# yangao07/LAMSA

Hardware: AMD Instinct MI355X
Metric: aligned Gbase/s, 10 kbp ONT-error reads (12%: sub/ins/del 4% each), -T ont2d vs GRCh37-sized stand-in; inputs resident in HBM when the timed region starts (upload excluded: see pcie_inclusive_*) (higher is better)
Workload: dtype int32

## Files before the change

lamsa_amd/csrc/hp_align_api.hip:

```cpp
#include <hip/hip_runtime.h>
#include <algorithm>
#include <atomic>
#include <map>
#include <mutex>
#include <stdlib.h>
#include <string.h>
#include <time.h>
#include "hp_phase.h"
#include "hp_handle.h"
#include "hp_hostprep.h"

using namespace hp;

#ifndef HP_WAVES_PER_SIMD
#define HP_WAVES_PER_SIMD 4
#endif
__global__ __launch_bounds__(64, HP_WAVES_PER_SIMD) void k_align_batch(AlignArgs a)
{
    __shared__ int32_t lds[HP_BOTH_LDS_WORDS];
    const int slot = blockIdx.x;
    for (;;) {
        int u = 0;
        if (wv::leader()) u = atomicAdd(a.counter, 1);
        u = wv::uni(u);
// ... 144 lines not shown
    for (int64_t i = (int64_t)blockIdx.x * blockDim.x + threadIdx.x; i < n; i += (int64_t)gridDim.x * blockDim.x) { const int b = src[i]; dst[i] = ((b & 63) << 4) | (b >> 6); }
}
__global__ void k_off_widen(const int32_t *src, int64_t *dst, int64_t n)
{
    for (int64_t i = (int64_t)blockIdx.x * blockDim.x + threadIdx.x; i < n; i += (int64_t)gridDim.x * blockDim.x) dst[i] = src[i];
}
#define HP_SCAN_BLOCK 4096
__global__ __launch_bounds__(256) void k_scan_sums(const uint8_t *src, int64_t n, int64_t *sums)
{
    __shared__ int part[256];
    const int64_t b0 = (int64_t)blockIdx.x * HP_SCAN_BLOCK;
    int s = 0;
    for (int i = threadIdx.x; i < HP_SCAN_BLOCK; i += 256) { const int64_t k = b0 + i; s += k < n ? src[k] : 0; }
    part[threadIdx.x] = s;
    __syncthreads();
    for (int st = 128; st > 0; st >>= 1) { if ((int)threadIdx.x < st) part[threadIdx.x] += part[threadIdx.x + st]; __syncthreads(); }
    if (threadIdx.x == 0) sums[blockIdx.x] = part[0];
}
__global__ __launch_bounds__(256) void k_scan_bases(int64_t *sums, int64_t nb)
{
    __shared__ long long tot[256];
    const int64_t per = (nb + 255) / 256, a = (int64_t)threadIdx.x * per, b = a + per < nb ? a + per : nb;
    long long s = 0;
    for (int64_t i = a; i < b; ++i) s += sums[i];
    tot[threadIdx.x] = s;
    __syncthreads();
    if (threadIdx.x == 0) { long long run = 0; for (int t = 0; t < 256; ++t) { const long long v = tot[t]; tot[t] = run; run += v; } }
    __syncthreads();
    long long run = tot[threadIdx.x];
    for (int64_t i = a; i < b; ++i) { const long long v = sums[i]; sums[i] = run; run += v; }
}
__global__ __launch_bounds__(256) void k_scan_apply(const uint8_t *src, int64_t n, const int64_t *bases, int64_t *dst)
{
    __shared__ int part[256];
    const int64_t b0 = (int64_t)blockIdx.x * HP_SCAN_BLOCK + (int64_t)threadIdx.x * 16;
    int v[16], s = 0;
#pragma unroll
    for (int i = 0; i < 16; ++i) { const int64_t k = b0 + i; v[i] = k < n ? src[k] : 0; s += v[i]; }
    part[threadIdx.x] = s;
    __syncthreads();
    if (threadIdx.x == 0) { int run = 0; for (int t = 0; t < 256; ++t) { const int x = part[t]; part[t] = run; run += x; } }
    __syncthreads();
    long long run = bases[blockIdx.x] + part[threadIdx.x];
#pragma unroll
    for (int i = 0; i < 16; ++i) { const int64_t k = b0 + i; if (k < n) dst[k] = run; run += v[i]; }
}

static double now_s() { timespec t; clock_gettime(CLOCK_MONOTONIC, &t); return t.tv_sec + 1e-9 * t.tv_nsec; }
static const bool g_trace = getenv("LAMSA_HP_TRACE") != nullptr;
static const bool g_noshare = getenv("LAMSA_HP_FULL_GRIDS") != nullptr;
static const bool g_nowave = getenv("LAMSA_HP_NO_WAVE_JOBS") != nullptr;
static const bool g_nolane = getenv("LAMSA_HP_NO_LANE_DP") != nullptr;
static const bool g_mono = getenv("LAMSA_HP_ONE_KERNEL") != nullptr;

struct HostBuf {
    void *p = nullptr, *dev = nullptr; size_t cap = 0;
    int ensure(size_t bytes) {
        if (bytes <= cap) return 0;
        if (p) hipHostFree(p);
        p = dev = nullptr; cap = 0;
        size_t want = bytes + bytes / 4 + 256;
        if (hipHostMalloc(&p, want, hipHostMallocMapped) != hipSuccess) { p = nullptr; return -1; }
        if (hipHostGetDevicePointer(&dev, p, 0) != hipSuccess) { hipHostFree(p); p = nullptr; return -1; }
        cap = want;
        return 0;
    }
    void release() { if (p) hipHostFree(p); p = dev = nullptr; cap = 0; }
};

struct OutDev {
    DevBuf buf; HostBuf host; int64_t stream_cap = 0; int n_cap = 0;
    static size_t hdr(int n) { return al256(8 * (size_t)n) + 3 * al256(4 * (size_t)n) + 256 + al256(16 * (size_t)n); }
    int ensure(int n, int64_t cap) { stream_cap = cap; n_cap = n; return buf.ensure(4 * (size_t)cap + 256) || host.ensure(hdr(n) + 256); }
    int64_t *off() const { return (int64_t *)host.dev; }
    int32_t *len(int n) const { return (int32_t *)((char *)host.dev + al256(8 * (size_t)n)); }
    int32_t *st(int n) const { return (int32_t *)((char *)host.dev + al256(8 * (size_t)n) + al256(4 * (size_t)n)); }
    int32_t *tb(int n) const { return (int32_t *)((char *)host.dev + al256(8 * (size_t)n) + 2 * al256(4 * (size_t)n)); }
    unsigned long long *diag(int n) const { return (unsigned long long *)((char *)host.dev + al256(8 * (size_t)n) + 3 * al256(4 * (size_t)n)); }
    const unsigned long long *h_diag(int n) const { return (const unsigned long long *)((const char *)host.p + al256(8 * (size_t)n) + 3 * al256(4 * (size_t)n)); }
    int32_t *work(int n) const { return (int32_t *)((char *)host.dev + al256(8 * (size_t)n) + 3 * al256(4 * (size_t)n) + 256); }
    const int32_t *h_work(int n) const { return (const int32_t *)((const char *)host.p + al256(8 * (size_t)n) + 3 * al256(4 * (size_t)n) + 256); }
    const int64_t *h_off() const { return (const int64_t *)host.p; }
    const int32_t *h_len(int n) const { return (const int32_t *)((const char *)host.p + al256(8 * (size_t)n)); }
    const int32_t *h_st(int n) const { return (const int32_t *)((const char *)host.p + al256(8 * (size_t)n) + al256(4 * (size_t)n)); }
    const int32_t *h_tb(int n) const { return (const int32_t *)((const char *)host.p + al256(8 * (size_t)n) + 2 * al256(4 * (size_t)n)); }
    int32_t *stream(int) const { return (int32_t *)buf.p; }
    void release() { buf.release(); host.release(); }
};

struct Slot {
    DevBuf bin, misc, slab, pers, prof; OutDev out1;
    HostBuf args_host;
    hipEvent_t ep[7] = {nullptr, nullptr, nullptr, nullptr, nullptr, nullptr, nullptr};
    hipStream_t cs = nullptr;
    bool valid = false;
    bool phased = false;
    int32_t n_reads = 0; int64_t n_bases = 0, n_cig = 0, n_hits = 0;
    BatchIn in; const int32_t *d_order = nullptr;
    std::vector<int32_t> order, h_len, h_H; std::vector<uint8_t> h_skip;
    int32_t max_L = 0, max_H = 0;
    int32_t sort_pb = 40, sort_cb = 24;
    hipEvent_t e0 = nullptr, e1 = nullptr;
};

struct AlignState {
    Slot slot[2];
    int fifo[2] = {0, 0}, n_fifo = 0;
    int res_fifo[2] = {0, 0}, n_res = 0;
    DevBuf retry_list;
    OutDev out2;
    HostBuf stream;
    std::vector<int32_t> r_len, r_st, r_tb, r_work; std::vector<int64_t> r_off;
};

static std::map<lamsa_hp_handle *, AlignState *> g_states;
static std::mutex g_states_lock;
static AlignState *state_of(lamsa_hp_handle *h)
{
    std::lock_guard<std::mutex> guard(g_states_lock);
    auto it = g_states.find(h);
    if (it != g_states.end()) return it->second;
    return g_states[h] = new AlignState();
}
extern "C" void lamsa_hp_release_state_(lamsa_hp_handle *h)
{
    AlignState *S = nullptr;
    {
        std::lock_guard<std::mutex> guard(g_states_lock);
        auto it = g_states.find(h);
        if (it == g_states.end()) return;
        S = it->second;
        g_states.erase(it);
    }
    if (h->stream) hipStreamSynchronize(h->stream);
    if (h->stream_b) hipStreamSynchronize(h->stream_b);
    for (Slot &T : S->slot) { T.bin.release(); T.misc.release(); T.slab.release(); T.pers.release(); T.prof.release(); T.args_host.release(); T.out1.release(); for (hipEvent_t e : {T.e0, T.e1, T.ep[0], T.ep[1], T.ep[2], T.ep[3], T.ep[4], T.ep[5], T.ep[6]}) if (e) hipEventDestroy(e); }
    S->retry_list.release(); S->out2.release(); S->stream.release();
    delete S;
}

static int grow(lamsa_hp_handle *h, DevBuf &b, size_t bytes)
{
    if (bytes <= b.cap) return 0;
    if (hipStreamSynchronize(h->stream) != hipSuccess || hipStreamSynchronize(h->stream_b) != hipSuccess) return -1;
    return b.ensure(bytes);
}

static size_t tag_slab_per_base(int tags, int eqx) { return (size_t)((tags & HP_TAGS_LISTS) ? 152 : 128) + ((tags & LAMSA_HP_TAG_EQX) ? (size_t)eqx : 0); }
static size_t slab_bytes_for(const lamsa_hp_para &P, int L, int H, int scale, int tags)
{
    const size_t z = (2 * (size_t)P.band_w + 128) * ((size_t)L + 256);
    return al256(((size_t)256 << 10) + (size_t)scale * tag_slab_per_base(tags, 40) * (size_t)L + 424 * (size_t)H + z * (size_t)(scale > 1 ? 4 : 1));
}


static int upload_into(lamsa_hp_handle *h, Slot *S, const lamsa_hp_batch *B)
{
    S->valid = false;
    const double t_0 = now_s();
    const int n = B->n_reads;
    const int64_t n_slots = n ? B->seed_off[n] : 0, n_hits = n_slots ? B->hit_off[n_slots] : 0, n_bases = n ? B->read_off[n] : 0;
    S->h_len.assign((size_t)n, 0); S->h_H.assign((size_t)n, 0); S->h_skip.assign((size_t)n + 1, 0); S->max_L = 0; S->max_H = 0;
    if (n && (B->seed_off[0] != 0 || B->read_off[0] != 0 || (n_slots && B->hit_off[0] != 0))) { h->err = "offsets must start at 0"; return LAMSA_HP_EINVAL; }
    const bool packed_off = B->h_cig_off == nullptr, cig_bytes = B->cig8 != nullptr;
    if (B->n_cig < 0 || (!packed_off && B->n_cig > 0x7fffffffll)) { h->err = "more than 2^31-1 seed CIGAR elements with 32-bit h_cig_off: pass h_cig_off = NULL (CIGARs back to back in hit order) or split the batch"; return LAMSA_HP_EINVAL; }
    if (!cig_bytes && !B->cig && B->n_cig > 0) { h->err = "neither cig nor cig8 given"; return LAMSA_HP_EINVAL; }
    {
        std::atomic<int> bad(0);
        const int64_t sl = h->para.seed_len, ss = h->para.seed_step > 0 ? h->para.seed_step : 1;
        std::atomic<long long> max_pos(0), sum_cig(0);
        hp_parallel_blocks(n, [&](int r0, int r1) {
            long long mp = 0, sc = 0;
            for (int r = r0; r < r1 && !bad.load(std::memory_order_relaxed); ++r) {
                const int64_t L = B->read_off[r + 1] - B->read_off[r], ns = B->seed_off[r + 1] - B->seed_off[r];
                if (L < 0 || L > (1 << 24) || ns < 0) { bad = 1; return; }
                if (ns > HP_MAX_SLOTS) S->h_skip[r] = 1;
                {
                    const int64_t sa = L < sl ? 0 : 1 + (L - sl) / ss;
                    if (B->seed_all[r] != sa || B->last_len[r] != L - sl - (sa - 1) * ss) { bad = 7; return; }
                    if (sa > 32767) S->h_skip[r] = 1;
                }
                int64_t H = 0;
                for (int64_t s = B->seed_off[r]; s < B->seed_off[r + 1]; ++s) {
                    const int64_t m = B->hit_off[s + 1] - B->hit_off[s];
                    if (m < 0 || (m > HP_MAX_HITS_PER_SEED && !S->h_skip[r])) { bad = 2; return; }
                    if (B->seed_id[s] < 1 || B->seed_id[s] > B->seed_all[r] || (s > B->seed_off[r] && B->seed_id[s] <= B->seed_id[s - 1])) { bad = 3; return; }
                    H += m;
                }
                if (H > (1 << 22) && !S->h_skip[r]) { bad = 4; return; }
                for (int64_t i = B->read_off[r]; i < B->read_off[r + 1]; ++i) if (B->read_seq[i] > 4) { bad = 5; return; }
                for (int64_t k = B->hit_off[B->seed_off[r]]; k < B->hit_off[B->seed_off[r + 1]]; ++k) {
                    mp = B->h_pos[k] > mp ? B->h_pos[k] : mp;
                    if (B->h_len_dif[k] < -127 || B->h_len_dif[k] > 127) S->h_skip[r] = 1;
                    if (B->h_chr[k] < 1 || B->h_chr[k] > h->n_seqs || (B->h_strand[k] != 1 && B->h_strand[k] != -1) || B->h_pos[k] < 0 || B->h_pos[k] >= (1ll << 40) ||
                        (!packed_off && (B->h_cig_off[k] < 0 || (int64_t)B->h_cig_off[k] + B->h_cig_n[k] > B->n_cig))) { bad = 6; return; }
                    sc += B->h_cig_n[k];
                }
                S->h_len[r] = (int32_t)L; S->h_H[r] = (int32_t)H;
            }
            long long seen = max_pos.load();
            while (mp > seen && !max_pos.compare_exchange_weak(seen, mp)) { }
            sum_cig += sc;
        });
        static const char *why[] = {"", "read longer than 2^24 bases", "too many hits in one seed", "seed ids must be ascending in [1, seed_all]",
                                    "too many hits in one read", "read base code > 4",
                                    "bad hit record (contig id, strand, position or seed CIGAR range)",
                                    "seed_all / last_len do not match the read length and the handle's seed length and step"};
        if (bad) { h->err = why[bad.load()]; return LAMSA_HP_EINVAL; }
        if (packed_off && sum_cig.load() != B->n_cig) { h->err = "h_cig_off is NULL but the h_cig_n do not add up to n_cig"; return LAMSA_HP_EINVAL; }
        for (int r = 0; r < n; ++r) { if (S->h_skip[r]) { S->h_len[r] = 0; S->h_H[r] = 0; } S->max_L = std::max(S->max_L, S->h_len[r]); S->max_H = std::max(S->max_H, S->h_H[r]); }
        auto bits = [](unsigned long long x) { int b = 0; while (x) { ++b; x >>= 1; } return b; };
        S->sort_pb = bits((unsigned long long)max_pos.load()); S->sort_cb = bits((unsigned long long)(2 * (long long)h->n_seqs + 1));
    }
    const double t_1 = now_s();
    S->order.resize((size_t)n);
    for (int r = 0; r < n; ++r) S->order[r] = r;
    {
        std::vector<double> cost((size_t)n);
        for (int r = 0; r < n; ++r) cost[r] = (double)S->h_H[r] * S->h_H[r] / 64.0 + (double)S->h_len[r] * (2.0 * h->para.band_w + 1) / 16.0;
        std::stable_sort(S->order.begin(), S->order.end(), [&](int x, int y) { return cost[x] > cost[y]; });
    }
    size_t off = 0;
    auto place = [&](size_t bytes) { size_t o = off; off = al256(off + bytes + 16); return o; };
    const size_t o_roff = place(8 * ((size_t)n + 1)), o_rseq = place((size_t)n_bases), o_sall = place(4 * (size_t)n), o_last = place(4 * (size_t)n),
                 o_soff = place(8 * ((size_t)n + 1)), o_sid = place(4 * (size_t)n_slots), o_hoff = place(8 * ((size_t)n_slots + 1)),
                 o_pos = place(8 * (size_t)n_hits), o_chr = place(4 * (size_t)n_hits), o_coff = place(8 * (size_t)n_hits), o_nm = place(2 * (size_t)n_hits),
                 o_ld = place(2 * (size_t)n_hits), o_st = place((size_t)n_hits), o_cn = place((size_t)n_hits), o_cig = place(4 * (size_t)B->n_cig), o_ord = place(4 * (size_t)n),
                 o_stage = place(packed_off ? 8 * ((size_t)n_hits / HP_SCAN_BLOCK + 2) : 4 * (size_t)n_hits), o_cig8 = place(cig_bytes ? (size_t)B->n_cig : 0), o_skip = place((size_t)n);
    const double t_3 = now_s();
    if (S->bin.ensure(off)) { h->err = "hipMalloc(batch)"; return LAMSA_HP_ENOMEM; }
    char *d = (char *)S->bin.p;
    hipStream_t s = h->copy_stream;
    static const int64_t zero64 = 0;
#define UP(o, src, bytes) do { if ((bytes) > 0) HIPCHK(h, hipMemcpyAsync(d + (o), (src), (bytes), hipMemcpyHostToDevice, s), LAMSA_HP_EKERNEL); } while (0)
    if (n) { UP(o_roff, B->read_off, 8 * ((size_t)n + 1)); UP(o_soff, B->seed_off, 8 * ((size_t)n + 1)); }
    else { UP(o_roff, &zero64, 8); UP(o_soff, &zero64, 8); }
    UP(o_rseq, B->read_seq, (size_t)n_bases); UP(o_sall, B->seed_all, 4 * (size_t)n); UP(o_last, B->last_len, 4 * (size_t)n);
    UP(o_sid, B->seed_id, 4 * (size_t)n_slots);
    if (n_slots) UP(o_hoff, B->hit_off, 8 * ((size_t)n_slots + 1)); else UP(o_hoff, &zero64, 8);
    UP(o_pos, B->h_pos, 8 * (size_t)n_hits); UP(o_chr, B->h_chr, 4 * (size_t)n_hits);
    if (!packed_off) UP(o_stage, B->h_cig_off, 4 * (size_t)n_hits);
    UP(o_nm, B->h_nm, 2 * (size_t)n_hits); UP(o_ld, B->h_len_dif, 2 * (size_t)n_hits); UP(o_st, B->h_strand, (size_t)n_hits); UP(o_cn, B->h_cig_n, (size_t)n_hits);
    if (cig_bytes) UP(o_cig8, B->cig8, (size_t)B->n_cig); else UP(o_cig, B->cig, 4 * (size_t)B->n_cig);
    UP(o_ord, S->order.data(), 4 * (size_t)n); UP(o_skip, S->h_skip.data(), (size_t)n);
#undef UP
    if (cig_bytes && B->n_cig > 0) hipLaunchKernelGGL(k_cig8_expand, dim3(2048), dim3(256), 0, s, (const uint8_t *)(d + o_cig8), (int32_t *)(d + o_cig), (int64_t)B->n_cig);
    if (n_hits > 0) {
        if (!packed_off) hipLaunchKernelGGL(k_off_widen, dim3(2048), dim3(256), 0, s, (const int32_t *)(d + o_stage), (int64_t *)(d + o_coff), (int64_t)n_hits);
        else {
            const int64_t nb = (n_hits + HP_SCAN_BLOCK - 1) / HP_SCAN_BLOCK;
            hipLaunchKernelGGL(k_scan_sums, dim3((unsigned)nb), dim3(256), 0, s, (const uint8_t *)(d + o_cn), (int64_t)n_hits, (int64_t *)(d + o_stage));
            hipLaunchKernelGGL(k_scan_bases, dim3(1), dim3(256), 0, s, (int64_t *)(d + o_stage), nb);
            hipLaunchKernelGGL(k_scan_apply, dim3((unsigned)nb), dim3(256), 0, s, (const uint8_t *)(d + o_cn), (int64_t)n_hits, (const int64_t *)(d + o_stage), (int64_t *)(d + o_coff));
        }
    }
    HIPCHK(h, hipGetLastError(), LAMSA_HP_EKERNEL);
    HIPCHK(h, hipStreamSynchronize(s), LAMSA_HP_EKERNEL);
    if (g_trace) fprintf(stderr, "[lamsa_hp] upload: validate %.1f ms, order %.1f ms, copy %.1f ms (%.2f GB on the device)\n", 1e3 * (t_1 - t_0), 1e3 * (t_3 - t_1), 1e3 * (now_s() - t_3), off / 1e9);
    BatchIn &in = S->in;
    in.n_reads = n; in.read_skip = (const uint8_t *)(d + o_skip); in.read_off = (const int64_t *)(d + o_roff); in.read_seq = (const uint8_t *)(d + o_rseq);
    in.seed_all = (const int32_t *)(d + o_sall); in.last_len = (const int32_t *)(d + o_last); in.seed_off = (const int64_t *)(d + o_soff);
    in.seed_id = (const int32_t *)(d + o_sid); in.hit_off = (const int64_t *)(d + o_hoff); in.h_pos = (const int64_t *)(d + o_pos);
    in.h_chr = (const int32_t *)(d + o_chr); in.h_cig_off = (const int64_t *)(d + o_coff); in.h_nm = (const int16_t *)(d + o_nm);
    in.h_len_dif = (const int16_t *)(d + o_ld); in.h_strand = (const int8_t *)(d + o_st); in.h_cig_n = (const uint8_t *)(d + o_cn);
    in.cig = (const int32_t *)(d + o_cig);
    S->d_order = (const int32_t *)(d + o_ord);
    S->n_reads = n; S->n_bases = n_bases; S->n_cig = B->n_cig; S->n_hits = n_hits;
    S->valid = true;
    return LAMSA_HP_OK;
}

static int cap_waves(int n_waves, size_t slab_per_wave, int n_cu)
{
    static const size_t budget = []() { size_t f = 0, t = 0; if (hipMemGetInfo(&f, &t) != hipSuccess || t == 0) { t = (size_t)288 << 30; f = t; } return std::min(t / 4, f / 3); }();
    if (slab_per_wave * (size_t)n_waves <= budget) return n_waves;
    size_t fit = budget / (slab_per_wave ? slab_per_wave : 1);
    if (n_cu > 0 && fit >= (size_t)n_cu) fit -= fit % (size_t)n_cu;
    return fit < 1 ? 1 : (int)fit;
}

#ifdef HP_PROF
static void prof_report(Slot &T, const long long *d_prof, int n)
{
    if (!d_prof) return;
    {
        std::vector<long long> pr((size_t)n * 64);
        hipMemcpy(pr.data(), d_prof, sizeof(long long) * pr.size(), hipMemcpyDeviceToHost);
        if (const char *dump = getenv("LAMSA_HP_PROF_DUMP")) {
            if (FILE *fp = fopen(dump, "wb")) {
                for (int r = 0; r < n; ++r) { long long hl[2] = {T.h_H[r], T.h_len[r]}; fwrite(hl, 8, 2, fp); fwrite(&pr[(size_t)r * 64], 8, 64, fp); }
                fclose(fp);
            }
        }
        std::vector<int> idx((size_t)n); for (int i = 0; i < n; ++i) idx[i] = i;
        auto tot = [&](int r) { long long t = 0; for (int k = 0; k < 6; ++k) t += pr[(size_t)r * 64 + k]; return t; };
        std::sort(idx.begin(), idx.end(), [&](int x, int y) { return tot(x) > tot(y); });
        long long sum[64] = {0}; for (int r = 0; r < n; ++r) for (int k = 0; k < 64; ++k) sum[k] += pr[(size_t)r * 64 + k];
        fprintf(stderr, "[HP_PROF] cycles: setup chain1 fill1 chain2 fill2 publish | in chain1: init+minext mainscan track pop-loop bound+flines | o_l H\n");
        fprintf(stderr, "[HP_PROF] SUM  "); for (int k = 0; k < 11; ++k) fprintf(stderr, " %lld", sum[k] / 1000000); fprintf(stderr, " (Mcycles) targets %lld trips %lld init_Mcyc %lld\n", sum[11], sum[12], sum[13] / 1000000);
#ifdef HP_PROF_TRACK
        fprintf(stderr, "[HP_PROF] branch tracking (-DHP_PROF_TRACK: the line_build stamps below are off): marking pass, image build and write-back %lld Mcyc; %lld seeds visited; %lld tracks, %lld Mcyc in them, %lld steps up; "
                        "%lld arrivals at a node with several sons, %lld Mcyc in cut_branch\n", sum[16] / 1000000, sum[19], sum[18], sum[17] / 1000000, sum[20], sum[21], sum[22] / 1000000);
#endif
        fprintf(stderr, "[HP_PROF] line_build: %lld lines (%lld without a gap), %lld anchors, %lld gaps | Mcyc: anchor walk %lld, gap list %lld, gaps in lanes %lld, gaps one by one %lld, assembly %lld\n",
                sum[21], sum[22], sum[12], sum[23], sum[16] / 1000000, sum[17] / 1000000, sum[18] / 1000000, sum[19] / 1000000, sum[20] / 1000000);
        fprintf(stderr, "[HP_PROF] gaps: %lld in lines with fewer than HP_GAP_MIN gaps (%lld lines with gaps); lane gaps: %lld hits scanned, %lld refused (range too long or too many active hits)\n", sum[54], sum[55], sum[11], sum[13]);
        { const char *nm[] = {"ksw_global", "ksw_extend", "backtrack", "ref_fetch", "head_fix", "frag_extend", "split_mapping", "tail_fix", "res_split", "res_aux", "mini_line_regs", "sort index"};
          for (int k = 0; k < 12; ++k) fprintf(stderr, "[HP_PROF] %-16s %8lld Mcyc %10lld calls\n", nm[k], sum[24 + 2 * k] / 1000000, sum[25 + 2 * k]);
#ifdef HP_PROF_FILL
          fprintf(stderr, "[HP_PROF] in frags_merge: boundary repair (merge_cigar_full) %lld Mcyc %lld calls; junctions through split_mapping %lld Mcyc %lld calls; fragments of several seeds %lld Mcyc %lld calls; 64-step gathers %lld Mcyc %lld\n", sum[16] / 1000000, sum[17], sum[18] / 1000000, sum[19], sum[20] / 1000000, sum[21], sum[22] / 1000000, sum[23]);
#endif
          fprintf(stderr, "[HP_PROF] direction-matrix bytes in HBM %lld (%lld jobs); hits passed through nodes_per_init %lld (%lld calls)\n", sum[52], sum[53], sum[54], sum[55]);
          fprintf(stderr, "[HP_PROF] chain_first start: seed loop %lld, node_set loop %lld, min_extend %lld Mcyc (%lld reads with a MIN pass)\n", sum[56] / 1000000, sum[57] / 1000000, sum[58] / 1000000, sum[59]);
          fprintf(stderr, "[HP_PROF] query <= 62: ksw_extend %lld Mcyc %lld calls, ksw_global %lld Mcyc %lld calls\n", sum[60] / 1000000, sum[61], sum[62] / 1000000, sum[63]);
          const char *bn[] = {"[bi_extend total]", "[bi_extend after left ext]", "17-32", "33-64", "65-128", "129-256", "257-512", ">512"};
          for (int k = 0; k < 2; ++k) fprintf(stderr, "[HP_PROF] ksw_extend qlen %-8s %8lld Mcyc %10lld calls\n", bn[k], sum[48 + 2 * k] / 1000000, sum[49 + 2 * k]); }
        {
            std::vector<long long> pd((size_t)n * 64);
            hipMemcpy(pd.data(), d_prof + ((size_t)n + 1) * 64, sizeof(long long) * pd.size(), hipMemcpyDeviceToHost);
            long long sd[64] = {0}; for (int r = 0; r < n; ++r) for (int k = 0; k < 64; ++k) sd[k] += pd[(size_t)r * 64 + k];
            const char *cn[] = {"one set, q <= 62", "packed, one set", "packed, two sets", "band 1 set slides", "band 2 sets slides", "band 4 sets slides", "int32 sets", "LDS / HBM rows",
                                "band 1 set fixed", "band 2 sets fixed", "band 4 sets fixed"};
            for (int c = 0; c < 11; ++c) fprintf(stderr, "[HP_PROF] wave jobs, ksw_extend %-18s %8lld Mcyc %10lld Mcells %9lld calls %10lld rows\n", cn[c], sd[4 * c] / 1000000, sd[4 * c + 1] / 1000000, sd[4 * c + 2], sd[4 * c + 3]);
            fprintf(stderr, "[HP_PROF] wave jobs, junctions of the class 'band 2 sets fixed': %lld jobs, wj_run %lld Mcyc of which staging %lld; ksw_bi_extend %lld Mcyc of which after the left extension %lld; "
                            "in ksw_extend_band<2>: setup and first fill %lld, rows %lld, backtrack %lld Mcyc\n",
                    sd[51], sd[50] / 1000000, sd[49] / 1000000, sd[47] / 1000000, sd[48] / 1000000, sd[44] / 1000000, sd[45] / 1000000, sd[46] / 1000000);
        }
        for (int q = 0; q < 8 && q < n; ++q) { int r = idx[q]; fprintf(stderr, "[HP_PROF] read %d L=%d:", r, T.h_len[r]); for (int k = 0; k < 11; ++k) fprintf(stderr, " %lld", pr[(size_t)r * 64 + k] / 1000000); fprintf(stderr, " | o_l %lld H %lld | targets %lld trips %lld init_Mcyc %lld\n", pr[(size_t)r * 64 + 14], pr[(size_t)r * 64 + 15], pr[(size_t)r * 64 + 11], pr[(size_t)r * 64 + 12], pr[(size_t)r * 64 + 13] / 1000000); }
    }
}
#endif

struct PhasedLayout { size_t bytes, o[15]; int unit_cap, lj_cap, wj_cap; int64_t fl_cap, line_cap, job_cap; };
static PhasedLayout phased_layout(int n, int64_t n_hits, int64_t n_bases, int64_t stream_cap)
{
    PhasedLayout Y;
    const size_t n_ent = (size_t)n_hits + (size_t)n + 1;
    Y.unit_cap = 8 * n + 1024;
    Y.fl_cap = 4 * n_hits + 2304 * (int64_t)n + 4096; Y.line_cap = stream_cap + 64 * (int64_t)Y.unit_cap;
    Y.job_cap = std::min<int64_t>(0x7fffff00ll, 4096 + 256 * (int64_t)n + 2 * n_bases);
    Y.lj_cap = (int)std::min<int64_t>(0x3fffffffll, 1024 + 16 * (int64_t)n + n_bases / 100);
    Y.wj_cap = (int)std::min<int64_t>(0x3fffffffll, 1024 + 32 * (int64_t)n + n_bases / 200);
    size_t off = 0;
    auto place = [&](size_t bytes) { size_t o = off; off = al256(off + bytes + 16); return o; };
    const size_t sz[15] = {sizeof(PhaseArgs), sizeof(PhaseCtl), sizeof(RdMeta) * ((size_t)n + 1), sizeof(NodeS) * n_ent, 4 * n_ent, 8 * n_ent, sizeof(UnitRec) * 2 * (size_t)Y.unit_cap,
                           4 * 2 * (size_t)PH_NBUCKET * Y.unit_cap, 4 * (size_t)Y.fl_cap, 4 * (size_t)Y.line_cap, 4 * (size_t)Y.job_cap, sizeof(LjRec) * (size_t)Y.lj_cap, 4 * (size_t)LJ_NBUCKET * Y.lj_cap,
                           sizeof(WjRec) * (size_t)Y.wj_cap, 4 * (size_t)WJ_NBUCKET * Y.wj_cap};
    for (int k = 0; k < 15; ++k) Y.o[k] = place(sz[k]);
    Y.bytes = off;
    return Y;
}
static int64_t main_stream_cap(int n, int64_t n_bases, int tags)
{
    return 1024 + (int64_t)n * 256 + 4 * n_bases + ((tags & LAMSA_HP_TAG_MISMATCHES) ? (int64_t)n * 128 + 2 * n_bases : 0) + ((tags & LAMSA_HP_TAG_EQX) ? (int64_t)n * 128 + 4 * n_bases : 0);
}

struct SlabPlan { size_t chain, fill, wj, wjb, wjb_off; int w_chain, w_fill, w_dp, w_wj, n_wjb, shape; size_t bytes; };
static int chain_shape(const lamsa_hp_para &P, int64_t n_reads, int64_t n_bases)
{
    static const int force = getenv("LAMSA_HP_CHAIN_SHAPE") ? atoi(getenv("LAMSA_HP_CHAIN_SHAPE")) : -1;
    if (force >= 0 && force < 3) return force;
    const int64_t mean_L = n_reads > 0 ? n_bases / n_reads : 0, ss = P.seed_step > 0 ? P.seed_step : 1;
    const int64_t est = mean_L / ss * 2 / 3;
    for (int k = 0; k < 2; ++k) if (est <= g_chain_shapes[k].lds_words / 5) return k;
    return 2;
}
static SlabPlan slab_plan(lamsa_hp_handle *h, int max_L, int max_H, bool shared = false, int shape = 0)
{
    SlabPlan Q;
    Q.shape = shape;
    const lamsa_hp_para &P = h->para;
    Q.chain = al256(((size_t)256 << 10) + 128 * (size_t)max_L + 424 * (size_t)max_H);
    Q.fill = al256(((size_t)256 << 10) + tag_slab_per_base(h->result_tags, 16) * (size_t)max_L + sizeof(cig_t) * 3 * HP_LJ_CIG * 64 + (size_t)HP_LJ_QSMALL * HP_LJ_TSMALL * 64 + 64);
    { static const int kb = getenv("LAMSA_HP_WJ_SLAB_KB") ? atoi(getenv("LAMSA_HP_WJ_SLAB_KB")) : 0;
      Q.wj = ((size_t)(kb > 0 ? kb : 1024) << 10) + 33 * 256; }
    Q.wjb = al256((size_t)wj_need(&P, WJ_HEAD, max_L, max_L + 2 * P.hash_step + 64) + ((size_t)64 << 10)) + 33 * 256;
    if (Q.wjb < Q.wj) Q.wjb = Q.wj;
    if (g_nowave) Q.fill = std::max(Q.fill, slab_bytes_for(P, max_L, max_H, 1, h->result_tags));
    if (h->scratch_limit) { const size_t lim = al256(h->scratch_limit); Q.chain = std::min(Q.chain, lim); Q.fill = std::min(Q.fill, lim); Q.wj = std::min(Q.wj, lim); Q.wjb = std::min(Q.wjb, lim); }
    int pc = 0, pf = 0, pd = 0, pw = 0;
    if (hipOccupancyMaxActiveBlocksPerMultiprocessor(&pc, g_chain_shapes[shape].k1, 64, 0) != hipSuccess || pc < 1) pc = 4 * g_chain_shapes[shape].waves_per_simd;
    if (hipOccupancyMaxActiveBlocksPerMultiprocessor(&pf, k_fill, 64, 0) != hipSuccess || pf < 1) pf = 4;
    if (hipOccupancyMaxActiveBlocksPerMultiprocessor(&pd, k_filldp_small, 64, 0) != hipSuccess || pd < 1) pd = 4;
    if (hipOccupancyMaxActiveBlocksPerMultiprocessor(&pw, k_filldp_wave, 64, 0) != hipSuccess || pw < 1) pw = 4;
    if (shared && !g_noshare) { pc = std::min(pc, 8); pf = std::min(pf, 16); pw = std::min(pw, 16); }
    { static const int cf = getenv("LAMSA_HP_FILL_PER_CU") ? atoi(getenv("LAMSA_HP_FILL_PER_CU")) : 0, cc = getenv("LAMSA_HP_CHAIN_PER_CU") ? atoi(getenv("LAMSA_HP_CHAIN_PER_CU")) : 0,
                       cw = getenv("LAMSA_HP_WJ_PER_CU") ? atoi(getenv("LAMSA_HP_WJ_PER_CU")) : 0;
      if (cf > 0 && cf < pf) pf = cf;
      if (cc > 0 && cc < pc) pc = cc;
      if (cw > 0 && cw < pw) pw = cw; }
    Q.w_chain = cap_waves(h->n_cu * pc, Q.chain, h->n_cu); Q.w_fill = cap_waves(h->n_cu * pf, Q.fill, h->n_cu);
    Q.w_dp = std::min(h->n_cu * pd, Q.w_fill); Q.w_wj = cap_waves(h->n_cu * pw, Q.wj, h->n_cu);
    { const size_t budget_big = (size_t)12 << 30; size_t nb = budget_big / Q.wjb; if (nb < 1) nb = 1; Q.n_wjb = (int)std::min<size_t>(nb, (size_t)Q.w_wj); }
    Q.wjb_off = al256(Q.wj * (size_t)Q.w_wj);
    const size_t wj_bytes = Q.wjb_off + Q.wjb * (size_t)Q.n_wjb;
    Q.bytes = std::max(std::max(Q.chain * (size_t)Q.w_chain, Q.fill * (size_t)Q.w_fill), wj_bytes);
    return Q;
}

static int launch_phased(lamsa_hp_handle *h, AlignState *S, Slot &T, Slot &Ln, OutDev &O, hipEvent_t e0, hipEvent_t e1)
{
    const int n = T.n_reads;
    const int64_t n_hits = T.n_hits;
    const SlabPlan Q = slab_plan(h, T.max_L, T.max_H, S->n_fifo + S->n_res > 0, chain_shape(h->para, T.n_reads, T.n_bases));
    const int w_chain = Q.w_chain, w_fill = Q.w_fill, w_dp = Q.w_dp, w_wj = Q.w_wj;
    const PhasedLayout Y = phased_layout(n, n_hits, T.n_bases, O.stream_cap);
    const int unit_cap = Y.unit_cap, lj_cap = Y.lj_cap; const int64_t fl_cap = Y.fl_cap, line_cap = Y.line_cap, job_cap = Y.job_cap;
    const size_t off = Y.bytes, o_args = Y.o[0], o_ctl = Y.o[1], o_meta = Y.o[2], o_nd = Y.o[3], o_ns = Y.o[4], o_sx = Y.o[5], o_un = Y.o[6], o_bq = Y.o[7], o_fl = Y.o[8], o_ln = Y.o[9],
                 o_jb = Y.o[10], o_lj = Y.o[11], o_lq = Y.o[12], o_wj = Y.o[13], o_wq = Y.o[14];
    if (grow(h, Ln.slab, Q.bytes) || grow(h, Ln.pers, off) || Ln.misc.ensure(256)) { h->err = "hipMalloc(slab)"; return LAMSA_HP_ENOMEM; }
    char *d = (char *)Ln.pers.p;
    PhaseArgs a;
    a.P = h->para;
    a.ref.pac = h->d_pac; a.ref.l_pac = h->l_pac; a.ref.n_seqs = h->n_seqs; a.ref.seq_off = h->d_seq_off; a.ref.seq_len = h->d_seq_len;
    a.in = T.in; a.in.tags = h->result_tags;
    a.out.read_out_off = O.off(); a.out.read_out_len = O.len(n); a.out.read_status = O.st(n); a.out.read_tbases = O.tb(n); a.out.read_work = O.work(n); a.out.stream = O.stream(n);
    a.out.stream_cap = O.stream_cap; a.out.cursor = (unsigned long long *)((char *)Ln.misc.p + 64); a.out.diag = O.diag(n);
    a.slab = (char *)Ln.slab.p; a.slab_per_wave = Q.chain; a.slab_fill = Q.fill; a.slab_wj = Q.wj; a.slab_wjb = Q.wjb; a.wjb_off = Q.wjb_off; a.n_wjb = Q.n_wjb; a.sort_pb = T.sort_pb; a.sort_cb = T.sort_cb;
    a.order = T.d_order; a.n_reads = n; a.prof = nullptr;
#ifdef HP_PROF
    if (Ln.prof.ensure(sizeof(long long) * 64 * 2 * ((size_t)n + 1))) { h->err = "hipMalloc(prof)"; return LAMSA_HP_ENOMEM; }
    a.prof = (long long *)Ln.prof.p;
    HIPCHK(h, hipMemsetAsync(Ln.prof.p, 0, sizeof(long long) * 64 * 2 * ((size_t)n + 1), Ln.cs), LAMSA_HP_EKERNEL);
#endif
    a.g_nd = (NodeS *)(d + o_nd); a.g_nseed = (int32_t *)(d + o_ns); a.g_sidx = (int32_t *)(d + o_sx); a.meta = (RdMeta *)(d + o_meta);
    a.units = (UnitRec *)(d + o_un); a.unit_cap = unit_cap; a.bucket_q = (int32_t *)(d + o_bq);
    a.fl_base = (int32_t *)(d + o_fl); a.fl_cap = fl_cap; a.line_base = (int32_t *)(d + o_ln); a.line_cap = line_cap; a.ctl = (PhaseCtl *)(d + o_ctl);
    a.job_base = (int32_t *)(d + o_jb); a.job_cap = job_cap;
    a.ljobs = (LjRec *)(d + o_lj); a.lj_bucket = (int32_t *)(d + o_lq); a.lj_cap = g_nolane ? 0 : lj_cap;
    a.wjobs = (WjRec *)(d + o_wj); a.wj_bucket = (int32_t *)(d + o_wq); a.wj_cap = g_nowave ? 0 : Y.wj_cap;
    const bool list = !g_nolane || !g_nowave;
    hipStream_t s = Ln.cs;
    HIPCHK(h, hipMemsetAsync(Ln.misc.p, 0, 128, s), LAMSA_HP_EKERNEL);
    HIPCHK(h, hipMemsetAsync(d + o_ctl, 0, (o_meta - o_ctl) + sizeof(RdMeta) * ((size_t)n + 1), s), LAMSA_HP_EKERNEL);
    if (Ln.args_host.ensure(sizeof a)) { h->err = "hipHostMalloc(args)"; return LAMSA_HP_ENOMEM; }
    memcpy(Ln.args_host.p, &a, sizeof a);
    HIPCHK(h, hipMemcpyAsync(d + o_args, Ln.args_host.p, sizeof a, hipMemcpyHostToDevice, s), LAMSA_HP_EKERNEL);
    const PhaseArgs *da = (const PhaseArgs *)(d + o_args);
    HIPCHK(h, hipEventRecord(e0, s), LAMSA_HP_EKERNEL);
    hipLaunchKernelGGL(g_chain_shapes[Q.shape].k1, dim3(std::min(w_chain, n)), dim3(64), 0, s, da);
    HIPCHK(h, hipEventRecord(Ln.ep[0], s), LAMSA_HP_EKERNEL);
    if (list) {
        hipLaunchKernelGGL(k_filllist, dim3(w_fill), dim3(64), 0, s, da, 0);
        HIPCHK(h, hipEventRecord(Ln.ep[5], s), LAMSA_HP_EKERNEL);
        if (!g_nowave) hipLaunchKernelGGL(k_filldp_wave, dim3(w_wj), dim3(64), 0, s, da, 0);
        HIPCHK(h, hipEventRecord(Ln.ep[6], s), LAMSA_HP_EKERNEL);
        if (!g_nolane) hipLaunchKernelGGL(k_filldp_small, dim3(w_dp), dim3(64), 0, s, da, 0);
    } else { HIPCHK(h, hipEventRecord(Ln.ep[5], s), LAMSA_HP_EKERNEL); HIPCHK(h, hipEventRecord(Ln.ep[6], s), LAMSA_HP_EKERNEL); }
    HIPCHK(h, hipEventRecord(Ln.ep[4], s), LAMSA_HP_EKERNEL);
    hipLaunchKernelGGL(k_fill, dim3(w_fill), dim3(64), 0, s, da, 0);
    HIPCHK(h, hipEventRecord(Ln.ep[1], s), LAMSA_HP_EKERNEL);
    hipLaunchKernelGGL(g_chain_shapes[Q.shape].k2, dim3(std::min(w_chain, n)), dim3(64), 0, s, da);
    HIPCHK(h, hipEventRecord(Ln.ep[2], s), LAMSA_HP_EKERNEL);
    if (list) {
        HIPCHK(h, hipMemsetAsync(&((PhaseCtl *)(d + o_ctl))->q_head[5], 0, 16, s), LAMSA_HP_EKERNEL);
        hipLaunchKernelGGL(k_filllist, dim3(w_fill), dim3(64), 0, s, da, 1);
        if (!g_nowave) hipLaunchKernelGGL(k_filldp_wave, dim3(w_wj), dim3(64), 0, s, da, 1);
        if (!g_nolane) hipLaunchKernelGGL(k_filldp_small, dim3(w_dp), dim3(64), 0, s, da, 1);
    }
    hipLaunchKernelGGL(k_fill, dim3(w_fill), dim3(64), 0, s, da, 1);
    HIPCHK(h, hipEventRecord(Ln.ep[3], s), LAMSA_HP_EKERNEL);
    hipLaunchKernelGGL(k_publish, dim3(std::min(h->n_cu * 8, n)), dim3(64), 0, s, da);
    HIPCHK(h, hipGetLastError(), LAMSA_HP_EKERNEL);
    HIPCHK(h, hipEventRecord(e1, s), LAMSA_HP_EKERNEL);
    Ln.phased = true;
    return LAMSA_HP_OK;
}

static int launch_align(lamsa_hp_handle *h, AlignState *S, Slot &T, Slot &Ln, OutDev &O, const int32_t *d_order, int n_units, int scale, int max_L, int max_H,
                        hipEvent_t e0, hipEvent_t e1, bool wait)
{
    size_t slab_per_wave = slab_bytes_for(h->para, max_L, max_H, scale, h->result_tags);
    if (scale == 1 && h->scratch_limit && slab_per_wave > h->scratch_limit) slab_per_wave = al256(h->scratch_limit);
    int per_cu = 0;
    if (hipOccupancyMaxActiveBlocksPerMultiprocessor(&per_cu, k_align_batch, 64, 0) != hipSuccess || per_cu < 1) per_cu = 4;
    int n_waves = h->n_cu * per_cu;
    if (n_waves > n_units) n_waves = n_units;
    n_waves = cap_waves(n_waves, slab_per_wave, h->n_cu);
    if (grow(h, Ln.slab, slab_per_wave * (size_t)n_waves) || Ln.misc.ensure(256)) { h->err = "hipMalloc(slab)"; return LAMSA_HP_ENOMEM; }
    const int n = T.n_reads;
    AlignArgs a;
    a.P = h->para;
    a.ref.pac = h->d_pac; a.ref.l_pac = h->l_pac; a.ref.n_seqs = h->n_seqs; a.ref.seq_off = h->d_seq_off; a.ref.seq_len = h->d_seq_len;
    a.in = T.in; a.in.tags = h->result_tags;
    a.out.read_out_off = O.off(); a.out.read_out_len = O.len(n); a.out.read_status = O.st(n); a.out.read_tbases = O.tb(n); a.out.read_work = O.work(n); a.out.stream = O.stream(n);
    a.out.stream_cap = O.stream_cap; a.out.cursor = (unsigned long long *)((char *)Ln.misc.p + 64); a.out.diag = nullptr;
    a.slab = (char *)Ln.slab.p; a.slab_per_wave = slab_per_wave; a.counter = (int32_t *)Ln.misc.p;
    a.order = d_order; a.n_units = n_units; a.scale = scale; a.prof = nullptr; a.sort_pb = T.sort_pb; a.sort_cb = T.sort_cb;
    hipStream_t s = Ln.cs;
    HIPCHK(h, hipMemsetAsync(Ln.misc.p, 0, 128, s), LAMSA_HP_EKERNEL);
    HIPCHK(h, hipEventRecord(e0, s), LAMSA_HP_EKERNEL);
    hipLaunchKernelGGL(k_align_batch, dim3(n_waves), dim3(64), 0, s, a);
    HIPCHK(h, hipGetLastError(), LAMSA_HP_EKERNEL);
    HIPCHK(h, hipEventRecord(e1, s), LAMSA_HP_EKERNEL);
    if (wait) HIPCHK(h, hipStreamSynchronize(s), LAMSA_HP_EKERNEL);
#ifdef HP_PROF
    prof_report(T, a.prof, n);
#endif
    return LAMSA_HP_OK;
}

static int slot_events(lamsa_hp_handle *h, Slot &Ln)
{
    Ln.cs = &Ln == &state_of(h)->slot[1] ? h->stream_b : h->stream;
    if (!Ln.e0) HIPCHK(h, hipEventCreate(&Ln.e0), LAMSA_HP_EKERNEL);
    if (!Ln.e1) HIPCHK(h, hipEventCreate(&Ln.e1), LAMSA_HP_EKERNEL);
    for (hipEvent_t &e : Ln.ep) if (!e) HIPCHK(h, hipEventCreate(&e), LAMSA_HP_EKERNEL);
    return LAMSA_HP_OK;
}

static int start_main(lamsa_hp_handle *h, AlignState *S, Slot &T, Slot &Ln)
{
    int rc = slot_events(h, Ln);
    if (rc) return rc;
    const int n = T.n_reads;
    if (n == 0) return LAMSA_HP_OK;
    if (Ln.out1.ensure(n, main_stream_cap(n, T.n_bases, h->result_tags))) { h->err = "hipMalloc(out)"; return LAMSA_HP_ENOMEM; }
    Ln.phased = false;
    if (!g_mono) return launch_phased(h, S, T, Ln, Ln.out1, Ln.e0, Ln.e1);
    return launch_align(h, S, T, Ln, Ln.out1, T.d_order, n, 1, T.max_L, T.max_H, Ln.e0, Ln.e1, false);
}

#define DL(dst, src, bytes) HIPCHK(h, hipMemcpyAsync((dst), (src), (bytes), hipMemcpyDeviceToHost, h->copy_stream), LAMSA_HP_EKERNEL)
#define DLSYNC() HIPCHK(h, hipStreamSynchronize(h->copy_stream), LAMSA_HP_EKERNEL)

static int finish_main(lamsa_hp_handle *h, AlignState *S, Slot &T, Slot &Ln, lamsa_hp_result *R)
{
    const int n = T.n_reads;
    for (float &v : h->kernel_ms) v = 0;
    S->r_st.assign((size_t)n + 1, 0); S->r_off.assign((size_t)n + 1, 0); S->r_len.assign((size_t)n + 1, 0); S->r_tb.assign((size_t)n + 1, 0); S->r_work.assign(4 * (size_t)n + 4, 0);
    if (S->stream.ensure(64)) { h->err = "hipHostMalloc(results)"; return LAMSA_HP_ENOMEM; }
    if (n == 0) {
        if (R) { R->stream = (const int32_t *)S->stream.p; R->stream_words = 0; R->read_off = S->r_off.data(); R->read_len = S->r_len.data(); R->read_status = S->r_st.data(); R->read_tbases = S->r_tb.data(); R->read_work = S->r_work.data(); }
        return LAMSA_HP_OK;
    }
    const double t_0 = now_s();
    HIPCHK(h, hipEventSynchronize(Ln.e1), LAMSA_HP_EKERNEL);
    const double t_1 = now_s();
    hipEventElapsedTime(&h->kernel_ms[0], Ln.e0, Ln.e1);
    if (Ln.phased) {
        hipEvent_t ev[6] = {Ln.e0, Ln.ep[0], Ln.ep[1], Ln.ep[2], Ln.ep[3], Ln.e1};
        for (int k = 0; k < 5; ++k) hipEventElapsedTime(&h->kernel_ms[2 + k], ev[k], ev[k + 1]);
        const unsigned long long *dg = Ln.out1.h_diag(n);
        for (int k = 0; k < 4; ++k) h->kernel_ms[7 + k] = dg[2 * k + 1] >= dg[2 * k] && dg[2 * k + 1] ? (float)((double)(dg[2 * k + 1] - dg[2 * k]) * 1e-5) : 0.f;
        h->kernel_ms[11] = (float)dg[8]; h->kernel_ms[12] = (float)dg[9];
        hipEventElapsedTime(&h->kernel_ms[13], Ln.ep[0], Ln.ep[4]);
        hipEventElapsedTime(&h->kernel_ms[14], Ln.ep[0], Ln.ep[5]);
        hipEventElapsedTime(&h->kernel_ms[15], Ln.ep[5], Ln.ep[6]);
        h->kernel_ms[16] = (float)dg[12]; h->kernel_ms[17] = (float)((double)dg[13] * 1e-6); h->kernel_ms[18] = (float)dg[14]; h->kernel_ms[19] = (float)((double)dg[15] * 4e-6); h->kernel_ms[20] = (float)((double)dg[16] * 1e-6);
#ifdef HP_PROF
        prof_report(T, (const long long *)Ln.prof.p, n);
#endif
    }
    memcpy(S->r_off.data(), Ln.out1.h_off(), 8 * (size_t)n); memcpy(S->r_len.data(), Ln.out1.h_len(n), 4 * (size_t)n);
    memcpy(S->r_st.data(), Ln.out1.h_st(n), 4 * (size_t)n); memcpy(S->r_tb.data(), Ln.out1.h_tb(n), 4 * (size_t)n); memcpy(S->r_work.data(), Ln.out1.h_work(n), 16 * (size_t)n);
    unsigned long long used1 = 0;
    for (int r = 0; r < n; ++r) if (S->r_off[r] >= 0 && (unsigned long long)(S->r_off[r] + S->r_len[r]) > used1) used1 = (unsigned long long)(S->r_off[r] + S->r_len[r]);
    if ((int64_t)used1 > Ln.out1.stream_cap) used1 = (unsigned long long)Ln.out1.stream_cap;
    std::vector<int32_t> again;
    for (int r = 0; r < n; ++r) if ((S->r_st[r] & LAMSA_HP_ST_OVERFLOW) || S->r_off[r] < 0) again.push_back(r);
#ifdef HP_CHAIN_STOP
    again.clear();
#endif
    unsigned long long used2 = 0;
    if (!again.empty()) {
        int mL = 0, mH = 0; int64_t cap2 = 1024;
        for (int r : again) { mL = std::max(mL, T.h_len[r]); mH = std::max(mH, T.h_H[r]); cap2 += read_out_cap(T.h_len[r], 8, h->result_tags); }
        if (grow(h, S->out2.buf, 4 * (size_t)cap2 + 256) || S->out2.host.ensure(OutDev::hdr(n) + 256) || grow(h, S->retry_list, 4 * again.size())) { h->err = "hipMalloc(retry)"; return LAMSA_HP_ENOMEM; }
        S->out2.stream_cap = cap2;
        HIPCHK(h, hipMemcpyAsync(S->retry_list.p, again.data(), 4 * again.size(), hipMemcpyHostToDevice, Ln.cs), LAMSA_HP_EKERNEL);
        int rc = launch_align(h, S, T, Ln, S->out2, (const int32_t *)S->retry_list.p, (int)again.size(), 8, mL, mH, h->ev0, h->ev1, true);
        if (rc) return rc;
        hipEventElapsedTime(&h->kernel_ms[1], h->ev0, h->ev1);
        const int64_t *off2 = S->out2.h_off(); const int32_t *len2 = S->out2.h_len(n), *st2 = S->out2.h_st(n), *tb2 = S->out2.h_tb(n), *wk2 = S->out2.h_work(n);
        for (int r : again) if (off2[r] >= 0 && (unsigned long long)(off2[r] + len2[r]) > used2) used2 = (unsigned long long)(off2[r] + len2[r]);
        if ((int64_t)used2 > cap2) used2 = (unsigned long long)cap2;
        for (int r : again) { S->r_st[r] = st2[r]; S->r_len[r] = len2[r]; S->r_tb[r] = tb2[r]; for (int q = 0; q < 4; ++q) S->r_work[4 * r + q] = wk2[4 * r + q]; S->r_off[r] = off2[r] < 0 ? -1 : (int64_t)used1 + off2[r]; }
    }
    for (int r = 0; r < n; ++r) if (S->r_off[r] < 0) { S->r_off[r] = 0; S->r_len[r] = 0; S->r_st[r] |= LAMSA_HP_ST_OVERFLOW; }
    if (!R) return LAMSA_HP_OK;
    if (S->stream.ensure(4 * (size_t)(used1 + used2) + 64)) { h->err = "hipHostMalloc(results)"; return LAMSA_HP_ENOMEM; }
    int32_t *hs = (int32_t *)S->stream.p;
    if (used1) DL(hs, Ln.out1.stream(n), 4 * (size_t)used1);
    if (used2) DL(hs + used1, S->out2.stream(n), 4 * (size_t)used2);
    DLSYNC();
    if (g_trace) fprintf(stderr, "[lamsa_hp] collect: waited %.1f ms for the kernel (%.1f ms), results %.1f ms (%.2f GB)\n", 1e3 * (t_1 - t_0), h->kernel_ms[0], 1e3 * (now_s() - t_1), 4e-9 * (double)(used1 + used2));
    R->stream = hs; R->stream_words = (int64_t)(used1 + used2); R->read_off = S->r_off.data(); R->read_len = S->r_len.data(); R->read_status = S->r_st.data(); R->read_tbases = S->r_tb.data(); R->read_work = S->r_work.data();
    return LAMSA_HP_OK;
}
#undef DL
#undef DLSYNC

static int check_batch_args(lamsa_hp_handle *h, const lamsa_hp_batch *B)
{
    if (!h || !B || B->n_reads < 0) return LAMSA_HP_EINVAL;
    if (!h->d_pac) { h->err = "handle was created without a reference"; return LAMSA_HP_EINVAL; }
    HIPCHK(h, hipSetDevice(h->device), LAMSA_HP_ENODEV);
    return LAMSA_HP_OK;
}

extern "C" int lamsa_hp_upload_batch(lamsa_hp_handle *h, const lamsa_hp_batch *B)
{
    int rc = check_batch_args(h, B);
    if (rc) return rc;
    AlignState *S = state_of(h);
    if (S->n_fifo || S->n_res) { h->err = "batches are in flight: collect them first"; return LAMSA_HP_EINVAL; }
    return upload_into(h, &S->slot[0], B);
}
// ... 124 lines not shown
```

lamsa_amd/csrc/hp_chain.h:

```cpp
#pragma once
#include "hp_batch.h"
#include "hp_sort.h"

namespace hp {

enum { F_MATCH = 0, F_SPLIT_MATCH = 1, F_MISMATCH = 2, F_MATCH_THD = 2, F_LONG_MISMATCH = 3, F_INSERT = 4, F_DELETE = 5,
       F_CHR_DIF = 6, F_REVERSE = 7, F_UNCONNECT = 8, F_UNMATCH = 9, F_INIT = 20 };
enum { MIN_FLAG = 1, MULTI_FLAG = 2, UNLIMITED_FLAG = 3, WHOLE_FLAG = 4, TRACKED_FLAG = 5 };
enum { L_MERGB = 0, L_NMERG = 1, L_MERGH = 2, L_INTER = 4, L_DUMP = 8 };

HP_INL int score_table(int flag) { return flag <= 3 ? 1 : (flag <= 7 ? -3 : -6); }

#define HP_MAX_SLOTS 16383
#define HP_MAX_HITS_PER_SEED 16383

struct NodeS {
    int64_t pos;
    int32_t chr;
    int32_t slot_j;
    int16_t sid;
    int8_t strand, len_dif8;
    int8_t dp_flag;
    uint8_t son_flag;
    uint8_t match_flag;
    uint8_t pad_;
    int32_t score, NM;
};

struct ReadCtx {
    Ctx cx;
    RefView ref;
    int L, seed_all, seed_out, last_len, H;
    const uint8_t *read;
    uint8_t *rc_read; bool rc_ready;
    const uint8_t *cur_read;
    long long t_bases;
    long long n_pairs;
    long long cs_words;
    bool flip;
    const int32_t *seed_id;
    const int64_t *hit_off;
    int64_t hb;
    const int64_t *h_pos, *h_cig_off; const int32_t *h_chr; const int16_t *h_nm, *h_len_dif;
    const int8_t *h_strand; const uint8_t *h_cig_n; const int32_t *cig;
    int32_t *n_from, *n_in_de, *n_son_n, *n_first, *n_last, *n_next;
    int32_t *n_max_score, *n_max_NM, *n_max_node, *n_node_n, *n_seed;
    NodeS *nd;
    const int32_t *srt, *rnk;
    bool nodes_ready;
    HP_L int32_t *leaf_bits; bool leaf_on;
    long long *prof;
};

HP_INL int hoff(const ReadCtx &r, int x) { return (int)(r.hit_off[x] - r.hb); }
HP_INL int mapn(const ReadCtx &r, int x) { return (int)(r.hit_off[x + 1] - r.hit_off[x]); }
HP_INL int sid(const ReadCtx &r, int x) { int s = r.seed_id[x]; return r.flip ? r.seed_all + 1 - s : s; }
HP_INL int nx(const ReadCtx &r, int node) { return node < 0 ? -1 : r.n_seed[node]; }

HP_INL void node_set(ReadCtx &r, int n, int from, int score, int NM, int match_flag, int dp_flag)
{
    r.nd[n].son_flag = F_INIT; r.n_from[n] = from; r.nd[n].score = score; r.nd[n].NM = NM;
    r.nd[n].match_flag = (uint8_t)match_flag; r.nd[n].dp_flag = (int8_t)dp_flag;
    r.n_node_n[n] = 1; r.n_in_de[n] = 0; r.n_son_n[n] = 0; r.n_first[n] = -1; r.n_last[n] = -1;
    r.n_max_score[n] = score; r.n_max_NM[n] = NM; r.n_max_node[n] = n;
}
HP_INL void add_son(ReadCtx &r, int fa, int son)
{
    ++r.n_in_de[fa];
    r.n_next[son] = -1;
    if (r.n_son_n[fa] == 0) r.n_first[fa] = son; else r.n_next[r.n_last[fa]] = son;
    r.n_last[fa] = son;
    ++r.n_son_n[fa];
}

HP_INL NodeS node_load(const HP_G NodeS *p)
{
    int a[4], b[4];
    hp_load16(p, a); hp_load16((const HP_G char *)p + 16, b);
    NodeS q;
    q.pos = (int64_t)(((unsigned long long)(unsigned)a[1] << 32) | (unsigned)a[0]); q.chr = a[2]; q.slot_j = a[3];
    q.sid = (int16_t)(b[0] & 0xffff); q.strand = (int8_t)((b[0] >> 16) & 0xff); q.len_dif8 = (int8_t)((b[0] >> 24) & 0xff);
    q.dp_flag = (int8_t)(b[1] & 0xff); q.son_flag = (uint8_t)((b[1] >> 8) & 0xff); q.match_flag = (uint8_t)((b[1] >> 16) & 0xff); q.pad_ = 0;
    q.score = b[2]; q.NM = b[3];
    return q;
}

struct EdgeK { int seed_step, seed_len, match_dis, high_err, mis3, sv_len, half_split; };
HP_INL EdgeK edge_consts(const lamsa_hp_para *P)
{
    EdgeK k; k.seed_step = P->seed_step; k.seed_len = P->seed_len; k.match_dis = P->match_dis; k.high_err = P->aln_mode & 2;
    k.mis3 = 3 * P->mismatch_thd; k.sv_len = P->SV_len_thd; k.half_split = P->split_len / 2;
    return k;
}
HP_INL int edge_flag_packed(const EdgeK &k, const NodeS &pre, const NodeS &cur)
{
    if ((pre.slot_j >> 14) == (cur.slot_j >> 14)) return F_UNCONNECT;
    const int sp = pre.strand;
    if (cur.chr != pre.chr || cur.strand != sp) return F_CHR_DIF;
    const int idp = pre.sid, idc = cur.sid, did = iabs(idp - idc);
    if (did * k.seed_step < k.seed_len) return F_UNCONNECT;
    const int64_t exp = pre.pos + (int64_t)(sp * (idc - idp) * k.seed_step);
    const int64_t act = cur.pos;
    const int dis = (int)((int64_t)sp * ((idp < idc) ? (act - exp) : (exp - act)) - ((sp * (idp - idc) < 0) ? pre.len_dif8 : cur.len_dif8));
    const int mat_dis = k.match_dis * (k.high_err ? did : 1);
    if (dis <= mat_dis && dis >= -mat_dis) return did == 1 ? F_MATCH : (did <= k.mis3 ? F_MISMATCH : F_LONG_MISMATCH);
    if (dis > mat_dis && dis < k.sv_len) return F_DELETE;
    if ((dis < -mat_dis && dis >= 0 - (did * k.seed_step - k.seed_len)) || (dis < -k.half_split && dis >= -k.sv_len)) return F_INSERT;
    return F_UNCONNECT;
}

HP_NOINL void nodes_per_init(ReadCtx &r, int k0, int k1, int from, int dp_flag, int which, int rlo = 0, int rhi = 0x7fffffff)
{
#ifdef HP_PROF
    if (r.prof) { r.prof[54] += k1 - k0; r.prof[55] += 1; }
#endif
#ifdef HP_PROF
    const long long t0_ = wv::clock();
#endif
    const HP_G NodeS *ns = (const HP_G NodeS *)r.nd;
    const EdgeK K = edge_consts(r.cx.P);
    NodeS F; F.pos = 0; F.chr = 0; F.slot_j = 0; F.sid = 0; F.strand = 0; F.len_dif8 = 0; F.pad_ = 0; F.dp_flag = 0; F.son_flag = 0; F.match_flag = 0; F.score = 0; F.NM = 0;
    int from_nm = 0;
    if (from >= 0) { F = node_load(ns + from); from_nm = r.h_nm[from]; r.n_pairs += k1 > k0 ? k1 - k0 : 0; }
    for (int b = k0; b < k1; b += 64) {
        WAVE_FOR(l) {
            const int k = b + l;
            if (k < k1) {
                const int df = r.nd[k].dp_flag;
                const bool take = which == 0 ? (df == dp_flag || df == 0 - dp_flag) : (df != TRACKED_FLAG);
                if (take) {
                    if (from < 0) {
                        const int rk = rhi == 0x7fffffff ? 0 : r.rnk[k];
                        if (rk >= rlo && rk <= rhi) node_set(r, k, from, 1, r.h_nm[k], F_MATCH, dp_flag);
                        else r.nd[k].dp_flag = (int8_t)(0 - dp_flag);
                    } else {
                        const NodeS Q = node_load(ns + k);
                        const int flag = k == from ? F_MATCH : edge_flag_packed(K, F, Q);
                        if (flag != F_UNCONNECT && flag != F_CHR_DIF) node_set(r, k, from, 2 + score_table(flag), r.h_nm[k] + from_nm, flag, dp_flag);
                        else r.nd[k].dp_flag = (int8_t)(0 - dp_flag);
                    }
                }
            }
        }
    }
    wv::sync();
#ifdef HP_PROF
    if (r.prof) r.prof[13] += wv::clock() - t0_;
#endif
}

struct ScanT { NodeS T; int tkey, x, t_NM; long long Rw; };

HP_INL NodeS node_unpack(const int *a, const int *b)
{
    NodeS q;
    q.pos = (int64_t)(((unsigned long long)(unsigned)a[1] << 32) | (unsigned)a[0]); q.chr = a[2]; q.slot_j = a[3];
    q.sid = (int16_t)(b[0] & 0xffff); q.strand = (int8_t)((b[0] >> 16) & 0xff); q.len_dif8 = (int8_t)((b[0] >> 24) & 0xff);
    q.dp_flag = (int8_t)(b[1] & 0xff); q.son_flag = (uint8_t)((b[1] >> 8) & 0xff); q.match_flag = (uint8_t)((b[1] >> 16) & 0xff); q.pad_ = 0;
    q.score = b[2]; q.NM = b[3];
    return q;
}

HP_INL void scan_eval(const EdgeK &K, const ScanT &S, const NodeS &Q, int p, int inb, int start_slot, int dp_flag,
                      long long &key, int &bp, int &bf, int &negp, int &n_p, int &n_f, int &n_c, int &n_n, int &outw, int &oka)
{
    const int POSMAX = (1 << 28) - 1;
    long long dp = Q.pos - S.T.pos; if (dp < 0) dp = -dp;
    const int inwin = inb & ((Q.chr * 2 + (Q.strand > 0 ? 1 : 0)) == S.tkey) & (dp <= S.Rw);
    outw = !inwin;
    const int qslot = Q.slot_j >> 14;
    const int flag = edge_flag_packed(K, Q, S.T);
    const int ok = inwin & (qslot >= start_slot) & (qslot < S.x) & (Q.dp_flag == dp_flag) & !((Q.strand == 1) & (Q.son_flag <= F_MATCH_THD)) &
                   (flag != F_UNCONNECT) & (flag != F_CHR_DIF);
    const int pos = (int)((unsigned)(S.x - 1 - qslot) << 14) | (Q.slot_j & 16383);
    const int cand = Q.score + 1 + score_table(flag);
    const int nm = Q.NM + S.t_NM;
    const int isneg = ok & (Q.strand == -1) & (flag <= F_MATCH_THD);
    const long long k = ((long long)(cand + 32768) << 47) | ((long long)(524287 - nm) << 28) | (long long)(POSMAX - pos);
    const long long kk = ok ? k : -1;
    const bool better = kk > key;
    key = better ? kk : key; bp = better ? p : bp; bf = better ? flag : bf;
    const int np = isneg ? -pos : -0x7fffffff;
    const bool nb = np > negp;
    negp = nb ? np : negp; n_p = nb ? p : n_p; n_f = nb ? flag : n_f; n_c = nb ? cand : n_c; n_n = nb ? nm : n_n;
    oka |= ok;
}

HP_NOINL void dp_update_range(ReadCtx &r, int k0, int k1, int start_slot, int dp_flag, bool force, bool sons, const uint8_t *only = nullptr)
{
    const HP_G uint8_t *g_only = (const HP_G uint8_t *)only;
    const HP_G NodeS *ns = (const HP_G NodeS *)r.nd;
    HP_G NodeS *gd = (HP_G NodeS *)r.nd;
    HP_G int32_t *g_from = (HP_G int32_t *)r.n_from;
    HP_G int32_t *g_node_n = (HP_G int32_t *)r.n_node_n, *g_in_de = (HP_G int32_t *)r.n_in_de, *g_son_n = (HP_G int32_t *)r.n_son_n;
    HP_G int32_t *g_first = (HP_G int32_t *)r.n_first, *g_last = (HP_G int32_t *)r.n_last, *g_next = (HP_G int32_t *)r.n_next;
    const EdgeK K = edge_consts(r.cx.P);
    const HP_G int32_t *g_srt = (const HP_G int32_t *)r.srt, *g_rnk = (const HP_G int32_t *)r.rnk;
    const int sid_lo = start_slot < r.seed_out ? r.seed_id[start_slot] : 0;
    const int H = r.H;
#ifdef HP_PROF
    const long long tu0_ = wv::clock();
    if (r.prof) { r.prof[13] += 1; }
#endif
    for (int tb = k0; tb < k1; tb += 64) {
#ifdef HP_PROF
        const long long tp0_ = wv::clock();
#endif
        wv::Lane<int> Ta0, Ta1, Ta2, Ta3, Tb0, Tb1, Tb2, Tb3, Trk, Tfrom, c;
        WAVE_FOR(l) {
            const int k = tb + l, kk = k < k1 ? k : k0;
            int a[4], b[4];
            hp_load16(ns + kk, a); hp_load16((const HP_G char *)(ns + kk) + 16, b);
            const int rk = g_rnk[kk];
            Ta0[l] = a[0]; Ta1[l] = a[1]; Ta2[l] = a[2]; Ta3[l] = a[3]; Tb0[l] = b[0]; Tb1[l] = b[1]; Tb2[l] = b[2]; Tb3[l] = b[3];
            Trk[l] = rk; Tfrom[l] = g_from[kk];
            int due = 0;
            if (!force) {
                const NodeS Tk = node_unpack(a, b);
                if (k < k1 && Tk.dp_flag == dp_flag && g_only) due = g_only[kk];
                else if (k < k1 && Tk.dp_flag == dp_flag) {
                    const int dm = Tk.sid - sid_lo;
                    const int mdm_ = K.match_dis * (K.high_err ? dm : 1);
                    long long Rk = K.sv_len > dm * K.seed_step ? K.sv_len : dm * K.seed_step;
                    if (mdm_ + 1 > Rk) Rk = mdm_ + 1;
                    Rk += 128 + (long long)dm * K.seed_step;
                    const int tk_ = Tk.chr * 2 + (Tk.strand > 0 ? 1 : 0);
#pragma unroll
                    for (int d = -1; d <= 1; d += 2) {
                        const int i2 = rk + d;
                        if (i2 >= 0 && i2 < H) {
                            const NodeS Nb = node_load(ns + g_srt[i2]);
                            long long dp_ = Nb.pos - Tk.pos; if (dp_ < 0) dp_ = -dp_;
                            due |= ((Nb.chr * 2 + (Nb.strand > 0 ? 1 : 0)) == tk_) & (dp_ <= Rk);
                        }
                    }
                }
            }
            c[l] = due;
        }
        unsigned long long todo = force ? 1ull : wv::ballot(c);
#ifdef HP_PROF
        if (r.prof) { r.prof[13] += 1; }
#endif
        if (!todo) continue;
#ifdef HP_PROF
        const long long tq0_ = wv::clock();
#endif
        int li = __builtin_ctzll(todo);
        wv::Lane<int> pn0, pn1;
        wv::Lane<int> Qa[2][4], Qb[2][4];
        {
            const int rT = wv::bcast(Trk, li);
            WAVE_FOR(l) {
                const int i0 = rT - 1 - l, i1 = rT + 1 + l;
                pn0[l] = g_srt[i0 >= 0 ? i0 : rT]; pn1[l] = g_srt[i1 < H ? i1 : rT];
            }
            WAVE_FOR(l) {
                int a[4], b[4];
                hp_load16(ns + pn0[l], a); hp_load16((const HP_G char *)(ns + pn0[l]) + 16, b);
#pragma unroll
                for (int q = 0; q < 4; ++q) { Qa[0][q][l] = a[q]; Qb[0][q][l] = b[q]; }
                hp_load16(ns + pn1[l], a); hp_load16((const HP_G char *)(ns + pn1[l]) + 16, b);
#pragma unroll
                for (int q = 0; q < 4; ++q) { Qa[1][q][l] = a[q]; Qb[1][q][l] = b[q]; }
            }
        }
#ifdef HP_PROF
        if (r.prof) r.prof[13] += 1;
#endif
        for (;;) {
            const int t = tb + li;
#ifdef HP_PROF
            if (r.prof) r.prof[11] += 1;
#endif
            ScanT S;
            {
                int a[4] = { wv::bcast(Ta0, li), wv::bcast(Ta1, li), wv::bcast(Ta2, li), wv::bcast(Ta3, li) };
                int b[4] = { wv::bcast(Tb0, li), wv::bcast(Tb1, li), wv::bcast(Tb2, li), wv::bcast(Tb3, li) };
                S.T = node_unpack(a, b);
            }
            const int rT = wv::bcast(Trk, li), t_from = wv::bcast(Tfrom, li);
            S.x = S.T.slot_j >> 14; S.t_NM = S.T.NM; S.tkey = S.T.chr * 2 + (S.T.strand > 0 ? 1 : 0);
            {
                const int did_max = S.T.sid - sid_lo;
                const int mdm = K.match_dis * (K.high_err ? did_max : 1);
                long long Rw = K.sv_len > did_max * K.seed_step ? K.sv_len : did_max * K.seed_step;
                if (mdm + 1 > Rw) Rw = mdm + 1;
                S.Rw = Rw + 128 + (long long)did_max * K.seed_step;
            }
            todo &= todo - 1;
            const bool has_next = todo != 0;
            const int li2 = has_next ? __builtin_ctzll(todo) : li;
            wv::Lane<int> pm0, pm1;
            if (has_next) {
                const int rT2 = wv::bcast(Trk, li2);
                WAVE_FOR(l) {
                    const int i0 = rT2 - 1 - l, i1 = rT2 + 1 + l;
                    pm0[l] = g_srt[i0 >= 0 ? i0 : rT2]; pm1[l] = g_srt[i1 < H ? i1 : rT2];
                }
            }
            r.n_pairs += (rT < 64 ? rT : 64) + (H - 1 - rT < 64 ? H - 1 - rT : 64);
            wv::Lane<long long> key;
            wv::Lane<int> bp, bf, negp, n_p, n_f, n_c, n_n, out0, out1, okl;
            WAVE_FOR(l) {
#ifdef HP_PROF
                if (l == 0 && r.prof) r.prof[13] += 1;
#endif
                key[l] = -1; bp[l] = 0; bf[l] = 0; negp[l] = -0x7fffffff; n_p[l] = 0; n_f[l] = 0; n_c[l] = 0; n_n[l] = 0;
                int ow[2], oka = 0;
#pragma unroll
                for (int u = 0; u < 2; ++u) {
                    int a[4], b[4];
#pragma unroll
                    for (int q = 0; q < 4; ++q) { a[q] = Qa[u][q][l]; b[q] = Qb[u][q][l]; }
                    const NodeS Q = node_unpack(a, b);
                    const int idx = u ? rT + 1 + l : rT - 1 - l;
                    scan_eval(K, S, Q, u ? pn1[l] : pn0[l], idx >= 0 && idx < H, start_slot, dp_flag,
                              key[l], bp[l], bf[l], negp[l], n_p[l], n_f[l], n_c[l], n_n[l], ow[u], oka);
                }
                out0[l] = ow[0]; out1[l] = ow[1]; okl[l] = oka;
            }
            bool live0 = wv::ballot(out0) == 0, live1 = wv::ballot(out1) == 0;
            int any_ok = wv::ballot(okl) != 0;
            for (int cc = 1; live0 || live1; ++cc) {
#ifdef HP_PROF
                if (r.prof) r.prof[13] += 1;
#endif
                {   const int lo_left = rT - cc * 64, hi_left = H - 1 - rT - cc * 64;
                    r.n_pairs += (live0 ? (lo_left < 0 ? 0 : (lo_left < 64 ? lo_left : 64)) : 0) + (live1 ? (hi_left < 0 ? 0 : (hi_left < 64 ? hi_left : 64)) : 0); }
                WAVE_FOR(l) {
                    int idx[2], inb[2], pn[2];
#pragma unroll
                    for (int u = 0; u < 2; ++u) {
                        idx[u] = rT + (u ? 1 : -1) * (1 + cc * 64 + l);
                        inb[u] = (u ? live1 : live0) && idx[u] >= 0 && idx[u] < H;
                        pn[u] = g_srt[inb[u] ? idx[u] : rT];
                    }
                    NodeS Q[2];
#pragma unroll
                    for (int u = 0; u < 2; ++u) Q[u] = node_load(ns + pn[u]);
                    int ow[2], oka = 0;
#pragma unroll
                    for (int u = 0; u < 2; ++u)
                        scan_eval(K, S, Q[u], pn[u], inb[u], start_slot, dp_flag, key[l], bp[l], bf[l], negp[l], n_p[l], n_f[l], n_c[l], n_n[l], ow[u], oka);
                    out0[l] = ow[0]; out1[l] = ow[1]; okl[l] = oka;
                }
                if (live0 && wv::ballot(out0) != 0) live0 = false;
                if (live1 && wv::ballot(out1) != 0) live1 = false;
                any_ok |= wv::ballot(okl) != 0;
            }
            int max_from = t_from, max_score = S.T.score, max_NM = S.t_NM, max_flag = 0;
            bool changed = false;
            if (any_ok) {
                const int npos = wv::reduce_max(negp);
                if (npos != -0x7fffffff) {
                    wv::Lane<int> w;
                    WAVE_FOR(l) w[l] = negp[l] == npos;
                    const int wl = __builtin_ctzll(wv::ballot(w));
                    max_from = wv::bcast(n_p, wl); max_flag = wv::bcast(n_f, wl); max_score = wv::bcast(n_c, wl); max_NM = wv::bcast(n_n, wl);
                    changed = max_from != t_from;
                } else {
                    const long long best_key = wv::reduce_max64(key);
                    if (best_key >= 0) {
                        const int nm = 524287 - (int)((best_key >> 28) & 524287);
                        const int cand = (int)(best_key >> 47) - 32768;
                        if (cand > max_score || (cand == max_score && nm < max_NM)) {
                            wv::Lane<int> w;
                            WAVE_FOR(l) w[l] = key[l] == best_key;
                            const int wl = __builtin_ctzll(wv::ballot(w));
                            max_from = wv::bcast(bp, wl); max_flag = wv::bcast(bf, wl); max_score = cand; max_NM = nm;
                            changed = max_from != t_from;
                        }
                    }
                }
            }
            if (changed) {
                gd[max_from].son_flag = (uint8_t)max_flag;
                g_from[t] = max_from; gd[t].score = max_score; gd[t].NM = max_NM; gd[t].match_flag = (uint8_t)max_flag;
            }
            if (has_next) {
                WAVE_FOR(l) {
                    int a[4], b[4];
                    hp_load16(ns + pm0[l], a); hp_load16((const HP_G char *)(ns + pm0[l]) + 16, b);
#pragma unroll
                    for (int q = 0; q < 4; ++q) { Qa[0][q][l] = a[q]; Qb[0][q][l] = b[q]; }
                    hp_load16(ns + pm1[l], a); hp_load16((const HP_G char *)(ns + pm1[l]) + 16, b);
#pragma unroll
                    for (int q = 0; q < 4; ++q) { Qa[1][q][l] = a[q]; Qb[1][q][l] = b[q]; }
                    pn0[l] = pm0[l]; pn1[l] = pm1[l];
                }
            }
            if (changed) {
                g_node_n[t] = g_node_n[max_from] + 1;
            }
            if (changed && sons) {
// ... 821 lines not shown

HP_NOINL void line_filter(ReadCtx &r, LSet &L, int ls, int len, Trig *trg, int per_max_multi)
{
    const size_t mark = arena_mark(r.cx.tmp);
    int32_t *mb, *cl_off, *cl_nm, *mfv, *mfn, *spare = nullptr; int spare_n = 0;
    if (L.xtra && 6 * len + 7 <= L.xtra_n) {
        mb = L.xtra; cl_off = mb + (len + 1); cl_nm = cl_off + (len + 2); mfv = cl_nm + (len + 1); mfn = mfv + (2 * len + 2);
        spare = mfn + (len + 1); spare_n = L.xtra_n - (6 * len + 7);
    } else {
        mb = (int32_t *)arena_alloc(r.cx, sizeof(int32_t) * (size_t)(len + 1));
        cl_off = (int32_t *)arena_alloc(r.cx, sizeof(int32_t) * (size_t)(len + 2));
        cl_nm = (int32_t *)arena_alloc(r.cx, sizeof(int32_t) * (size_t)(len + 1));
        mfv = (int32_t *)arena_alloc(r.cx, sizeof(int32_t) * (size_t)(2 * len + 2));
        mfn = (int32_t *)arena_alloc(r.cx, sizeof(int32_t) * (size_t)(len + 1));
    }
    if (!mb || !cl_off || !cl_nm || !mfv || !mfn) { arena_release(r.cx.tmp, mark); return; }
    int m_i = -1, nb = 0;
    for (int _i = ls; _i < ls + len; ++_i) {
        const int i = L.rank[_i];
        if (L.mf[i] & L_DUMP) continue;
        if (trg) {
            if (L.mf[i] & L_NMERG) { ++m_i; cl_off[m_i] = nb; cl_nm[m_i] = 1; mb[nb++] = i; }
            else if (L.mf[i] & L_MERGH) { ++m_i; cl_off[m_i] = nb; cl_nm[m_i] = 0; mb[nb++] = i; }
            else { if (m_i < 0) { r.cx.status |= ST_REFEXIT; arena_release(r.cx.tmp, mark); return; } mb[nb++] = i; }
        } else {
            if (L.mf[i] & L_NMERG) continue;
            if (L.mf[i] & L_MERGH) { ++m_i; cl_off[m_i] = nb; cl_nm[m_i] = 0; mb[nb++] = i; }
            else { if (m_i < 0) { r.cx.status |= ST_REFEXIT; arena_release(r.cx.tmp, mark); return; } mb[nb++] = i; }
        }
    }
    cl_off[m_i + 1] = nb;
    for (int c = 0; c <= m_i; ++c) {
        int32_t *mf = mfv + cl_off[c] + c;
        const int mbn = cl_off[c + 1] - cl_off[c];
        if (!trg) { pick_in_cluster(r, L, mb + cl_off[c], mbn, per_max_multi, nullptr, nullptr, spare, spare_n); continue; }
        if (cl_nm[c]) { mf[0] = mb[cl_off[c]]; mfn[c] = 1; continue; }
        const int n = pick_in_cluster(r, L, mb + cl_off[c], mbn, per_max_multi, trg->cnt, mf, spare, spare_n);
        mfn[c] = n;
        for (int ii = 1; ii < n; ++ii) {
            const int j = mf[ii], _j = L.sel[j];
            for (int k = 0; k < trg->cnt[j]; ++k) {
                int head = -1;
                const int n1 = trg->n1[trg->off[j] + k], n2 = trg->n2[trg->off[j] + k];
                for (int _l = _j + 1; _l < ls + len; ++_l) {
                    const int l = L.rank[_l];
                    if ((L.mf[l] & 0x3) != 0) break;
                    if (firstx(r, L, l) > r.n_seed[n1] && lastx(r, L, l) < r.n_seed[n2]) {
                        const int mfl = r.nd[n2].match_flag;
                        if (mfl == F_MISMATCH || mfl == F_LONG_MISMATCH) {
                            const int s = L.pool[L.start[l]], e = L.pool[L.start[l] + L.len[l] - 1];
                            const int st = r.h_strand[s];
                            if (st == r.h_strand[n1] || r.h_chr[s] != r.h_chr[n1] ||
                                st * r.h_pos[s] < st * r.h_pos[n2] || st * r.h_pos[e] > st * r.h_pos[n1]) continue;
                            L.mf[l] = L_INTER; HP_STAT(14);
                            if (head == -1) { L.mf[l] |= L_NMERG; head = l; }
                            else { L.mf[l] |= L_MERGB; L.mh[l] = head; L.mf[head] = L_INTER | L_MERGH; }
                        }
                    }
                }
            }
        }
    }
    if (trg && m_i > 0) {
        int a = mfv[cl_off[0] + 0], b = mfv[cl_off[1] + 1];
        if (lastx(r, L, a) - firstx(r, L, a) < 2 && lastx(r, L, b) - firstx(r, L, b) >= 2) dump_edge_cluster(L, ls, len, mfv + cl_off[0], mfn[0]);
        a = mfv[cl_off[m_i] + m_i]; b = mfv[cl_off[m_i - 1] + m_i - 1];
        if (lastx(r, L, a) - firstx(r, L, a) < 2 && lastx(r, L, b) - firstx(r, L, b) >= 2) dump_edge_cluster(L, ls, len, mfv + cl_off[m_i] + m_i, mfn[m_i]);
    }
    arena_release(r.cx.tmp, mark);
}

HP_NOINL int set_bound(ReadCtx &r, LSet &L, int ls, int len, Trig *trg)
{
    if (len <= 0) return len;
    const size_t mark = arena_mark(r.cx.tmp);
    int32_t *tmp = (L.xtra && len + 1 <= L.xtra_n) ? L.xtra : (int32_t *)arena_alloc(r.cx, sizeof(int32_t) * (size_t)(len + 1));
    if (!tmp) return 0;
    sort_endpos(r, L, ls, len, tmp);
    arena_release(r.cx.tmp, mark);
    L.mf[L.rank[ls]] = L_NMERG;
    for (int i = 1; i < len; ++i) line_merge(r, L, L.rank[ls + i], L.rank[ls + i - 1], r.cx.P->ovlp_rat);
    line_filter(r, L, ls, len, trg, r.cx.P->ske_max);
    int cur = ls;
    for (int _l = ls; _l < ls + len; ++_l) { const int l = L.rank[_l]; if (!(L.mf[l] & L_DUMP)) L.rank[cur++] = l; }
    return cur - ls;
}

struct FLines {
    int n, nfrag;
    int32_t *line_score, *left_bound, *right_bound, *frag_off;
    int32_t *fr_seed_off;
    int32_t *fr_seed;
    int32_t *jt, *gt;
    int32_t *ht;
    const int32_t *jarena;
};
enum { GS_OFF, GS_N, GS_TLEN, GS_HAS, GS_WORDS };
enum { ES_OFF, ES_N, ES_REFLEN, ES_READLEN, ES_HAS, ES_WORDS = 8, ES_LINE = 2 * ES_WORDS };

struct FlStore { int32_t *base; int64_t cap; unsigned long long *cursor; int64_t got_off; int32_t got_tot; };
HP_INL int flines_words(int line_n, int tot) { return 4 * (line_n + 1) + (tot + 2) + tot + 4 + 2 * GS_WORDS * (tot + 2) + ES_LINE * (line_n + 1); }
HP_INL void flines_bind(FLines &F, int32_t *m, int line_n, int tot)
{
    F.line_score = m; F.left_bound = m + (line_n + 1); F.right_bound = m + 2 * (line_n + 1); F.frag_off = m + 3 * (line_n + 1);
    F.fr_seed_off = m + 4 * (line_n + 1); F.fr_seed = F.fr_seed_off + (tot + 2);
    F.jt = F.fr_seed + tot + 4; F.gt = F.jt + GS_WORDS * (tot + 2);
    F.ht = F.gt + GS_WORDS * (tot + 2);
    F.jarena = nullptr;
}

HP_NOINL bool build_flines(ReadCtx &r, LSet &L, int line_n, FLines &F, FlStore *fs = nullptr)
{
    F.n = 0; F.nfrag = 0;
    if (line_n == 0) return true;
    int tot = 0;
    for (int _l = 0; _l < line_n; ++_l) tot += L.len[L.rank[_l]];
    int32_t *m = nullptr;
    if (fs) {
        const int words = (flines_words(line_n, tot) + 3) & ~3;
        unsigned long long off = 0;
        if (wv::leader()) off = atomicAdd(fs->cursor, (unsigned long long)words);
        off = (unsigned long long)wv::uni64((long long)off);
        if ((int64_t)(off + (unsigned long long)words) > fs->cap) { r.cx.status |= ST_OVERFLOW; return false; }
        m = fs->base + off; fs->got_off = (int64_t)off; fs->got_tot = tot;
    } else m = (int32_t *)arena_alloc(r.cx, sizeof(int32_t) * (size_t)flines_words(line_n, tot));
    if (!m) return false;
    flines_bind(F, m, line_n, tot);
    { HP_G int32_t *gj = (HP_G int32_t *)F.jt; const int nw = 2 * GS_WORDS * (tot + 2) + ES_LINE * (line_n + 1); for (int b0 = 0; b0 < nw; b0 += 64) { WAVE_FOR(l) { if (b0 + l < nw) gj[b0 + l] = 0; } } }
    const lamsa_hp_para *P = r.cx.P;
    const HP_G NodeS *gns = (const HP_G NodeS *)r.nd;
    if (P->aln_mode & 1) {
        for (int _i = 0; _i < line_n; ++_i) {
            const int li = L.rank[_i];
            int32_t *ni = L.pool + L.start[li]; const int ll = L.len[li];
            HP_G int32_t *gni = (HP_G int32_t *)ni;
            int last_i = 0, st_p = 0, ld_p = 0; long long pos_p = 0;
            for (int j0 = 0; j0 < ll; j0 += 64) {
                wv::Lane<int> plo, phi, ldl, stl, mfl;
                WAVE_FOR(l) {
                    const int j = j0 + l;
                    int a[4] = {0, 0, 0, 0}, b[4] = {0, 0, 0, 0};
                    if (j < ll) { const int c = gni[j]; hp_load16(gns + c, a); hp_load16((const HP_G char *)(gns + c) + 16, b); }
                    plo[l] = a[0]; phi[l] = a[1]; stl[l] = (int)(int8_t)((b[0] >> 16) & 0xff); ldl[l] = (int)(int8_t)((b[0] >> 24) & 0xff); mfl[l] = (b[1] >> 16) & 0xff;
                }
                const int cnt = ll - j0 < 64 ? ll - j0 : 64;
                for (int q = 0; q < cnt; ++q) {
                    const int j = j0 + q;
                    const long long pos_c = (long long)(((unsigned long long)(unsigned)wv::bcast(phi, q) << 32) | (unsigned)wv::bcast(plo, q));
                    const int st = wv::bcast(stl, q), ld_c = wv::bcast(ldl, q), mf_c = wv::bcast(mfl, q);
                    if (j == 0) { pos_p = pos_c; ld_p = ld_c; st_p = st; continue; }
                    const bool ovl = (long long)(P->seed_len + (st == 1 ? ld_p : ld_c)) > (long long)st * (pos_c - pos_p) && mf_c != F_INSERT;
                    if (j < ll - 1) {
                        if (ovl) gni[j] = -1; else { last_i = j; pos_p = pos_c; ld_p = ld_c; st_p = st; }
                    } else if (ll - 1 != last_i && ovl) gni[last_i] = -1;
                }
            }
            (void)st_p;
        }
        wv::sync();
    }
    int nf = 0, ns = 0;
    for (int _l = 0; _l < line_n; ++_l) {
        const int li = L.rank[_l];
        const int32_t *ln = L.pool + L.start[li]; const int ll = L.len[li];
        const HP_G int32_t *gln = (const HP_G int32_t *)ln;
        F.frag_off[_l] = nf;
        F.right_bound[_l] = r.seed_all + 1;
        int pre = -1, mf_pre = 0;
        for (int j1 = ll - 1; j1 >= 0; j1 -= 64) {
            wv::Lane<int> idl, mfl;
            WAVE_FOR(l) {
                const int j = j1 - l;
                int id = -1, mf = 0;
                if (j >= 0) { id = gln[j]; if (id >= 0) { int b[4]; hp_load16((const HP_G char *)(gns + id) + 16, b); mf = (b[1] >> 16) & 0xff; } }
                idl[l] = id; mfl[l] = mf;
            }
            const int cnt = j1 + 1 < 64 ? j1 + 1 : 64;
            for (int q = 0; q < cnt; ++q) {
                const int id = wv::bcast(idl, q);
                if (j1 - q == ll - 1) { pre = id; mf_pre = wv::bcast(mfl, q); F.fr_seed_off[nf] = ns; F.fr_seed[ns++] = pre; continue; }
                if (id < 0) continue;
                const int mf = mf_pre;
                pre = id; mf_pre = wv::bcast(mfl, q);
                if (mf == F_INSERT || mf == F_DELETE || mf == F_MISMATCH || mf == F_LONG_MISMATCH) { ++nf; F.fr_seed_off[nf] = ns; F.fr_seed[ns++] = pre; }
                else if (mf == F_MATCH) F.fr_seed[ns++] = pre;
                else { r.cx.status |= ST_REFEXIT; return false; }
            }
        }
        ++nf;
        F.left_bound[_l] = 0;
        F.line_score[_l] = L.ls[li];
    }
    F.frag_off[line_n] = nf; F.fr_seed_off[nf] = ns;
    F.n = line_n; F.nfrag = nf;
    return true;
}

}
#include "hp_cluster.h"
#include "hp_gaps.h"
namespace hp {

HP_NOINL int lines_pop(ReadCtx &r, NScore &ns, LSet &L, Trig &T, int32_t *_line, const Clusters *C)
{
    int l_i = 0, next_start = 0, line_score = 0, line_NM = 0;
    GapCache gc; gc.n = 0; gc.used = 0; gc.cap = 0; gc.ids = nullptr;
    if (C) gapcache_init(r, gc);
    for (;;) {
        int max_node = ns_pop(ns, &line_score, &line_NM);
        if (max_node < 0) break;
        int32_t *ln = L.pool + next_start;
        T.off[l_i] = T.used; T.cnt[l_i] = 0;
        const int node_i = line_build(r, max_node, ln, _line, &line_score, &line_NM, T, l_i, C, C ? &gc : nullptr);
        if (node_i < 0) return -1;
        { HP_G int32_t *g_ln = (HP_G int32_t *)ln; const int half = node_i / 2;
          for (int k0 = 0; k0 < half; k0 += 64) { WAVE_FOR(l) { const int k = k0 + l; if (k < half) { const int t = g_ln[k], u = g_ln[node_i - k - 1]; g_ln[k] = u; g_ln[node_i - k - 1] = t; } } }
          wv::sync(); }
        L.start[l_i] = next_start; L.len[l_i] = node_i; L.ls[l_i] = L.bs[l_i] = line_score; L.nm[l_i] = line_NM;
        L.mf[l_i] = 0; L.mh[l_i] = 0; L.lb[l_i] = L.rb[l_i] = 0;
        ++l_i; next_start += node_i + 1;
        if (r.cx.status & ST_REFEXIT) return -1;
    }
    return l_i;
}

#ifdef HP_PROF
#define HP_CSTAMP(k) do { const long long now_ = wv::clock(); if (r.prof) r.prof[(k)] += now_ - tc_; tc_ = now_; } while (0)
#else
#define HP_CSTAMP(k) do { } while (0)
#endif

HP_NOINL bool chain_first(ReadCtx &r, FLines &F, FlStore *fs = nullptr)
{
#ifdef HP_PROF
    long long tc_ = wv::clock();
#endif
    const lamsa_hp_para *P = r.cx.P;
    const int seed_out = r.seed_out, H = r.H;
    F.n = 0; F.nfrag = 0;
    int min_n = P->first_loci_thd, min_exist = 0, min_num = 0;
    {
        const HP_G int64_t *g_hoff = (const HP_G int64_t *)r.hit_off;
        for (int i0 = 0; i0 < seed_out; i0 += 64) {
            wv::Lane<int> few;
            WAVE_FOR(l) { const int i = i0 + l; few[l] = i < seed_out && (int)(g_hoff[i + 1] - g_hoff[i]) <= min_n; }
            min_num += __builtin_popcountll(wv::ballot(few));
        }
        min_exist = min_num > 0;
    }
    const bool all_min = (!min_exist || min_num * 3 < seed_out);
#ifdef HP_PROF
    long long tq_ = wv::clock(); if (r.prof) r.prof[56] += tq_ - tc_;
#endif
    if (!r.nodes_ready) {
        for (int base = 0; base < H; base += 64) {
            WAVE_FOR(l) {
                const int k = base + l;
                if (k < H) node_set(r, k, -1, 1, r.h_nm[k], F_MATCH, (all_min || mapn(r, r.n_seed[k]) <= min_n) ? MIN_FLAG : MULTI_FLAG);
            }
        }
        wv::sync();
    }
    r.nodes_ready = false;
#ifdef HP_PROF
    { const long long t2_ = wv::clock(); if (r.prof) r.prof[57] += t2_ - tq_; tq_ = t2_; }
#endif
    if (all_min) min_n = P->per_aln_m;
    struct Loc { Clusters C; NScore ns; LSet L, S; Trig T; };
    Loc *loc = (Loc *)arena_alloc(r.cx, sizeof(Loc));
    if (!loc) return false;
    const size_t cmark = arena_mark(r.cx.tmp);
    Clusters &C = loc->C;
    bool have_cl = false;
    if (seed_out > 1 && HP_CL_CAP_RT(1) > 0) {
        have_cl = clusters_build(r, C, (HP_L uint64_t *)r.cx.lds, r.cx.lds_words / 2);
        if (!have_cl && (r.cx.status & ST_OVERFLOW)) return false;
    }
    const bool do_me = min_n != P->per_aln_m && seed_out > 1;
    if (do_me && !have_cl) min_extend_all(r, min_n);
#ifdef HP_PROF
    { const long long t2_ = wv::clock(); if (r.prof) { r.prof[58] += t2_ - tq_; r.prof[59] += all_min ? 0 : 1; } }
#endif
    HP_CSTAMP(6);
#if defined(HP_CHAIN_STOP) && HP_CHAIN_STOP == 1
    return true;
#endif
    if (seed_out > 1) {
        bool any_big = false;
        if (!have_cl) dp_update_range(r, hoff(r, 1), H, 0, MIN_FLAG, false, false);
        else {
            const HP_G int32_t *g_cs = (const HP_G int32_t *)C.cs, *g_srt = (const HP_G int32_t *)r.srt;
            HP_G uint8_t *g_big = (HP_G uint8_t *)C.big;
            HP_STAT_MAX(48, C.n_cl);
            for (int c0 = 0; c0 < C.n_cl; c0 += 63) {
                wv::Lane<int> csl;
                WAVE_FOR(l) { const int c = c0 + l; csl[l] = c <= C.n_cl ? g_cs[c] : H; }
                const int cn = C.n_cl - c0 < 63 ? C.n_cl - c0 : 63;
                wv::Lane<int> csn = csl;
                WAVE_FOR(l) { const int c = c0 + l + 1; csn[l] = c <= C.n_cl ? g_cs[c] : H; }
                const bool geo32 = (long long)(r.seed_id[seed_out - 1] - r.seed_id[0] + 1) * P->seed_step <= 0x3fffffffll;
                if (geo32 && HP_CL_CAP_RT(1 << 20) >= HP_CLL_MCAP) {
                    const EdgeK K = edge_consts(P);
                    wv::sync();
                    WAVE_FOR(l) { const int n = csn[l] - csl[l]; if (l < cn && n >= 2 && n <= HP_CLL_MCAP) { HP_STAT_ADD(34, 1); HP_STAT_MAX(47, n); cluster_lane(r, K, C, r.cx.lds + l, csl[l], n, do_me); } }
                    wv::sync();
                }
                for (int q = 0; q < cn; ++q) {
                    const int lo = wv::bcast(csl, q), n = wv::bcast(csl, q + 1) - lo;
                    if (n < 2) continue;
                    if (geo32 && HP_CL_CAP_RT(1 << 20) >= HP_CLL_MCAP && n <= HP_CLL_MCAP) continue;
                    if (n <= HP_CL_CAP_RT(r.cx.lds_words / 5) && dp_cluster_lds(r, C, lo, n, do_me)) { HP_STAT_ADD(32, 1); HP_STAT_MAX(40, n); continue; }
                    HP_STAT_ADD(33, 1); HP_STAT_MAX(41, n);
                    if (do_me) min_extend_clusters(r, C, lo, lo + n);
                    for (int i0 = 0; i0 < n; i0 += 64) { WAVE_FOR(l) { if (i0 + l < n) g_big[g_srt[lo + i0 + l]] = 1; } }
                    any_big = true;
                }
            }
            wv::sync();
            if (any_big) dp_update_range(r, hoff(r, 1), H, 0, MIN_FLAG, false, false, C.big);
        }
        if (!have_cl) arena_release(r.cx.tmp, cmark);
        if (!build_sons(r, (HP_L uint64_t *)r.cx.lds, r.cx.lds_words / 2)) return false;
    }

    HP_CSTAMP(7);
#if defined(HP_CHAIN_STOP) && HP_CHAIN_STOP == 2
    return true;
#endif
    NScore &ns = loc->ns;
    if (!ns_alloc(r.cx, ns, H + 1, 0)) return false;
    ns.min_score_thd = 2;
#ifdef HP_PROF_TRACK
    const long long ti0_ = wv::clock();
#endif
    const TrImg img = have_cl && seed_out > 1 ? track_image_build(r, C.cs, C.n_cl, seed_out - 1) : TrImg{0, 0, 0, 0};
#ifdef HP_PROF_TRACK
    if (HP_PROF_CHAIN_ON && r.prof) r.prof[16] += wv::clock() - ti0_;
#endif
    if (img.on && all_min) HP_STAT_ADD(63, 1);
    track_leaves_img(r, 0, seed_out - 1, MIN_FLAG, ns, img);
#ifdef HP_PROF_TRACK
    const long long ti1_ = wv::clock();
#endif
    if (img.on) track_image_store(r, img);
#ifdef HP_PROF_TRACK
    if (HP_PROF_CHAIN_ON && r.prof) r.prof[16] += wv::clock() - ti1_;
#endif

    HP_CSTAMP(8);
#if defined(HP_CHAIN_STOP) && HP_CHAIN_STOP == 3
    return true;
#endif
    const int o_l = ns.node_n;
    LSet &L = loc->L;
    Trig &T = loc->T;
    if (!lset_alloc(r.cx, L, 2 * H + o_l + 16, o_l)) return false;
    T.cap = 2 * H + 2 * o_l + 16; T.used = 0;
    T.n1 = (int32_t *)arena_alloc(r.cx, sizeof(int32_t) * (size_t)T.cap);
    T.n2 = (int32_t *)arena_alloc(r.cx, sizeof(int32_t) * (size_t)T.cap);
    T.off = (int32_t *)arena_alloc(r.cx, sizeof(int32_t) * (size_t)(o_l + 1));
    T.cnt = (int32_t *)arena_alloc(r.cx, sizeof(int32_t) * (size_t)(o_l + 1));
    int32_t *_line = (int32_t *)arena_alloc(r.cx, sizeof(int32_t) * (size_t)(H + 2));
    if (!T.n1 || !T.n2 || !T.off || !T.cnt || !_line) return false;
    const int l_i = lines_pop(r, ns, L, T, _line, have_cl ? &C : nullptr);
    if (l_i < 0) return false;
    L.n = l_i;
    HP_CSTAMP(9);
#if defined(HP_CHAIN_STOP) && HP_CHAIN_STOP == 4
    return true;
#endif
    LSet &S = loc->S;
    const bool staged = lset_stage(r, L, l_i, S);
    HP_STAT_ADD(staged ? 35 : 36, 1);
    HP_STAT_MAX(44, l_i);
    LSet &LL = staged ? S : L;
    const int line_n = set_bound(r, LL, 0, l_i, &T);
    const bool okf = build_flines(r, LL, line_n, F, fs);
    HP_CSTAMP(10);
    if (r.prof) { r.prof[14] = o_l; r.prof[15] = H; }
    return okf;
}

struct RegB { int32_t is_rev, chr; int64_t pos; };
struct Regs {
    int n;
    int32_t *beg, *end; RegB *rb, *re;
    int m;
    int32_t *r_beg, *r_end, *r_bs, *r_bn, *r_es, *r_en;
};

HP_NOINL int multi_line(ReadCtx &r, int left_b, int right_b, const Regs &G, int reg_i, LSet &L)
{
    if (left_b + 1 >= right_b) return 0;
    const lamsa_hp_para *P = r.cx.P;
    const int start = left_b + 1, end = right_b - 1, dp_flag = WHOLE_FLAG;
    nodes_per_init(r, hoff(r, start), hoff(r, end + 1), -1, dp_flag, 1);
    if (start + 1 <= end) dp_update_range(r, hoff(r, start + 1), hoff(r, end + 1), start, dp_flag, false, true);
    const size_t mark = arena_mark(r.cx.tmp);
    NScore *nsp = (NScore *)arena_alloc(r.cx, sizeof(NScore));
    if (!nsp) return 0;
    NScore &ns = *nsp;
    if (!ns_alloc(r.cx, ns, hoff(r, end + 1) - hoff(r, start) + 1, 0)) return 0;
    ns.min_score_thd = 0;
    track_leaves(r, start, end, dp_flag, ns);
    int l_i = 0, next_start = 0, score = 0, NM = 0;
    for (;;) {
        int rr = ns_pop(ns, &score, &NM);
        if (rr < 0) break;
        int node_i = r.n_node_n[rr] - 1;
        if (l_i >= L.cap || next_start + node_i + 1 > L.pool_cap) { r.cx.status |= ST_OVERFLOW; break; }
        L.start[l_i] = next_start; L.len[l_i] = node_i + 1; L.mf[l_i] = 0; L.mh[l_i] = 0; L.lb[l_i] = L.rb[l_i] = 0;
        next_start += node_i + 1;
        int hit = 0;
        const int64_t expect = (int64_t)((r.n_seed[rr] - left_b) * P->seed_step);
        for (int i = 0; i < G.r_bn[reg_i] && !hit; ++i) {
            const RegB &b = G.re[G.r_bs[reg_i] + i];
            int64_t d = (r.h_pos[rr] - b.pos) - expect; if (d < 0) d = -d;
            if (r.h_chr[rr] == b.chr && d < P->SV_len_thd) hit = 1;
        }
        for (int i = 0; i < G.r_en[reg_i] && !hit; ++i) {
            const RegB &b = G.rb[G.r_es[reg_i] + i];
            int64_t d = (r.h_pos[rr] - b.pos) - expect; if (d < 0) d = -d;
            if (r.h_chr[rr] == b.chr && d < P->SV_len_thd) hit = 1;
        }
        if (hit) { if (score > 1) score += score / 2; else score++; }
        L.ls[l_i] = L.bs[l_i] = score; L.nm[l_i] = NM;
        int32_t *node = L.pool + L.start[l_i];
        while (rr >= 0) {
            if (node_i < 0) { r.cx.status |= ST_REFEXIT; arena_release(r.cx.tmp, mark); return 0; }
            node[node_i--] = rr;
            rr = r.n_from[rr];
        }
        if (node_i >= 0) { r.cx.status |= ST_REFEXIT; arena_release(r.cx.tmp, mark); return 0; }
        ++l_i;
    }
    arena_release(r.cx.tmp, mark);
    return l_i;
}

HP_NOINL bool chain_remain(ReadCtx &r, const Regs &G, FLines &F, FlStore *fs = nullptr)
{
    const lamsa_hp_para *P = r.cx.P;
    const int seed_out = r.seed_out, H = r.H;
    F.n = 0; F.nfrag = 0;
    LSet *lt = (LSet *)arena_alloc(r.cx, 2 * sizeof(LSet));
    if (!lt) return false;
    LSet &L = lt[0], &T = lt[1];
    if (!lset_alloc(r.cx, L, H + 16, H + 1) || !lset_alloc(r.cx, T, H + 16, H + 1)) return false;
    int l_n = 0, next_start = 0;
    for (int i = 0; i < G.m; ++i) {
        const int left_id = (G.r_beg[i] + P->seed_inv - 1) / P->seed_step + 1;
        int right_id = (G.r_end[i] - 1) / P->seed_step + 1;
        if (right_id > r.seed_all) right_id -= 1;
        int left = -2, right = -2;
        for (int j = 0; j < seed_out; ++j) if (r.seed_id[j] >= left_id) { left = j - 1; break; }
        if (left == -2) continue;
        for (int j = seed_out - 1; j >= 0; --j) if (r.seed_id[j] <= right_id) { right = j + 1; break; }
        if (right == -2) continue;
        int l = multi_line(r, left, right, G, i, T);
        if (r.cx.status & ST_REFEXIT) return false;
        T.n = l;
        l = set_bound(r, T, 0, l, nullptr);
        for (int _j = 0; _j < l; ++_j) {
            const int j = T.rank[_j], d = l_n + _j;
            if (d >= L.cap || next_start + T.len[j] > L.pool_cap) { r.cx.status |= ST_OVERFLOW; return false; }
            L.start[d] = next_start; L.len[d] = T.len[j]; L.lb[d] = T.lb[j]; L.rb[d] = T.rb[j]; L.mf[d] = T.mf[j]; L.mh[d] = T.mh[j];
            L.ls[d] = T.ls[j]; L.bs[d] = T.bs[j]; L.nm[d] = T.nm[j];
            for (int k = 0; k < T.len[j]; ++k) L.pool[next_start + k] = T.pool[T.start[j] + k];
            next_start += T.len[j];
            L.rank[d] = d;
        }
        l_n += l;
    }
    L.n = l_n;
    return build_flines(r, L, l_n, F, fs);
}

}
```

lamsa_amd/csrc/hp_cluster.h:

```cpp
#pragma once

namespace hp {

#ifndef HP_CL_CAP_RT
#define HP_CL_CAP_RT(cap) (cap)
#endif

struct Clusters {
    int n_cl;
    int32_t *cs;
    int32_t *cl_lo_r;
    int32_t *ce;
    int32_t *csrt;
    uint8_t *big;
    long long reach;
};

HP_INL long long cluster_reach(const ReadCtx &r)
{
    const lamsa_hp_para *P = r.cx.P;
    const int did = r.seed_out > 0 ? r.seed_id[r.seed_out - 1] - r.seed_id[0] : 0;
    const int mdm = P->match_dis * ((P->aln_mode & 2) ? did : 1);
    long long R = P->SV_len_thd > did * P->seed_step ? P->SV_len_thd : (long long)did * P->seed_step;
    if (mdm + 1 > R) R = mdm + 1;
    R += 128 + (long long)did * P->seed_step;
    const long long R2 = (long long)did * (P->seed_step + P->match_dis) + 256;
    return R > R2 ? R : R2;
}

HP_NOINL bool clusters_build(ReadCtx &r, Clusters &C, HP_L uint64_t *lw, int lds_n)
{
    const int H = r.H;
    C.n_cl = 0; C.reach = cluster_reach(r);
    C.cs = (int32_t *)arena_alloc(r.cx, sizeof(int32_t) * (size_t)(H + 2));
    C.cl_lo_r = (int32_t *)arena_alloc(r.cx, sizeof(int32_t) * (size_t)(H + 1));
    C.csrt = (int32_t *)arena_alloc(r.cx, sizeof(int32_t) * (size_t)(H + 1));
    C.ce = (int32_t *)arena_alloc(r.cx, sizeof(int32_t) * (size_t)(H + 1));
    C.big = (uint8_t *)arena_alloc(r.cx, (size_t)H + 64);
    if (!C.cs || !C.cl_lo_r || !C.csrt || !C.ce || !C.big) return false;
    const HP_G NodeS *ns = (const HP_G NodeS *)r.nd;
    const HP_G int32_t *g_srt = (const HP_G int32_t *)r.srt, *g_rnk = (const HP_G int32_t *)r.rnk;
    HP_G int32_t *g_cs = (HP_G int32_t *)C.cs, *g_lo = (HP_G int32_t *)C.cl_lo_r;
    HP_G uint8_t *g_big = (HP_G uint8_t *)C.big;
    const long long R = C.reach;
    int n_cl = 0, run_start = 0;
    for (int i0 = 0; i0 < H; i0 += 64) {
        wv::Lane<int> b;
        WAVE_FOR(l) {
            const int i = i0 + l;
            int v = 0;
            if (i < H) {
                g_big[i] = 0;
                if (i == 0) v = 1;
                else {
                    const NodeS A = node_load(ns + g_srt[i]), B = node_load(ns + g_srt[i - 1]);
                    v = (A.chr != B.chr) | (A.strand != B.strand) | (A.pos - B.pos > R);
                }
            }
            b[l] = v;
        }
        const unsigned long long m = wv::ballot(b);
        WAVE_FOR(l) {
            const int i = i0 + l;
            if (i < H) {
                const unsigned long long below = m & ((2ull << l) - 1);
                g_lo[i] = below ? i0 + 63 - __builtin_clzll(below) : run_start;
                if (b[l]) g_cs[n_cl + __builtin_popcountll(m & ((1ull << l) - 1))] = i;
            }
        }
        n_cl += __builtin_popcountll(m);
        if (m) run_start = i0 + 63 - __builtin_clzll(m);
    }
    wv::sync();
    g_cs[n_cl] = H;
    C.n_cl = n_cl;
    wv::sync();
    { HP_G int32_t *g_ce = (HP_G int32_t *)C.ce; for (int c0 = 0; c0 < n_cl; c0 += 64) { WAVE_FOR(l) { const int c = c0 + l; if (c < n_cl) g_ce[g_cs[c]] = g_cs[c + 1]; } } }
    const size_t mark = arena_mark(r.cx.tmp);
    uint64_t *work = (uint64_t *)arena_alloc(r.cx, sizeof(uint64_t) * (size_t)(H + 1));
    if (!work) return false;
    const bool ok = sort_packed([&](int k) { return (uint64_t)(unsigned)g_lo[g_rnk[k]]; }, bits_of((unsigned)(H > 0 ? H : 1)), H,
                                (HP_G int32_t *)C.csrt, (HP_G int32_t *)nullptr, (HP_G uint64_t *)work, lw, lds_n);
    arena_release(r.cx.tmp, mark);
    return ok;
}


HP_NOINL void min_extend_clusters(ReadCtx &r, const Clusters &C, int p_lo, int p_hi)
{
    const HP_G NodeS *ns = (const HP_G NodeS *)r.nd;
    HP_G NodeS *gd = (HP_G NodeS *)r.nd;
    const HP_G int32_t *g_csrt = (const HP_G int32_t *)C.csrt, *g_lo = (const HP_G int32_t *)C.cl_lo_r;
    const EdgeK K = edge_consts(r.cx.P);
    const int H = r.H;
    long long pairs_ = 0;
    const size_t mark_ = arena_mark(r.cx.tmp);
    uint8_t *mk = (uint8_t *)arena_alloc(r.cx, (size_t)H + 64);
    if (!mk) return;
    HP_G uint8_t *gmk = (HP_G uint8_t *)mk;
    for (int b0 = p_lo; b0 < p_hi; b0 += 64) { WAVE_FOR(l) { if (b0 + l < p_hi) gmk[g_csrt[b0 + l]] = 0; } }
    wv::sync();
    for (int mbase = p_lo; mbase < p_hi; mbase += 64) {
        wv::Lane<int> Ma0, Ma1, Ma2, Ma3, Mb0, ism, mcl;
        WAVE_FOR(l) {
            const int p = mbase + l, pp = p < H ? p : H - 1;
            const int id = g_csrt[pp];
            int a[4], b[4];
            hp_load16(ns + id, a); hp_load16((const HP_G char *)(ns + id) + 16, b);
            Ma0[l] = a[0]; Ma1[l] = a[1]; Ma2[l] = a[2]; Ma3[l] = a[3]; Mb0[l] = b[0];
            const int cl = g_lo[pp];
            const bool lone = cl == pp && (pp + 1 >= H || g_lo[pp + 1] == pp + 1);
            mcl[l] = cl;
            ism[l] = p < p_hi && !lone && (int)(int8_t)(b[1] & 0xff) == MIN_FLAG;
        }
        const unsigned long long mset = wv::ballot(ism);
        if (!mset) continue;
        const int cl_first = wv::bcast(mcl, __builtin_ctzll(mset)), cl_last = wv::bcast(mcl, 63 - __builtin_clzll(mset));
        unsigned long long carry = 0;
        int carry_seed = -1, carry_cl = -1;
        for (int base = cl_first; base < H; base += 64) {
            wv::Lane<int> sd, qcl, elig, hit, qsid, qld, idl;
            wv::Lane<long long> qdiag;
            WAVE_FOR(l) {
                const int p = base + l, pp = p < H ? p : H - 1;
                const int id = g_csrt[pp];
                int a[4], b[4];
                hp_load16(ns + id, a); hp_load16((const HP_G char *)(ns + id) + 16, b);
                sd[l] = p < H ? (a[3] >> 14) : -1; qcl[l] = p < H ? g_lo[pp] : 0x7fffffff; idl[l] = id;
                elig[l] = p < H && (int)(int8_t)(b[1] & 0xff) == MULTI_FLAG;
                hit[l] = 0;
                const int sid_ = (int)(int16_t)(b[0] & 0xffff), st_ = (int)(int8_t)((b[0] >> 16) & 0xff);
                qsid[l] = sid_; qld[l] = (int)(int8_t)((b[0] >> 24) & 0xff);
                qdiag[l] = (long long)(((unsigned long long)(unsigned)a[1] << 32) | (unsigned)a[0]) - (long long)(st_ * sid_ * K.seed_step);
            }
            if (wv::bcast(qcl, 0) > cl_last) break;
            wv::Lane<int> psd = sd, pcl = qcl, rs, seg;
            wv::shr1(psd, -2); wv::shr1(pcl, -2);
            WAVE_FOR(l) rs[l] = psd[l] != sd[l] || pcl[l] != qcl[l];
            const unsigned long long rsm = wv::ballot(rs) | 1ull;
            WAVE_FOR(l) seg[l] = 63 - __builtin_clzll(rsm & ((2ull << l) - 1));
            const int last = H - 1 - base < 63 ? H - 1 - base : 63;
            pairs_ += (long long)__builtin_popcountll(mset) * (last + 1);
            const int s_last = wv::bcast(sd, last), c_last = wv::bcast(qcl, last), st_last = wv::bcast(seg, last);
            unsigned long long next_carry = 0;
            for (unsigned long long mm = mset; mm; mm &= mm - 1) {
                const int j = __builtin_ctzll(mm);
                const int ma0 = wv::bcast(Ma0, j), ma1 = wv::bcast(Ma1, j), ma3 = wv::bcast(Ma3, j), mb0 = wv::bcast(Mb0, j), mc = wv::bcast(mcl, j);
                const int msid = (int)(int16_t)(mb0 & 0xffff), mst = (int)(int8_t)((mb0 >> 16) & 0xff), mld = (int)(int8_t)((mb0 >> 24) & 0xff);
                const int xm = ma3 >> 14;
                const long long mdiag = (long long)(((unsigned long long)(unsigned)ma1 << 32) | (unsigned)ma0) - (long long)(mst * msid * K.seed_step);
                wv::Lane<int> q;
                WAVE_FOR(l) {
                    int v = 0;
                    if (elig[l] && qcl[l] == mc && sd[l] != xm) {
                        const bool q_first = sd[l] < xm;
                        const int did = iabs(qsid[l] - msid);
                        const long long D = q_first ? mdiag - qdiag[l] : qdiag[l] - mdiag;
                        const int ld = mst > 0 ? (q_first ? qld[l] : mld) : (q_first ? mld : qld[l]);
                        const long long dis = (long long)mst * D - (long long)ld;
                        const int mat_dis = K.match_dis * (K.high_err ? did : 1);
                        v = did * K.seed_step >= K.seed_len && dis <= mat_dis && dis >= -mat_dis;
                    }
                    q[l] = v;
                }
                const unsigned long long qb = wv::ballot(q);
                const bool cj = (carry >> j) & 1, run_on = carry_seed == s_last && carry_cl == c_last;
                if (!qb) { if (run_on && cj) next_carry |= 1ull << j; continue; }
                WAVE_FOR(l) {
                    if (q[l]) {
                        const unsigned long long earlier = qb & ((1ull << l) - 1) & ~((1ull << seg[l]) - 1);
                        if (earlier == 0 && !(sd[l] == carry_seed && qcl[l] == carry_cl && cj)) hit[l] = 1;
                    }
                }
                if ((qb >> st_last) != 0 || (run_on && cj)) next_carry |= 1ull << j;
            }
            WAVE_FOR(l) { if (hit[l]) gmk[idl[l]] = 1; }
            carry = next_carry; carry_seed = s_last; carry_cl = c_last;
        }
    }
    wv::sync();
    r.n_pairs += pairs_;
    for (int b0 = p_lo; b0 < p_hi; b0 += 64) { WAVE_FOR(l) { if (b0 + l < p_hi) { const int k = g_csrt[b0 + l]; if (gmk[k]) gd[k].dp_flag = MIN_FLAG; } } }
    wv::sync();
    arena_release(r.cx.tmp, mark_);
}


#define HP_CLL_MCAP (HP_LANE_STRIP_WORDS / 384 < 6 ? HP_LANE_STRIP_WORDS / 384 : 6)
HP_INL int gap_edge(const EdgeK &K, int sp, int qpos, int qsid, int qld, int tpos, int tsid, int tld)
{
    const int dsid = tsid - qsid, span = dsid * K.seed_step;
    if (span < K.seed_len) return F_UNCONNECT;
    const int dis = sp * (tpos - qpos) - span - (sp > 0 ? qld : tld);
    const int mat_dis = K.match_dis * (K.high_err ? dsid : 1);
    if (dis <= mat_dis && dis >= -mat_dis) return dsid == 1 ? F_MATCH : (dsid <= K.mis3 ? F_MISMATCH : F_LONG_MISMATCH);
    if (dis > mat_dis && dis < K.sv_len) return F_DELETE;
    if ((dis < -mat_dis && dis >= 0 - (span - K.seed_len)) || (dis < -K.half_split && dis >= -K.sv_len)) return F_INSERT;
    return F_UNCONNECT;
}

HP_INL void cluster_lane(ReadCtx &r, const EdgeK &K, const Clusters &C, HP_L int32_t *strip, int lo, int n, bool do_me)
{
    const HP_G NodeS *ns = (const HP_G NodeS *)r.nd;
    HP_G NodeS *gd = (HP_G NodeS *)r.nd;
    const HP_G int32_t *g_csrt = (const HP_G int32_t *)C.csrt;
    HP_G int32_t *g_from = (HP_G int32_t *)r.n_from, *g_node_n = (HP_G int32_t *)r.n_node_n;
#define CW(e, w) strip[((e) * 6 + (w)) * 64]
    int m = 0, sp = 0; int64_t pos0 = 0;
    unsigned is_min = 0, promoted = 0;
    for (int i0 = 0; i0 < n; i0 += 3) {
      int ids[3]; NodeS Qs[3];
#pragma unroll
      for (int u = 0; u < 3; ++u) ids[u] = g_csrt[lo + (i0 + u < n ? i0 + u : n - 1)];
#pragma unroll
      for (int u = 0; u < 3; ++u) Qs[u] = node_load(ns + ids[u]);
#pragma unroll
      for (int u = 0; u < 3; ++u) {
        if (i0 + u >= n) continue;
        const int id = ids[u];
        const NodeS Q = Qs[u];
        if (Q.dp_flag != MIN_FLAG && !(do_me && Q.dp_flag == MULTI_FLAG)) continue;
        if (m == 0) { pos0 = Q.pos; sp = Q.strand; }
        if (Q.dp_flag == MIN_FLAG) is_min |= 1u << m;
        CW(m, 0) = (int)(Q.pos - pos0); CW(m, 1) = Q.slot_j; CW(m, 2) = ((int)Q.sid & 0xffff) | (((int)Q.len_dif8 & 0xff) << 16);
        CW(m, 3) = (int)(((unsigned)Q.score << 16) | (unsigned)(Q.NM & 0xffff));
        CW(m, 4) = id; CW(m, 5) = (0xff << 24) | (1 << 16) | ((int)Q.son_flag << 8) | Q.match_flag;
        ++m;
      }
    }
    if (do_me && is_min != 0 && is_min != (1u << m) - 1) {
        for (int a = 0; a < m; ++a) {
            if (!((is_min >> a) & 1)) continue;
            const int apos = CW(a, 0), a2 = CW(a, 2), ax = CW(a, 1) >> 14;
            const int asid = (int)(short)(a2 & 0xffff), ald = (int)(int8_t)((a2 >> 16) & 0xff);
            int run_seed = -1; bool run_done = false;
            for (int q = 0; q < m; ++q) {
                if ((is_min >> q) & 1) continue;
                const int qx = CW(q, 1) >> 14;
                if (qx != run_seed) { run_seed = qx; run_done = false; }
                if (run_done || qx == ax) continue;
                const int q2 = CW(q, 2), qpos = CW(q, 0);
                const int qsid = (int)(short)(q2 & 0xffff), qld = (int)(int8_t)((q2 >> 16) & 0xff);
                const int flag = qx < ax ? gap_edge(K, sp, qpos, qsid, qld, apos, asid, ald) : gap_edge(K, sp, apos, asid, ald, qpos, qsid, qld);
                if (flag <= F_LONG_MISMATCH) { promoted |= 1u << q; run_done = true; }
            }
        }
    }
    const unsigned in_pass = is_min | promoted;
    bool any = false;
    for (int a = 1; a < m; ++a) {
        if (!((in_pass >> a) & 1)) continue;
        const int tpos = CW(a, 0), tsj = CW(a, 1), t2 = CW(a, 2), t3 = CW(a, 3);
        const int tslot = tsj >> 14, tsid = (int)(short)(t2 & 0xffff), tld = (int)(int8_t)((t2 >> 16) & 0xff);
        const int t_score = t3 >> 16, t_NM = t3 & 0xffff;
        int best_hi = -0x7fffffff, best_lo = -1, best_b = -1, best_f = 0, neg_p = -0x7fffffff, neg_b = -1, neg_f = 0, neg_hi = 0;
        for (int b = 0; b < a; ++b) {
            if (!((in_pass >> b) & 1)) continue;
            const int qsj = CW(b, 1), qslot = qsj >> 14;
            if (qslot >= tslot) continue;
            const int q5 = CW(b, 5);
            if (sp == 1 && ((q5 >> 8) & 0xff) <= F_MATCH_THD) continue;
            const int q2 = CW(b, 2), q3 = CW(b, 3);
            const int flag = gap_edge(K, sp, CW(b, 0), (int)(short)(q2 & 0xffff), (int)(int8_t)((q2 >> 16) & 0xff), tpos, tsid, tld);
            if (flag == F_UNCONNECT) continue;
            const int pos = ((tslot - 1 - qslot) << 14) | (qsj & 16383);
            const int cand = (q3 >> 16) + 1 + score_table(flag), nm = (q3 & 0xffff) + t_NM;
            const int hi = (int)(((unsigned)cand << 16) | (unsigned)(65535 - nm)), lo_ = (1 << 28) - 1 - pos;
            if (hi > best_hi || (hi == best_hi && lo_ > best_lo)) { best_hi = hi; best_lo = lo_; best_b = b; best_f = flag; }
            if (sp == -1 && flag <= F_MATCH_THD && 0 - pos > neg_p) { neg_p = 0 - pos; neg_b = b; neg_f = flag; neg_hi = hi; }
        }
        int w_b = -1, w_f = 0, w_score = t_score, w_nm = t_NM;
        if (neg_b >= 0) { w_b = neg_b; w_f = neg_f; w_score = neg_hi >> 16; w_nm = 65535 - (neg_hi & 0xffff); }
        else if (best_b >= 0) {
            const int cand = best_hi >> 16, nm = 65535 - (best_hi & 0xffff);
            if (cand > w_score || (cand == w_score && nm < w_nm)) { w_b = best_b; w_f = best_f; w_score = cand; w_nm = nm; }
        }
        if (w_b >= 0) {
            const int q5 = CW(w_b, 5);
            CW(a, 3) = (int)(((unsigned)w_score << 16) | (unsigned)(w_nm & 0xffff));
            CW(a, 5) = (w_b << 24) | ((((q5 >> 16) & 0xff) + 1) << 16) | (CW(a, 5) & 0xff00) | w_f;
            CW(w_b, 5) = (q5 & ~0xff00) | (w_f << 8);
            any = true;
        }
    }
    if (any || promoted) {
        for (int a = 0; a < m; ++a) {
            if (!((in_pass >> a) & 1) || !(any || ((promoted >> a) & 1))) continue;
            const int id = CW(a, 4), w2 = CW(a, 2), w3 = CW(a, 3), w5 = CW(a, 5);
            const int b0 = (w2 & 0xffff) | ((sp & 0xff) << 16) | (((w2 >> 16) & 0xff) << 24);
            hp_store16((HP_G char *)(gd + id) + 16, b0, MIN_FLAG | (((w5 >> 8) & 0xff) << 8) | ((w5 & 0xff) << 16), w3 >> 16, w3 & 0xffff);
            const int f = (w5 >> 24) & 0xff;
            g_from[id] = f == 0xff ? -1 : CW(f, 4);
            g_node_n[id] = (w5 >> 16) & 0xff;
        }
    }
#undef CW
}

struct ClLds { HP_L int32_t *w0, *w1, *w2, *w3, *w4; };
HP_INL ClLds cl_lds(HP_L int32_t *lds, int cap) { ClLds c; c.w0 = lds; c.w1 = lds + cap; c.w2 = lds + 2 * cap; c.w3 = lds + 3 * cap; c.w4 = lds + 4 * cap; return c; }

HP_INL NodeS cl_unpack(int w0, int w1, int w2, int w3, int chr, int strand)
{
    NodeS q;
    q.pos = (int64_t)(unsigned)w0; q.chr = chr; q.slot_j = (int)((unsigned)w1 >> 4);
    q.sid = (int16_t)((unsigned)w2 >> 17); q.strand = (int8_t)strand; q.len_dif8 = (int8_t)((w2 >> 9) & 0xff);
    q.dp_flag = (int8_t)((int)((unsigned)w1 << 28) >> 28); q.son_flag = (uint8_t)((w2 >> 4) & 31); q.match_flag = (uint8_t)(w2 & 15); q.pad_ = 0;
    q.score = w3 >> 16; q.NM = w3 & 0xffff;
    return q;
}

HP_NOINL bool dp_cluster_lds(ReadCtx &r, const Clusters &C, int lo, int n, bool do_me)
{
    const HP_G NodeS *ns = (const HP_G NodeS *)r.nd;
    HP_G NodeS *gd = (HP_G NodeS *)r.nd;
    const HP_G int32_t *g_srt = (const HP_G int32_t *)r.srt, *g_rnk = (const HP_G int32_t *)r.rnk, *g_csrt = (const HP_G int32_t *)C.csrt;
    const HP_G int16_t *g_hnm = (const HP_G int16_t *)r.h_nm;
    HP_G int32_t *g_from = (HP_G int32_t *)r.n_from, *g_node_n = (HP_G int32_t *)r.n_node_n;
    const ClLds L = cl_lds(r.cx.lds, r.cx.lds_words / 5);
    const EdgeK K = edge_consts(r.cx.P);
    const int dp_flag = MIN_FLAG;
    if ((long long)(r.seed_id[r.seed_out - 1] - r.seed_id[0] + 1) * K.seed_step > 0x3fffffffll) return false;
    const NodeS first = node_load(ns + g_srt[lo]);
    const int64_t pos0 = first.pos; const int strand = first.strand;
    int nm_sum = 0; int bad = 0;
    wv::Lane<int> bmin;
    WAVE_FOR(l) bmin[l] = 0x7fffffff;
    wv::sync();
    for (int i0 = 0; i0 < n; i0 += 64) {
        wv::Lane<int> nml, badl, nsl;
        WAVE_FOR(l) {
            const int i = i0 + l;
            int nmv = 0, bv = 0, sv = -0x7fffffff;
            if (i < n) {
                const int id = g_srt[lo + i];
                const NodeS q = node_load(ns + id);
                const int64_t rel = q.pos - pos0;
                bv = rel < 0 || rel > 0x7ffffff0ll || q.score < -30000 || q.score > 30000 || q.NM < 0 || q.NM > 65535 || q.sid < 0;
                nmv = g_hnm[id]; sv = 0 - (q.slot_j >> 14);
                L.w0[i] = (int)(unsigned)rel;
                L.w1[i] = (int)(((unsigned)q.slot_j << 4) | ((unsigned)q.dp_flag & 15u));
                L.w2[i] = (int)(((unsigned)(unsigned short)q.sid << 17) | (((unsigned)q.len_dif8 & 255u) << 9) | (((unsigned)q.son_flag & 31u) << 4) | ((unsigned)q.match_flag & 15u));
                L.w3[i] = (int)(((unsigned)q.score << 16) | ((unsigned)q.NM & 0xffffu));
                L.w4[i] = 1;
            }
            nml[l] = nmv; badl[l] = bv; nsl[l] = sv;
        }
        nm_sum += wv::reduce_sum(nml);
        if (wv::ballot(badl) != 0) bad = 1;
        const int mn = 0 - wv::reduce_max(nsl);
        WAVE_FOR(l) { if (l == (i0 >> 6)) bmin[l] = mn; }
    }
    if (bad || nm_sum > 65535 || n > 64 * 64) return false;
    wv::sync();
    const int sp = strand, POSMAX = (1 << 28) - 1, NEG = -0x7fffffff;
    long long pairs_ = 0;
    if (do_me) {
        const size_t mark = arena_mark(r.cx.tmp);
        int32_t *ml = (int32_t *)arena_alloc(r.cx, sizeof(int32_t) * 2 * (size_t)(n + 64));
        if (!ml) return false;
        HP_G int32_t *g_ml = (HP_G int32_t *)ml, *g_mk = (HP_G int32_t *)(ml + n + 64);
        int nml = 0, n_min = 0;
        for (int o0 = 0; o0 < n; o0 += 64) {
            wv::Lane<int> ism, isu, tll;
            WAVE_FOR(l) {
                const int o = o0 + l; const int tl = o < n ? g_rnk[g_csrt[lo + o]] - lo : 0;
                const int dpf = (int)((unsigned)L.w1[tl] << 28) >> 28;
                tll[l] = tl; isu[l] = o < n && dpf == MULTI_FLAG; ism[l] = o < n && dpf == MIN_FLAG;
            }
            const unsigned long long mu = wv::ballot(isu);
            WAVE_FOR(l) { if (isu[l]) { const int at = nml + __builtin_popcountll(mu & ((1ull << l) - 1)); g_ml[at] = tll[l]; g_mk[at] = 0; } }
            nml += __builtin_popcountll(mu); n_min += __builtin_popcountll(wv::ballot(ism));
        }
        wv::sync();
        if (nml > 0 && n_min > 0) {
            for (int o0 = 0; o0 < n; o0 += 64) {
                wv::Lane<int> ism, T0, T1, T2;
                WAVE_FOR(l) {
                    const int o = o0 + l; const int tl = o < n ? g_rnk[g_csrt[lo + o]] - lo : 0;
                    T0[l] = L.w0[tl]; T1[l] = L.w1[tl]; T2[l] = L.w2[tl];
                    ism[l] = o < n && ((int)((unsigned)T1[l] << 28) >> 28) == MIN_FLAG;
                }
                const unsigned long long mset = wv::ballot(ism);
                if (!mset) continue;
                unsigned long long carry = 0;
                int carry_seed = -1;
                for (int b0 = 0; b0 < nml; b0 += 64) {
                    wv::Lane<int> sd, q0, qsid, qld, hit;
                    WAVE_FOR(l) {
                        const int at = b0 + l;
                        int s_ = -1, p_ = 0, i_ = 0, d_ = 0;
                        if (at < nml) { const int tl = g_ml[at]; const int w1 = L.w1[tl], w2 = L.w2[tl]; s_ = (int)((unsigned)w1 >> 18); p_ = L.w0[tl]; i_ = (int)((unsigned)w2 >> 17); d_ = (int)(int8_t)((w2 >> 9) & 0xff); }
                        sd[l] = s_; q0[l] = p_; qsid[l] = i_; qld[l] = d_; hit[l] = 0;
                    }
                    wv::Lane<int> psd = sd, rs, seg;
                    wv::shr1(psd, -2);
                    WAVE_FOR(l) rs[l] = psd[l] != sd[l];
                    const unsigned long long rsm = wv::ballot(rs) | 1ull;
                    WAVE_FOR(l) seg[l] = 63 - __builtin_clzll(rsm & ((2ull << l) - 1));
                    const int last = nml - 1 - b0 < 63 ? nml - 1 - b0 : 63;
                    pairs_ += (long long)__builtin_popcountll(mset) * (last + 1);
                    const int s_last = wv::bcast(sd, last), st_last = wv::bcast(seg, last);
                    unsigned long long next_carry = 0;
                    for (unsigned long long mm = mset; mm; mm &= mm - 1) {
                        const int j = __builtin_ctzll(mm);
                        const int m0 = wv::bcast(T0, j), m1 = wv::bcast(T1, j), m2 = wv::bcast(T2, j);
                        const int xm = (int)((unsigned)m1 >> 18), msid = (int)((unsigned)m2 >> 17), mld = (int)(int8_t)((m2 >> 9) & 0xff);
                        wv::Lane<int> q;
                        WAVE_FOR(l) {
                            int v = 0;
                            if (sd[l] >= 0 && sd[l] != xm) {
                                const bool q_first = sd[l] < xm;
                                const int dsid = q_first ? msid - qsid[l] : qsid[l] - msid, span = dsid * K.seed_step;
                                const int dis = (q_first ? sp * (m0 - q0[l]) : sp * (q0[l] - m0)) - span - (sp > 0 ? (q_first ? qld[l] : mld) : (q_first ? mld : qld[l]));
                                const int mat_dis = K.match_dis * (K.high_err ? dsid : 1);
                                v = span >= K.seed_len && dis <= mat_dis && dis >= -mat_dis;
                            }
                            q[l] = v;
                        }
                        const unsigned long long qb = wv::ballot(q);
                        const bool cj = (carry >> j) & 1, run_on = carry_seed == s_last;
                        if (!qb) { if (run_on && cj) next_carry |= 1ull << j; continue; }
                        WAVE_FOR(l) {
                            if (q[l]) {
                                const unsigned long long earlier = qb & ((1ull << l) - 1) & ~((1ull << seg[l]) - 1);
                                if (earlier == 0 && !(sd[l] == carry_seed && cj)) hit[l] = 1;
                            }
                        }
                        if ((qb >> st_last) != 0 || (run_on && cj)) next_carry |= 1ull << j;
                    }
                    WAVE_FOR(l) { if (hit[l]) g_mk[b0 + l] = 1; }
                    carry = next_carry; carry_seed = s_last;
                }
            }
            wv::sync();
            for (int b0 = 0; b0 < nml; b0 += 64) {
                WAVE_FOR(l) { const int at = b0 + l; if (at < nml && g_mk[at]) { const int tl = g_ml[at]; L.w1[tl] = (L.w1[tl] & ~15) | MIN_FLAG; } }
            }
            wv::sync();
        }
        arena_release(r.cx.tmp, mark);
    }
    for (int o0 = 0; o0 < n; o0 += 64) {
        wv::Lane<int> tloc, T0, T1, T2, T3;
        WAVE_FOR(l) {
            const int o = o0 + l; const int tl = o < n ? g_rnk[g_csrt[lo + o]] - lo : 0;
            tloc[l] = tl; T0[l] = L.w0[tl]; T1[l] = L.w1[tl]; T2[l] = L.w2[tl]; T3[l] = L.w3[tl];
        }
        const int cnt = n - o0 < 64 ? n - o0 : 64;
        for (int q = 0; q < cnt; ++q) {
            const int t1 = wv::bcast(T1, q);
            if ((int)((unsigned)t1 << 28) >> 28 != dp_flag) continue;
            const int x = (int)((unsigned)t1 >> 18);
            if (x == 0) continue;
            const int ct = wv::bcast(tloc, q), t0 = wv::bcast(T0, q), t2 = wv::bcast(T2, q), t3 = wv::bcast(T3, q);
            const int tsid = (int)((unsigned)t2 >> 17), tld = (int)(int8_t)((t2 >> 9) & 0xff), t_score = t3 >> 16, t_NM = t3 & 0xffff;
            wv::Lane<int> bhi, blo, bi, bf, negp, n_i, n_f, n_hi, okl;
            WAVE_FOR(l) { bhi[l] = NEG; blo[l] = -1; bi[l] = 0; bf[l] = 0; negp[l] = NEG; n_i[l] = 0; n_f[l] = 0; n_hi[l] = 0; okl[l] = 0; }
            for (int i0 = 0; i0 < n; i0 += 64) {
                if (wv::bcast(bmin, i0 >> 6) >= x) continue;
                pairs_ += n - i0 < 64 ? n - i0 : 64;
                WAVE_FOR(l) {
                    const int i = i0 + l, ii = i < n ? i : 0;
                    const int q0 = L.w0[ii], q1 = L.w1[ii], q2 = L.w2[ii], q3 = L.w3[ii];
                    const int qslot = (int)((unsigned)q1 >> 18), qdpf = (int)((unsigned)q1 << 28) >> 28;
                    const int dsid = tsid - (int)((unsigned)q2 >> 17);
                    const int span = dsid * K.seed_step;
                    const int qld = (int)(int8_t)((q2 >> 9) & 0xff);
                    const int dis = sp * (t0 - q0) - span - (sp > 0 ? qld : tld);
                    const int mat_dis = K.match_dis * (K.high_err ? dsid : 1);
                    int flag = F_UNCONNECT;
                    if (span >= K.seed_len) {
                        if (dis <= mat_dis && dis >= -mat_dis) flag = dsid == 1 ? F_MATCH : (dsid <= K.mis3 ? F_MISMATCH : F_LONG_MISMATCH);
                        else if (dis > mat_dis && dis < K.sv_len) flag = F_DELETE;
                        else if ((dis < -mat_dis && dis >= 0 - (span - K.seed_len)) || (dis < -K.half_split && dis >= -K.sv_len)) flag = F_INSERT;
                    }
                    const int ok = (i < n) & (qslot < x) & (qdpf == dp_flag) & !((sp == 1) & (((q2 >> 4) & 31) <= F_MATCH_THD)) & (flag != F_UNCONNECT);
                    const int pos = ((x - 1 - qslot) << 14) | ((q1 >> 4) & 16383);
                    const int cand = (q3 >> 16) + 1 + score_table(flag);
                    const int hi = ok ? (int)(((unsigned)cand << 16) | (unsigned)(65535 - ((q3 & 0xffff) + t_NM))) : NEG;
                    const int lo_ = POSMAX - pos;
                    const bool better = hi > bhi[l] || (hi == bhi[l] && ok && lo_ > blo[l]);
                    bhi[l] = better ? hi : bhi[l]; blo[l] = better ? lo_ : blo[l]; bi[l] = better ? i : bi[l]; bf[l] = better ? flag : bf[l];
                    const int np = (ok & (sp == -1) & (flag <= F_MATCH_THD)) ? -pos : NEG;
                    const bool nb = np > negp[l];
                    negp[l] = nb ? np : negp[l]; n_i[l] = nb ? i : n_i[l]; n_f[l] = nb ? flag : n_f[l]; n_hi[l] = nb ? hi : n_hi[l];
                    okl[l] |= ok;
                }
            }
            if (wv::ballot(okl) == 0) continue;
            int max_from = -1, max_score = t_score, max_NM = t_NM, max_flag = 0;
            bool changed = false;
            const int npos = wv::reduce_max(negp);
            if (npos != NEG) {
                wv::Lane<int> w;
                WAVE_FOR(l) w[l] = negp[l] == npos;
                const int wl = __builtin_ctzll(wv::ballot(w));
                const int hi = wv::bcast(n_hi, wl);
                max_from = wv::bcast(n_i, wl); max_flag = wv::bcast(n_f, wl); max_score = hi >> 16; max_NM = 65535 - (hi & 0xffff);
                changed = true;
            } else {
                const int mh = wv::reduce_max(bhi);
                if (mh != NEG) {
                    const int cand = mh >> 16, nm = 65535 - (mh & 0xffff);
                    if (cand > max_score || (cand == max_score && nm < max_NM)) {
                        wv::Lane<int> l2;
                        WAVE_FOR(l) l2[l] = bhi[l] == mh ? blo[l] : -1;
                        const int ml = wv::reduce_max(l2);
                        wv::Lane<int> w;
                        WAVE_FOR(l) w[l] = bhi[l] == mh && blo[l] == ml;
                        const int wl = __builtin_ctzll(wv::ballot(w));
                        max_from = wv::bcast(bi, wl); max_flag = wv::bcast(bf, wl); max_score = cand; max_NM = nm;
                        changed = true;
                    }
                }
            }
            if (changed) {
                const int f2 = wv::uni(L.w2[max_from]), f4 = wv::uni(L.w4[max_from]);
                L.w2[max_from] = (f2 & ~(31 << 4)) | ((max_flag & 31) << 4);
                L.w2[ct] = (t2 & ~15) | (max_flag & 15);
                L.w3[ct] = (int)(((unsigned)max_score << 16) | ((unsigned)max_NM & 0xffffu));
                L.w4[ct] = ((max_from + 1) << 16) | (((f4 & 0xffff) + 1) & 0xffff);
                wv::sync();
            }
        }
    }
    r.n_pairs += pairs_;
    wv::sync();
    for (int i0 = 0; i0 < n; i0 += 64) {
        WAVE_FOR(l) {
            const int i = i0 + l;
            if (i < n) {
                const int id = g_srt[lo + i];
                const int w1 = L.w1[i], w2 = L.w2[i], w3 = L.w3[i], w4 = L.w4[i];
                const int b0 = (int)(((unsigned)w2 >> 17) & 0xffffu) | ((strand & 0xff) << 16) | (((w2 >> 9) & 0xff) << 24);
                const int dpf = (int)((unsigned)w1 << 28) >> 28;
                hp_store16((HP_G char *)(gd + id) + 16, b0, (dpf & 0xff) | (((w2 >> 4) & 31) << 8) | ((w2 & 15) << 16), w3 >> 16, w3 & 0xffff);
                const int fl = (int)((unsigned)w4 >> 16);
                g_from[id] = fl ? g_srt[lo + fl - 1] : -1;
                g_node_n[id] = w4 & 0xffff;
            }
        }
    }
    wv::sync();
    return true;
}

HP_NOINL bool build_sons(ReadCtx &r, HP_L uint64_t *lw, int lds_n)
{
    const int H = r.H;
    if (H == 0) return true;
    const size_t mark = arena_mark(r.cx.tmp);
    int32_t *ps = (int32_t *)arena_alloc(r.cx, sizeof(int32_t) * (size_t)(H + 1));
    uint64_t *work = (uint64_t *)arena_alloc(r.cx, sizeof(uint64_t) * (size_t)(H + 1));
    if (!ps || !work) { arena_release(r.cx.tmp, mark); return false; }
    const HP_G int32_t *g_from = (const HP_G int32_t *)r.n_from;
    HP_G int32_t *g_ps = (HP_G int32_t *)ps;
    HP_G int32_t *g_in_de = (HP_G int32_t *)r.n_in_de, *g_son_n = (HP_G int32_t *)r.n_son_n;
    HP_G int32_t *g_first = (HP_G int32_t *)r.n_first, *g_last = (HP_G int32_t *)r.n_last, *g_next = (HP_G int32_t *)r.n_next;
    const bool ok = sort_packed([&](int k) { const int f = g_from[k]; return (uint64_t)(unsigned)(f >= 0 ? f : H); }, bits_of((unsigned)H) , H,
                                g_ps, (HP_G int32_t *)nullptr, (HP_G uint64_t *)work, lw, lds_n);
    if (!ok) { arena_release(r.cx.tmp, mark); return false; }
    int run_start = 0;
    for (int i0 = 0; i0 < H; i0 += 64) {
        wv::Lane<int> st, tl, fl, fnl;
        WAVE_FOR(l) {
            const int i = i0 + l;
            int t = -1, f = -1, fp = -2, fn = -2;
            if (i < H) {
                t = g_ps[i]; f = g_from[t];
                fp = i > 0 ? g_from[g_ps[i - 1]] : -2;
                fn = i + 1 < H ? g_from[g_ps[i + 1]] : -2;
            }
            tl[l] = t; fl[l] = f; fnl[l] = fn;
            st[l] = i < H && f >= 0 && fp != f;
        }
        const unsigned long long m = wv::ballot(st);
        WAVE_FOR(l) {
            const int i = i0 + l, t = tl[l], f = fl[l];
            if (i < H && f >= 0) {
                const unsigned long long below = m & ((2ull << l) - 1);
                const int rs = below ? i0 + 63 - __builtin_clzll(below) : run_start;
                if (st[l]) g_first[f] = t;
                if (fnl[l] == f) g_next[t] = g_ps[i + 1];
                else { g_next[t] = -1; g_last[f] = t; g_son_n[f] = i - rs + 1; g_in_de[f] = i - rs + 1; }
            }
        }
        if (m) run_start = i0 + 63 - __builtin_clzll(m);
    }
    wv::sync();
    arena_release(r.cx.tmp, mark);
    return true;
}

}
```

lamsa_amd/csrc/hp_core.h:

```cpp
#pragma once
#include <hp/wave.h>
#include "../../include/lamsa_hp.h"

namespace hp {

typedef int32_t cig_t;
enum { C_M = 0, C_I = 1, C_D = 2, C_N = 3, C_S = 4, C_H = 5, C_EQ = 7, C_X = 8 };
enum { ST_OVERFLOW = LAMSA_HP_ST_OVERFLOW, ST_REFEXIT = LAMSA_HP_ST_REFEXIT, ST_UNSUPPORTED = LAMSA_HP_ST_UNSUPPORTED,
       ST_DEAD = ST_OVERFLOW | ST_REFEXIT | ST_UNSUPPORTED };

#define HP_NEG_INF (-0x40000000)

struct Arena {
    char *base; size_t cap, top;
};
HP_INL void arena_init(Arena &a, void *base, size_t cap) { a.base = (char *)base; a.cap = cap; a.top = 0; }
HP_INL size_t arena_mark(const Arena &a) { return a.top; }
HP_INL void arena_release(Arena &a, size_t m) { a.top = m; }

#ifndef HP_LDS_CELLS
#define HP_LDS_CELLS 512
#endif
#ifndef HP_LDS_Z_BYTES
#define HP_LDS_Z_BYTES 512
#endif
#define HP_LDS_WORDS (2 * HP_LDS_CELLS + HP_LDS_CELLS / 4 + HP_LDS_Z_BYTES / 4)
#ifndef HP_CHAIN_LDS_WORDS
#define HP_CHAIN_LDS_WORDS 2432
#endif
#define HP_BOTH_LDS_WORDS (HP_CHAIN_LDS_WORDS > HP_LDS_WORDS ? HP_CHAIN_LDS_WORDS : HP_LDS_WORDS)
#define HP_LANE_STRIP_WORDS HP_CHAIN_LDS_WORDS

struct Ctx {
    const lamsa_hp_para *P;
    HP_L int32_t *lds;
    int lds_words;
    Arena tmp;
    int status;
    long long n_cells;
    long long *prof;
    long long *prof_dp = nullptr;
    int lds_epoch;
};
#ifdef HP_PROF_FILL
#define HP_PROF_CHAIN_ON 0
#define HP_TADD_FILL(cx, slot, v) HP_TADD(cx, slot, v)
#else
#define HP_PROF_CHAIN_ON 1
#define HP_TADD_FILL(cx, slot, v) do { } while (0)
#endif
#ifdef HP_PROF
#define HP_T0(v) const long long v = wv::clock()
#define HP_TADD(cx, slot, v) do { if ((cx).prof) { (cx).prof[slot] += wv::clock() - (v); (cx).prof[(slot) + 1] += 1; } } while (0)
#else
#define HP_T0(v) do { } while (0)
#define HP_TADD(cx, slot, v) do { } while (0)
#endif

#ifndef HP_DPLOG
#define HP_DPLOG(kind, qlen, tlen, w, cells) do { } while (0)
#endif
#ifndef HP_STAT
#define HP_STAT(i) do { } while (0)
#endif
#ifndef HP_STAT_ADD
#define HP_STAT_ADD(i, n) ((void)0)
#endif
#ifndef HP_STAT_MAX
#define HP_STAT_MAX(i, v) ((void)0)
#endif

HP_INL void *arena_alloc(Ctx &cx, size_t bytes) {
    size_t b = (bytes + 15) & ~(size_t)15;
    if (cx.tmp.top + b > cx.tmp.cap) { cx.status |= ST_OVERFLOW; return nullptr; }
    void *p = cx.tmp.base + cx.tmp.top;
    cx.tmp.top += b;
    return p;
}

struct CigV { cig_t *c; int n, cap; };
HP_INL void cig_bind(CigV &v, cig_t *mem, int cap) { v.c = mem; v.n = 0; v.cap = mem ? cap : 0; }
HP_INL bool cig_alloc(Ctx &cx, CigV &v, int cap) {
    cig_t *m = (cig_t *)arena_alloc(cx, (size_t)cap * sizeof(cig_t));
    cig_bind(v, m, cap);
    return m != nullptr;
}
HP_INL void cig_raw_push(Ctx &cx, CigV &v, cig_t w) {
    if (v.n >= v.cap) { cx.status |= ST_OVERFLOW; return; }
    v.c[v.n++] = w;
}
HP_INL void cig_push0(Ctx &cx, CigV &v, cig_t w) {
    if (v.n > 0 && (v.c[v.n - 1] & 0xf) == (w & 0xf)) { v.c[v.n - 1] += (w >> 4) << 4; return; }
    cig_raw_push(cx, v, w);
}
HP_INL void cig_push1(Ctx &cx, CigV &v, cig_t w) { if ((w >> 4) == 0) return; cig_push0(cx, v, w); }
HP_FN void cig_pushv(Ctx &cx, CigV &v, const cig_t *c, int n) {
    if (n == 0) return;
    const HP_G cig_t *src = (const HP_G cig_t *)c;
    HP_G cig_t *dst = (HP_G cig_t *)v.c;
    const int vn = v.n;
    int j = 0;
    if (vn > 0) {
        const cig_t last = dst[vn - 1], c0 = src[0];
        if ((last & 0xf) == (c0 & 0xf)) { dst[vn - 1] = last + ((c0 >> 4) << 4); j = 1; }
        else if (((last & 0xf) == C_I && (c0 & 0xf) == C_S) || ((last & 0xf) == C_S && (c0 & 0xf) == C_I)) {
            dst[vn - 1] = (((last >> 4) + (c0 >> 4)) << 4) | C_S; j = 1;
        }
    }
    const int m = n - j;
    if (vn + m > v.cap) { cx.status |= ST_OVERFLOW; return; }
    for (int b0 = 0; b0 < m; b0 += 64) { WAVE_FOR(l) { const int i = b0 + l; if (i < m) dst[vn + i] = src[j + i]; } }
    v.n = vn + m;
    wv::sync();
}
HP_FN void cig_pushw(Ctx &cx, CigV &v, cig_t w) {
    if (v.n > 0) {
        const cig_t last = v.c[v.n - 1];
        if ((last & 0xf) == (w & 0xf)) { v.c[v.n - 1] = last + ((w >> 4) << 4); return; }
        if (((last & 0xf) == C_I && (w & 0xf) == C_S) || ((last & 0xf) == C_S && (w & 0xf) == C_I)) { v.c[v.n - 1] = (((last >> 4) + (w >> 4)) << 4) | C_S; return; }
    }
    if (v.n + 1 > v.cap) { cx.status |= ST_OVERFLOW; return; }
    v.c[v.n++] = w;
}
HP_FN void cig_invert(cig_t *c, int n) {
    HP_G cig_t *g = (HP_G cig_t *)c;
    for (int b0 = 0; b0 < n / 2; b0 += 64) {
        WAVE_FOR(l) { const int a = b0 + l; if (a < n / 2) { const cig_t x = g[a], y = g[n - 1 - a]; g[a] = y; g[n - 1 - a] = x; } }
    }
    wv::sync();
}
HP_FN int cig_readlen(const cig_t *c, int n) {
    const HP_G cig_t *g = (const HP_G cig_t *)c;
    int tot = 0;
    for (int b0 = 0; b0 < n; b0 += 64) {
        wv::Lane<int> x;
        WAVE_FOR(l) { const int i = b0 + l; int v = 0; if (i < n) { const cig_t w = g[i]; const int op = w & 0xf; if (op == C_M || op == C_I || op == C_S) v = w >> 4; } x[l] = v; }
        tot += wv::reduce_sum(x);
    }
    return tot;
}
HP_FN int cig_reflen(const cig_t *c, int n) {
    const HP_G cig_t *g = (const HP_G cig_t *)c;
    int tot = 0;
    for (int b0 = 0; b0 < n; b0 += 64) {
        wv::Lane<int> x;
        WAVE_FOR(l) { const int i = b0 + l; int v = 0; if (i < n) { const cig_t w = g[i]; const int op = w & 0xf; if (op == C_M || op == C_D || op == C_H) v = w >> 4; } x[l] = v; }
        tot += wv::reduce_sum(x);
    }
    return tot;
}

struct Seq { const uint8_t *p; int stride; };
HP_INL int seq_at(const Seq &s, int i) { return s.p[(long)i * s.stride]; }
HP_INL Seq seq_fwd(const uint8_t *p) { Seq s; s.p = p; s.stride = 1; return s; }
HP_INL Seq seq_rev(const uint8_t *p, int len) { Seq s; s.p = p + (len > 0 ? len - 1 : 0); s.stride = -1; return s; }

HP_INL int sub_score(const lamsa_hp_para *P, int t, int q) { return (t > 3 || q > 3) ? -1 : (t == q ? P->match : -P->mis); }

HP_INL int iabs(int x) { return x < 0 ? -x : x; }
HP_INL int imin(int a, int b) { return a < b ? a : b; }
HP_INL int imax(int a, int b) { return a > b ? a : b; }

}
```

lamsa_amd/csrc/hp_gaps.h:

```cpp
#pragma once

namespace hp {

#define HP_GAP_MCAP (HP_LANE_STRIP_WORDS / 384 < 6 ? HP_LANE_STRIP_WORDS / 384 : 6)
static_assert(HP_GAP_MCAP >= 2, "the chaining kernels need at least 768 words of LDS per wave");
#ifndef HP_GAP_RANGE
#define HP_GAP_RANGE 96
#endif
#ifndef HP_GAP_MIN
#define HP_GAP_MIN 6
#endif
#ifndef HP_WALK_MIN
#define HP_WALK_MIN 16
#endif

struct GapOut {
    int n;
    int ids[HP_GAP_MCAP], mfs[HP_GAP_MCAP];
    int d_score, d_NM;
    int r_from, r_score, r_NM, r_nn, r_mf;
};

HP_INL void gap_dp_core(const EdgeK &K, HP_L int32_t *strip, int m, int sp, int left, int left_x, int right_x, int tail, int left_NM,
                        bool r_ok, int rrel, int r_sid, int r_ld, int r_mf, int right_nm, GapOut &O)
// ... 135 lines not shown
    bool r_ok = false; int rrel = 0, r_sid = 0, r_ld = 0, r_mf = 0, right_nm = 0;
    if (tail) {
        const NodeS Rt = node_load(ns + right);
        const long long rr = Rt.pos - Fh.pos;
        right_nm = g_hnm[right]; r_sid = Rt.sid; r_ld = Rt.len_dif8; r_mf = Rt.match_flag; rrel = (int)rr;
        r_ok = Rt.chr == Fh.chr && Rt.strand == sp && rr <= 0x3fffffffll && rr >= -0x3fffffffll;
    }
#undef GW
    gap_dp_core(K, strip, m, sp, left, left_x, right_x, tail, head_nm, r_ok, rrel, r_sid, r_ld, r_mf, right_nm, O);
}

struct GapRest { int pool_n, d_score, d_NM; };
HP_NOINL MiniR mini_line_far(ReadCtx &r, int left, int right, int right_x, int32_t *line, int _head, int _tail)
{
    return mini_line(r, left, right, right_x, line, _head, _tail);
}
HP_NOINL GapRest gaps_one_by_one(ReadCtx &r, int G, int32_t *gp, int GA, int32_t *pool, int pool_n, int32_t *_line)
{
    Ctx &cx = r.cx;
    const int H = r.H;
    const int32_t *g_left = gp, *g_right = gp + GA, *g_rx = gp + 3 * GA, *g_tail = gp + 4 * GA, *o_lane = gp + 15 * GA;
    int32_t *o_n = gp + 6 * GA, *o_off = gp + 7 * GA;
    GapRest R; R.pool_n = pool_n; R.d_score = 0; R.d_NM = 0;
    for (int g0 = 0; g0 < G; g0 += 64) {
        wv::Lane<int> todo, lf, rt, rx, tl;
        WAVE_FOR(l) {
            const int g = g0 + l;
            todo[l] = g < G && !o_lane[g];
            lf[l] = g < G ? g_left[g] : -1; rt[l] = g < G ? g_right[g] : -1; rx[l] = g < G ? g_rx[g] : 0; tl[l] = g < G ? g_tail[g] : 0;
        }
        unsigned long long m = wv::ballot(todo);
        while (m) {
            const int q = __builtin_ctzll(m), g = g0 + q;
            m &= m - 1;
            const int left = wv::bcast(lf, q), right = wv::bcast(rt, q), right_x = wv::bcast(rx, q), tail = wv::bcast(tl, q);
            const int k_n = hoff(r, right_x) - hoff(r, nx(r, left) + 1);
            MiniR mr; mr.n = -1; mr.d_score = 0; mr.d_NM = 0;
            if (k_n <= 64) mr = mini_line_sets<1>(r, left, right, right_x, _line, 1, tail, k_n, nullptr);
            if (mr.n < 0) mr = mini_line_far(r, left, right, right_x, _line, 1, tail);
            const int n = mr.n, ds = mr.d_score, dn = mr.d_NM;
            if (cx.status & ST_REFEXIT) { R.pool_n = -1; return R; }
            if (R.pool_n + n > H + 8) { cx.status |= ST_OVERFLOW; R.pool_n = -1; return R; }
            o_n[g] = n; o_off[g] = R.pool_n;
            wv::sync();
            for (int k0 = 0; k0 < n; k0 += 64) { WAVE_FOR(l) { if (k0 + l < n) pool[R.pool_n + k0 + l] = _line[k0 + l]; } }
            R.pool_n += n; R.d_score += ds; R.d_NM += dn;
            wv::sync();
        }
    }
    return R;
}

#ifndef HP_GAPTAB_CAP_RT
#define HP_GAPTAB_CAP_RT(cap) (cap)
#endif
#ifndef HP_GAP_MCAP_RT
#define HP_GAP_MCAP_RT(cap) (cap)
#endif
#ifndef HP_GAPCACHE_MIN
#define HP_GAPCACHE_MIN 96
#endif
struct GapCache { int n, used, cap; int lo[4], off[4], cnt[4]; int32_t *ids; };
HP_INL void gapcache_init(ReadCtx &r, GapCache &gc) { gc.n = 0; gc.used = 0; gc.cap = r.H; gc.ids = (int32_t *)arena_alloc(r.cx, sizeof(int32_t) * (size_t)(r.H + 64)); if (!gc.ids) gc.cap = 0; }

HP_HOT GapRest gaps_by_cluster(ReadCtx &r, const Clusters &C, int max_node, int G, int32_t *gp, int GA, int32_t *pool, int32_t *pool_mf, int32_t *_line, GapCache *gc = nullptr, int cl_lo = -1, int cl_n = 0)
{
    Ctx &cx = r.cx;
    const int H = r.H, seed_out = r.seed_out;
    const EdgeK K = edge_consts(cx.P);
    GapRest R; R.pool_n = -2; R.d_score = 0; R.d_NM = 0;
    if (seed_out > HP_GAPTAB_CAP_RT(2 * cx.lds_words) || G > 32767 || HP_GAP_MCAP * 6 * 64 > cx.lds_words) return R;
    if ((long long)(r.seed_id[seed_out - 1] - r.seed_id[0] + 1) * K.seed_step > 0x3fffffffll) return R;
    const HP_G NodeS *ns = (const HP_G NodeS *)r.nd;
    HP_G NodeS *gd = (HP_G NodeS *)r.nd;
    const HP_G int16_t *g_hnm = (const HP_G int16_t *)r.h_nm;
    const HP_G int32_t *g_csrt = (const HP_G int32_t *)C.csrt;
    HP_G int32_t *g_from = (HP_G int32_t *)r.n_from, *g_node_n = (HP_G int32_t *)r.n_node_n;
    const int lo = cl_lo >= 0 ? cl_lo : C.cl_lo_r[r.rnk[max_node]], n_c = cl_lo >= 0 ? cl_n : C.ce[lo] - lo;
    if ((long long)(n_c - 1) * C.reach > 0x3fffffffll) return R;
    const int sp = r.h_strand[max_node];
    const HP_G int32_t *g_left = (const HP_G int32_t *)gp, *g_right = (const HP_G int32_t *)(gp + GA), *g_lx = (const HP_G int32_t *)(gp + 2 * GA),
                       *g_rx = (const HP_G int32_t *)(gp + 3 * GA), *g_tail = (const HP_G int32_t *)(gp + 4 * GA);
    HP_G int32_t *o_n = (HP_G int32_t *)(gp + 6 * GA), *o_off = (HP_G int32_t *)(gp + 7 * GA), *o_s0 = (HP_G int32_t *)(gp + 8 * GA), *o_m = (HP_G int32_t *)(gp + 9 * GA),
                 *o_lane = (HP_G int32_t *)(gp + 15 * GA);
    const size_t mark = arena_mark(cx.tmp);
    int32_t *sv = (int32_t *)arena_alloc(cx, sizeof(int32_t) * 8 * (size_t)(n_c + 1));
    int32_t *s_id = (int32_t *)arena_alloc(cx, sizeof(int32_t) * (size_t)(n_c + 64));
    int32_t *rs = (int32_t *)arena_alloc(cx, sizeof(int32_t) * (size_t)(n_c + 2));
    if (!sv || !s_id || !rs) { arena_release(cx.tmp, mark); R.pool_n = -1; return R; }
    HP_G int32_t *g_sv = (HP_G int32_t *)sv, *g_sid = (HP_G int32_t *)s_id, *g_rs = (HP_G int32_t *)rs;
    HP_L int16_t *tab = (HP_L int16_t *)cx.lds;
    wv::sync();
    { const int nw = (seed_out + 1) / 2; for (int w0 = 0; w0 < nw; w0 += 64) { WAVE_FOR(l) { if (w0 + l < nw) cx.lds[w0 + l] = -1; } } }
    wv::sync();
    for (int g0 = 0; g0 < G; g0 += 64) {
        WAVE_FOR(l) {
            const int g = g0 + l;
            if (g < G) { o_n[g] = 0; o_off[g] = 0; o_lane[g] = 1; const int x1 = g_rx[g]; for (int x = g_lx[g] + 1; x < x1; ++x) tab[x] = (int16_t)g; }
        }
    }
    wv::sync();
    const HP_G int32_t *g_src = g_csrt + lo; int n_src = n_c;
    if (gc && n_c >= HP_GAPCACHE_MIN && gc->cap > 0) {
        int e = -1, e_off = 0, e_cnt = 0;
#pragma unroll
        for (int q = 0; q < 4; ++q) if (q < gc->n && gc->lo[q] == lo) { e = q; e_off = gc->off[q]; e_cnt = gc->cnt[q]; }
        if (e < 0 && gc->n < 4 && gc->used + n_c <= gc->cap) {
            e = gc->n++; e_off = gc->used;
            HP_G int32_t *g_dst = (HP_G int32_t *)(gc->ids + gc->used);
            int cnt = 0;
            for (int i0 = 0; i0 < n_c; i0 += 64) {
                wv::Lane<int> isml, idl;
                WAVE_FOR(l) {
                    const int i = i0 + l;
                    int v = 0, id = 0;
                    if (i < n_c) { id = g_csrt[lo + i]; int b[4]; hp_load16((const HP_G char *)(ns + id) + 16, b); const int df = (int)(int8_t)(b[1] & 0xff); v = df == MULTI_FLAG || df == 0 - MULTI_FLAG; }
                    isml[l] = v; idl[l] = id;
                }
                const unsigned long long m = wv::ballot(isml);
                WAVE_FOR(l) { if (isml[l]) g_dst[cnt + __builtin_popcountll(m & ((1ull << l) - 1))] = idl[l]; }
                cnt += __builtin_popcountll(m);
            }
            e_cnt = cnt;
#pragma unroll
            for (int q = 0; q < 4; ++q) if (q == e) { gc->lo[q] = lo; gc->off[q] = e_off; gc->cnt[q] = cnt; }
            gc->used += cnt;
            wv::sync();
        }
        if (e >= 0) { g_src = (const HP_G int32_t *)(gc->ids + e_off); n_src = e_cnt; }
    }
    int n_surv = 0, n_eval = 0;
    for (int i0 = 0; i0 < n_src; i0 += 64) {
        wv::Lane<int> keep, u0, u1, u2, u3, u4, u5, ug, evl;
        WAVE_FOR(l) {
            const int i = i0 + l;
            int ev = 0;
            int kp = 0, w0 = 0, w1 = 0, w2 = 0, w3 = 0, w4 = 0, w5 = 0, wg = 0;
            if (i < n_src) {
                const int id = g_src[i];
                int a[4], b[4];
                hp_load16(ns + id, a); hp_load16((const HP_G char *)(ns + id) + 16, b);
                const int df = (int)(int8_t)(b[1] & 0xff);
                if (df == MULTI_FLAG || df == 0 - MULTI_FLAG) {
                    const int g = tab[a[3] >> 14];
                    if (g >= 0) {
                        const int left = g_left[g];
                        const NodeS F = node_load(ns + (left >= 0 ? left : g_right[g]));
                        const long long qpos = (long long)(((unsigned long long)(unsigned)a[1] << 32) | (unsigned)a[0]);
                        const int rel = (int)(qpos - F.pos);
                        const int qsid = (int)(int16_t)(b[0] & 0xffff), qld = (int)(int8_t)((b[0] >> 24) & 0xff), nm = g_hnm[id];
                        w0 = rel; w1 = a[3]; w2 = (qsid & 0xffff) | ((qld & 0xff) << 16); w4 = id; wg = g;
                        if (left >= 0) {
                            const int flag = gap_edge(K, sp, 0, F.sid, F.len_dif8, rel, qsid, qld);
                            ev = 1;
                            if (flag != F_UNCONNECT) {
                                kp = 1;
                                w3 = (int)(((unsigned)(2 + score_table(flag)) << 16) | (unsigned)((nm + g_hnm[left]) & 0xffff));
                                w5 = (0xff << 24) | (1 << 16) | (F_INIT << 8) | flag;
                            }
                        } else {
                            kp = 1; w3 = (int)((1u << 16) | (unsigned)(nm & 0xffff)); w5 = (0xff << 24) | (1 << 16) | (F_INIT << 8) | F_MATCH;
                        }
                    }
                }
            }
            keep[l] = kp; u0[l] = w0; u1[l] = w1; u2[l] = w2; u3[l] = w3; u4[l] = w4; u5[l] = w5; ug[l] = wg; evl[l] = ev;
        }
        n_eval += __builtin_popcountll(wv::ballot(evl));
        const unsigned long long m = wv::ballot(keep);
        if (!m) continue;
        WAVE_FOR(l) {
            if (keep[l]) {
                const int at = n_surv + __builtin_popcountll(m & ((1ull << l) - 1));
                hp_store16(g_sv + 8 * (size_t)at, u0[l], u1[l], u2[l], u3[l]); hp_store16(g_sv + 8 * (size_t)at + 4, u4[l], u5[l], ug[l], 0);
                g_sid[at] = u4[l];
            }
        }
        n_surv += __builtin_popcountll(m);
    }
    r.n_pairs += n_eval;
    wv::sync();
    int n_runs = 0;
    for (int j0 = 0; j0 < n_surv; j0 += 64) {
        wv::Lane<int> st;
        WAVE_FOR(l) { const int j = j0 + l; st[l] = j < n_surv && (j == 0 || g_sv[8 * (size_t)j + 6] != g_sv[8 * (size_t)(j - 1) + 6]); }
        const unsigned long long m = wv::ballot(st);
        WAVE_FOR(l) { if (st[l]) g_rs[n_runs + __builtin_popcountll(m & ((1ull << l) - 1))] = j0 + l; }
        n_runs += __builtin_popcountll(m);
    }
    WAVE_FOR(l) { if (l == 0) g_rs[n_runs] = n_surv; }
    wv::sync();
    int pool_n = 0, d_score = 0, d_NM = 0;
    bool any_wide = false;
    if (G > 0 && g_tail[0] == 0 && !(n_surv > 0 && g_sv[8 * (size_t)(n_surv - 1) + 6] == 0)) d_NM -= g_hnm[g_left[0]];
#define GW(e, w) strip[((e) * 6 + (w)) * 64]
    for (int q0 = 0; q0 < n_runs; q0 += 64) {
        wv::Lane<int> nn, ds, dn, gl;
        WAVE_FOR(l) {
            const int q = q0 + l;
            GapOut O; O.n = 0; O.d_score = 0; O.d_NM = 0; O.r_from = -1; O.r_score = 0; O.r_NM = 0; O.r_nn = 1; O.r_mf = 0;
            int g = -1;
            if (q < n_runs) {
                const int s0 = g_rs[q], m = g_rs[q + 1] - s0;
                g = g_sv[8 * (size_t)s0 + 6];
                if (m > HP_GAP_MCAP_RT(HP_GAP_MCAP)) { O.n = -1; o_lane[g] = 0; o_s0[g] = s0; o_m[g] = m; }
                else {
                    HP_L int32_t *strip = cx.lds + l;
                    HP_STAT(2); HP_STAT_MAX(43, m);
                    for (int e = 0; e < m; ++e) {
                        int u[4], v[4];
                        hp_load16(g_sv + 8 * (size_t)(s0 + e), u); hp_load16(g_sv + 8 * (size_t)(s0 + e) + 4, v);
                        GW(e, 0) = u[0]; GW(e, 1) = u[1]; GW(e, 2) = u[2]; GW(e, 3) = u[3]; GW(e, 4) = v[0]; GW(e, 5) = v[1];
                    }
                    const int left = g_left[g], right = g_right[g], tail = g_tail[g];
                    long long base = 0; int left_NM = 0, rrel = 0, r_sid = 0, r_ld = 0, r_mf = 0, right_nm = 0;
                    if (left >= 0) { const NodeS Fh = node_load(ns + left); base = Fh.pos; left_NM = g_hnm[left]; }
                    if (tail) {
                        const NodeS Rt = node_load(ns + right);
                        if (left < 0) base = Rt.pos;
                        rrel = (int)(Rt.pos - base); r_sid = Rt.sid; r_ld = Rt.len_dif8; r_mf = Rt.match_flag; right_nm = g_hnm[right];
                    }
                    O.r_from = left;
                    if (left < 0) HP_STAT(3);
                    gap_dp_core(K, strip, m, sp, left, g_lx[g], g_rx[g], tail, left_NM, tail != 0, rrel, r_sid, r_ld, r_mf, right_nm, O);
                    if (O.n >= 0 && tail) {
                        g_from[right] = O.r_from; gd[right].score = O.r_score; gd[right].NM = O.r_NM; g_node_n[right] = O.r_nn; gd[right].match_flag = (uint8_t)O.r_mf;
                    }
                }
            }
            nn[l] = O.n; ds[l] = O.n >= 0 ? O.d_score : 0; dn[l] = O.n >= 0 ? O.d_NM : 0; gl[l] = g;
            for (int k = 0; k < HP_GAP_MCAP; ++k) { if (k < O.n) { cx.lds[(k * 6 + 0) * 64 + l] = O.ids[k]; cx.lds[(k * 6 + 1) * 64 + l] = O.mfs[k]; } }
        }
        wv::Lane<int> bad, wide, cntl;
        WAVE_FOR(l) { bad[l] = nn[l] == -2; wide[l] = nn[l] == -1; cntl[l] = nn[l] > 0 ? nn[l] : 0; }
        if (wv::ballot(bad) != 0) { cx.status |= ST_REFEXIT; arena_release(cx.tmp, mark); R.pool_n = -1; return R; }
        if (wv::ballot(wide) != 0) any_wide = true;
        wv::Lane<int> pre = cntl;
        wv::scan_add_excl(pre);
        const int tot = wv::reduce_sum(cntl);
        if (pool_n + tot > H + 8) { cx.status |= ST_OVERFLOW; arena_release(cx.tmp, mark); R.pool_n = -1; return R; }
        WAVE_FOR(l) {
            if (nn[l] > 0) {
                const int g = gl[l], off = pool_n + pre[l];
                o_n[g] = nn[l]; o_off[g] = off;
                for (int k = 0; k < nn[l]; ++k) {
                    const int id = cx.lds[(k * 6 + 0) * 64 + l], mf = cx.lds[(k * 6 + 1) * 64 + l];
                    pool[off + k] = id; pool_mf[off + k] = mf; gd[id].match_flag = (uint8_t)mf;
                }
            }
        }
        pool_n += tot;
        d_score += wv::reduce_sum(ds); d_NM += wv::reduce_sum(dn);
        wv::sync();
    }
#undef GW
    if (any_wide) {
        for (int g0 = 0; g0 < G; g0 += 64) {
            wv::Lane<int> todo, lf, rt, rx, tl, s0l, ml;
            WAVE_FOR(l) {
                const int g = g0 + l;
                todo[l] = g < G && !o_lane[g];
                lf[l] = g < G ? g_left[g] : -1; rt[l] = g < G ? g_right[g] : -1; rx[l] = g < G ? g_rx[g] : 0; tl[l] = g < G ? g_tail[g] : 0;
                s0l[l] = todo[l] ? o_s0[g] : 0; ml[l] = todo[l] ? o_m[g] : 0;
            }
            unsigned long long m = wv::ballot(todo);
            while (m) {
                const int q = __builtin_ctzll(m), g = g0 + q;
                m &= m - 1;
                const int left = wv::bcast(lf, q), right = wv::bcast(rt, q), right_x = wv::bcast(rx, q), tail = wv::bcast(tl, q), s0 = wv::bcast(s0l, q), cnt = wv::bcast(ml, q);
                MiniR mr; mr.n = -1; mr.d_score = 0; mr.d_NM = 0;
                if (cnt <= 64) mr = mini_line_sets<1>(r, left, right, right_x, _line, 1, tail, cnt, s_id + s0);
                else if (cnt <= 64 * HP_MS_MAX_SETS) mr = mini_line_sets<HP_MS_MAX_SETS>(r, left, right, right_x, _line, 1, tail, cnt, s_id + s0);
                HP_STAT(4); HP_STAT_MAX(42, cnt);
                if (mr.n < 0) { HP_STAT(5); mr = mini_line_mem(r, left, right, right_x, _line, 1, tail); }
                const int n = mr.n, dsc = mr.d_score, dnm = mr.d_NM;
                if (cx.status & ST_REFEXIT) { arena_release(cx.tmp, mark); R.pool_n = -1; return R; }
                if (pool_n + n > H + 8) { cx.status |= ST_OVERFLOW; arena_release(cx.tmp, mark); R.pool_n = -1; return R; }
                o_n[g] = n; o_off[g] = pool_n;
                wv::sync();
                for (int k0 = 0; k0 < n; k0 += 64) { WAVE_FOR(l) { if (k0 + l < n) pool[pool_n + k0 + l] = _line[k0 + l]; } }
                pool_n += n; d_score += dsc; d_NM += dnm;
                wv::sync();
            }
        }
    }
    arena_release(cx.tmp, mark);
    R.pool_n = pool_n; R.d_score = d_score; R.d_NM = d_NM;
    return R;
}

HP_HOT int line_build(ReadCtx &r, int max_node, int32_t *ln, int32_t *_line, int *line_score, int *line_NM, Trig &T, int l_i, const Clusters *C = nullptr, GapCache *gc = nullptr)
{
    Ctx &cx = r.cx;
    const int H = r.H, seed_out = r.seed_out;
    const EdgeK K = edge_consts(cx.P);
    const size_t mark = arena_mark(cx.tmp);
    HP_G NodeS *gd = (HP_G NodeS *)r.nd;
    HP_G int32_t *g_from = (HP_G int32_t *)r.n_from, *g_node_n = (HP_G int32_t *)r.n_node_n;
    const HP_G int32_t *g_seed = (const HP_G int32_t *)r.n_seed;
    int32_t *anc = (int32_t *)arena_alloc(cx, sizeof(int32_t) * 2 * (size_t)(H + 2));
    if (!anc) { arena_release(cx.tmp, mark); return -1; }
    int32_t *anc_x = anc + (H + 2);
    int A = 0;
#if defined(HP_PROF) && !defined(HP_PROF_TRACK)
    long long tl_ = wv::clock();
#define HP_LSTAMP(k) do { const long long now_ = wv::clock(); if (r.prof) r.prof[(k)] += now_ - tl_; tl_ = now_; } while (0)
#else
#define HP_LSTAMP(k) do { } while (0)
#endif
    HP_G int32_t *g_anc = (HP_G int32_t *)anc, *g_ancx = (HP_G int32_t *)anc_x;
    bool walked = false;
    int cl_lo = -1, cl_n = 0;
    if (C) {
        const HP_G int32_t *g_srt = (const HP_G int32_t *)r.srt, *g_rnk = (const HP_G int32_t *)r.rnk;
        const int rk = r.rnk[max_node], lo = C->cl_lo_r[rk], n_c = C->ce[lo] - lo;
        cl_lo = lo; cl_n = n_c;
        if (n_c <= 6) HP_STAT(6); else if (n_c <= 16) HP_STAT(7); else HP_STAT(8);
        if (n_c >= HP_WALK_MIN && n_c <= cx.lds_words && r.n_node_n[max_node] >= HP_WALK_MIN) {
            wv::sync();
            for (int i0 = 0; i0 < n_c; i0 += 64) {
                WAVE_FOR(l) {
                    const int i = i0 + l;
                    if (i < n_c) { const int f = g_from[g_srt[lo + i]]; const int p = f >= 0 ? g_rnk[f] - lo : -1; cx.lds[i] = (unsigned)p < (unsigned)n_c ? p : -1; }
                }
            }
            wv::sync();
            int cur = rk - lo;
            while (cur >= 0 && A <= H) {
                wv::Lane<int> pl;
                WAVE_FOR(l) pl[l] = 0;
                int cnt = 0;
                while (cur >= 0 && cnt < 64 && A + cnt <= H) { WAVE_FOR(l) { if (l == cnt) pl[l] = cur; } ++cnt; cur = wv::uni(cx.lds[cur]); }
                WAVE_FOR(l) { if (l < cnt) g_anc[A + l] = g_srt[lo + pl[l]]; }
                A += cnt;
            }
            wv::sync();
            walked = true;
        }
    }
    if (!walked) for (int right = max_node; right >= 0 && A <= H; right = g_from[right]) anc[A++] = right;
    for (int i0 = 0; i0 < A; i0 += 64) { WAVE_FOR(l) { if (i0 + l < A) g_ancx[i0 + l] = g_seed[g_anc[i0 + l]]; } }
    wv::sync();
    HP_LSTAMP(16);
#if defined(HP_PROF) && !defined(HP_PROF_TRACK)
    if (HP_PROF_CHAIN_ON && r.prof) { r.prof[21] += 1; r.prof[12] += A; }
#endif
    {
        int any_gap = anc_x[0] < seed_out - 1;
        for (int i0 = 0; i0 < A && !any_gap; i0 += 64) {
            wv::Lane<int> ex;
            WAVE_FOR(l) { const int i = i0 + l; ex[l] = i < A && (i + 1 < A ? g_ancx[i + 1] : -1) < g_ancx[i] - 1; }
            any_gap = wv::ballot(ex) != 0;
        }
        if (!any_gap) {
            HP_G int32_t *g_ln0 = (HP_G int32_t *)ln;
            for (int i0 = 0; i0 < A; i0 += 64) { WAVE_FOR(l) { if (i0 + l < A) g_ln0[i0 + l] = g_anc[i0 + l]; } }
            wv::sync();
            arena_release(cx.tmp, mark);
            HP_LSTAMP(17);
#if defined(HP_PROF) && !defined(HP_PROF_TRACK)
            if (HP_PROF_CHAIN_ON && r.prof) r.prof[22] += 1;
#endif
            return A;
        }
    }
    const int GA = A + 2;
    int32_t *gp = (int32_t *)arena_alloc(cx, sizeof(int32_t) * 16 * (size_t)GA);
    int32_t *pool = (int32_t *)arena_alloc(cx, sizeof(int32_t) * 2 * (size_t)(H + 8));
    int32_t *posx = (int32_t *)arena_alloc(cx, sizeof(int32_t) * 2 * (size_t)(H + A + 8));
    if (!gp || !pool || !posx) { arena_release(cx.tmp, mark); return -1; }
    int32_t *g_left = gp, *g_right = gp + GA, *g_lx = gp + 2 * GA, *g_rx = gp + 3 * GA, *g_tail = gp + 4 * GA, *g_after = gp + 5 * GA,
            *o_n = gp + 6 * GA, *o_off = gp + 7 * GA, *o_ds = gp + 8 * GA, *o_dn = gp + 9 * GA, *o_rf = gp + 10 * GA, *o_rs = gp + 11 * GA, *o_rn = gp + 12 * GA,
            *o_rnn = gp + 13 * GA, *o_rmf = gp + 14 * GA, *o_lane = gp + 15 * GA;
    int32_t *pool_mf = pool + (H + 8);
    int G = 0;
    if (anc_x[0] < seed_out - 1) { g_left[0] = max_node; g_right[0] = -1; g_lx[0] = anc_x[0]; g_rx[0] = seed_out; g_tail[0] = 0; g_after[0] = -1; G = 1; }
    for (int i0 = 0; i0 < A; i0 += 64) {
        wv::Lane<int> ex, lf, lx;
        WAVE_FOR(l) {
            const int i = i0 + l;
            int e = 0, left = -1, left_x = -1;
            if (i < A) { if (i + 1 < A) { left = g_anc[i + 1]; left_x = g_ancx[i + 1]; } e = left_x < g_ancx[i] - 1; }
            ex[l] = e; lf[l] = left; lx[l] = left_x;
        }
        const unsigned long long m = wv::ballot(ex);
        WAVE_FOR(l) {
            if (ex[l]) {
                const int g = G + __builtin_popcountll(m & ((1ull << l) - 1)), i = i0 + l;
                g_left[g] = lf[l]; g_right[g] = g_anc[i]; g_lx[g] = lx[l]; g_rx[g] = g_ancx[i]; g_tail[g] = 1; g_after[g] = i;
            }
        }
        G += __builtin_popcountll(m);
    }
    wv::sync();
    HP_LSTAMP(17);
#if defined(HP_PROF) && !defined(HP_PROF_TRACK)
    if (HP_PROF_CHAIN_ON && r.prof) { r.prof[23] += G; if (G < HP_GAP_MIN) r.prof[54] += G; r.prof[55] += 1; }
#endif
    int pool_n = 0, d_score = 0, d_NM = 0;
    bool by_cluster = false;
    if (C) {
        const GapRest gr = gaps_by_cluster(r, *C, max_node, G, gp, GA, pool, pool_mf, _line, gc, cl_lo, cl_n);
        if (gr.pool_n == -1) { arena_release(cx.tmp, mark); return -1; }
        if (gr.pool_n >= 0) { by_cluster = true; pool_n = gr.pool_n; d_score = gr.d_score; d_NM = gr.d_NM; HP_STAT(0); HP_STAT_MAX(46, G); }
        HP_LSTAMP(18);
    }
    if (!by_cluster) {
        HP_STAT(1); HP_STAT_MAX(45, G);
        const bool use_lanes = HP_CL_CAP_RT(1) > 0 && G >= HP_GAP_MIN;
        for (int g0 = 0; g0 < G; g0 += 64) {
            wv::Lane<int> nn, ds, dn;
            WAVE_FOR(l) {
                const int g = g0 + l;
                GapOut O; O.n = -1; O.d_score = 0; O.d_NM = 0; O.r_from = -1; O.r_score = 0; O.r_NM = 0; O.r_nn = 1; O.r_mf = 0;
                if (g < G && g_left[g] >= 0 && use_lanes) { HP_STAT_ADD(39, 1); gap_lane(r, K, cx.lds + l, g_left[g], g_right[g], g_lx[g], g_rx[g], g_tail[g], O); }
                nn[l] = g < G ? O.n : 0; ds[l] = O.n >= 0 ? O.d_score : 0; dn[l] = O.n >= 0 ? O.d_NM : 0;
                if (g < G) {
                    o_n[g] = O.n; o_ds[g] = O.d_score; o_dn[g] = O.d_NM; o_rf[g] = O.r_from; o_rs[g] = O.r_score; o_rn[g] = O.r_NM; o_rnn[g] = O.r_nn; o_rmf[g] = O.r_mf; o_lane[g] = O.n >= 0;
                }
                for (int k = 0; k < HP_GAP_MCAP; ++k) { if (g < G && k < O.n) { cx.lds[(k * 6 + 0) * 64 + l] = O.ids[k]; cx.lds[(k * 6 + 1) * 64 + l] = O.mfs[k]; } }
            }
            wv::Lane<int> bad, cntl;
            WAVE_FOR(l) { bad[l] = nn[l] == -2; cntl[l] = nn[l] > 0 ? nn[l] : 0; }
            if (wv::ballot(bad) != 0) { cx.status |= ST_REFEXIT; arena_release(cx.tmp, mark); return -1; }
            wv::Lane<int> pre = cntl;
            wv::scan_add_excl(pre);
            WAVE_FOR(l) {
                const int g = g0 + l;
                if (g < G && nn[l] >= 0) {
                    o_off[g] = pool_n + pre[l];
                    for (int k = 0; k < nn[l]; ++k) { pool[pool_n + pre[l] + k] = cx.lds[((k) * 6 + 0) * 64 + l]; pool_mf[pool_n + pre[l] + k] = cx.lds[((k) * 6 + 1) * 64 + l]; }
                }
            }
            pool_n += wv::reduce_sum(cntl);
            d_score += wv::reduce_sum(ds); d_NM += wv::reduce_sum(dn);
            wv::sync();
        }
        for (int g0 = 0; g0 < G; g0 += 64) {
            WAVE_FOR(l) {
                const int g = g0 + l;
                if (g < G && o_lane[g]) {
                    if (g_tail[g]) {
                        const int right = g_right[g];
                        g_from[right] = o_rf[g]; gd[right].score = o_rs[g]; gd[right].NM = o_rn[g]; g_node_n[right] = o_rnn[g]; gd[right].match_flag = (uint8_t)o_rmf[g];
                    }
                    for (int k = 0; k < o_n[g]; ++k) gd[pool[o_off[g] + k]].match_flag = (uint8_t)pool_mf[o_off[g] + k];
                }
            }
        }
        wv::sync();
        HP_LSTAMP(18);
        {
            const GapRest gr = gaps_one_by_one(r, G, gp, GA, pool, pool_n, _line);
            if (gr.pool_n < 0) { arena_release(cx.tmp, mark); return -1; }
            pool_n = gr.pool_n; d_score += gr.d_score; d_NM += gr.d_NM;
        }
    }
    *line_score += d_score; *line_NM += d_NM;
    HP_LSTAMP(19);
    int node_i = 0;
    if (pool_n == 0) {
        HP_G int32_t *g_ln = (HP_G int32_t *)ln;
        for (int q0 = 0; q0 < A; q0 += 64) {
            wv::Lane<int> push, a0, a1;
            WAVE_FOR(l) {
                const int q = q0 + l;
                int p = 0, x0 = 0, x1 = 0;
                if (q < A) { x0 = g_anc[q]; g_ln[q] = x0; if (q > 0) { x1 = g_anc[q - 1]; p = g_ancx[q - 1] - g_ancx[q] > 2; } }
                push[l] = p; a0[l] = x0; a1[l] = x1;
            }
            const unsigned long long m = wv::ballot(push);
            const int cnt = __builtin_popcountll(m);
            if (!cnt) continue;
            if (T.used + cnt > T.cap) { cx.status |= ST_OVERFLOW; break; }
            WAVE_FOR(l) { if (push[l]) { const int at = T.used + __builtin_popcountll(m & ((1ull << l) - 1)); T.n1[at] = a0[l]; T.n2[at] = a1[l]; } }
            T.used += cnt; T.cnt[l_i] += cnt;
        }
        node_i = A;
        wv::sync();
    } else {
        HP_G int32_t *g_ln = (HP_G int32_t *)ln; HP_G int32_t *g_seg = (HP_G int32_t *)(posx + (H + A + 8));
        HP_G int32_t *g_na = g_ancx;
        HP_G int32_t *g_pa = (HP_G int32_t *)posx;
        const HP_G int32_t *gg_after = (const HP_G int32_t *)g_after, *gg_on = (const HP_G int32_t *)o_n, *gg_off = (const HP_G int32_t *)o_off;
        const HP_G int32_t *g_pool = (const HP_G int32_t *)pool;
        const int first = (G > 0 && g_after[0] == -1) ? 1 : 0;
        const int n_first = first ? o_n[0] : 0, off_first = first ? o_off[0] : 0;
        for (int i0 = 0; i0 < A; i0 += 64) { WAVE_FOR(l) { if (i0 + l < A) g_na[i0 + l] = 0; } }
        wv::sync();
        for (int g0 = first; g0 < G; g0 += 64) { WAVE_FOR(l) { const int g = g0 + l; if (g < G) g_na[gg_after[g]] = (gg_on[g] << 1) | 1; } }
        for (int k0 = 0; k0 < n_first; k0 += 64) { WAVE_FOR(l) { const int k = k0 + l; if (k < n_first) { g_ln[k] = g_pool[off_first + n_first - 1 - k]; g_seg[k] = k > 0; } } }
        wv::sync();
        int carry = n_first, carry_has = n_first > 0;
        for (int i0 = 0; i0 < A; i0 += 64) {
            wv::Lane<int> ex, has, pre;
            WAVE_FOR(l) { const int i = i0 + l; const int na = i < A ? g_na[i] : 0; ex[l] = na >> 1; has[l] = na & 1; }
            pre = ex;
            wv::scan_add_excl(pre);
            const int last_has = wv::bcast(has, 63);
            wv::shr1(has, carry_has);
            WAVE_FOR(l) {
                const int i = i0 + l;
                if (i < A) { const int p = i + carry + pre[l]; g_pa[i] = p; g_ln[p] = g_anc[i]; g_seg[p] = has[l]; }
            }
            carry += wv::reduce_sum(ex); carry_has = last_has;
        }
        wv::sync();
        for (int g0 = first; g0 < G; g0 += 64) {
            WAVE_FOR(l) {
                const int g = g0 + l;
                if (g < G) {
                    const int n = gg_on[g], off = gg_off[g], st = g_pa[gg_after[g]] + 1;
                    for (int k = 0; k < n; ++k) { g_ln[st + k] = g_pool[off + n - 1 - k]; g_seg[st + k] = 1; }
                }
            }
        }
        node_i = A + carry;
        wv::sync();
        for (int k0 = 0; k0 < pool_n; k0 += 64) { WAVE_FOR(l) { if (k0 + l < pool_n) gd[pool[k0 + l]].dp_flag = TRACKED_FLAG; } }
        HP_G int32_t *g_px = (HP_G int32_t *)posx;
        for (int q0 = 0; q0 < node_i; q0 += 64) { WAVE_FOR(l) { if (q0 + l < node_i) g_px[q0 + l] = g_seed[g_ln[q0 + l]]; } }
        wv::sync();
        for (int q0 = 1; q0 < node_i; q0 += 64) {
            wv::Lane<int> push;
            WAVE_FOR(l) { const int q = q0 + l; push[l] = q < node_i && g_seg[q] && g_px[q - 1] - g_px[q] > 2; }
            const unsigned long long m = wv::ballot(push);
            const int cnt = __builtin_popcountll(m);
            if (!cnt) continue;
            if (T.used + cnt > T.cap) { cx.status |= ST_OVERFLOW; break; }
            WAVE_FOR(l) { if (push[l]) { const int at = T.used + __builtin_popcountll(m & ((1ull << l) - 1)); T.n1[at] = g_ln[q0 + l]; T.n2[at] = g_ln[q0 + l - 1]; } }
            T.used += cnt; T.cnt[l_i] += cnt;
        }
        wv::sync();
    }
    arena_release(cx.tmp, mark);
    HP_LSTAMP(20);
#undef HP_LSTAMP
    return node_i;
}

}
```

Baseline: 4.188.

## Store diagonal-relative hit positions and template the cluster DP target loop on strand

```diff
diff --git a/lamsa_amd/csrc/hp_align_api.hip b/lamsa_amd/csrc/hp_align_api.hip
--- a/lamsa_amd/csrc/hp_align_api.hip
+++ b/lamsa_amd/csrc/hp_align_api.hip
@@ -470,8 +470,13 @@
         fprintf(stderr, "[HP_PROF] branch tracking (-DHP_PROF_TRACK: the line_build stamps below are off): marking pass, image build and write-back %lld Mcyc; %lld seeds visited; %lld tracks, %lld Mcyc in them, %lld steps up; "
                         "%lld arrivals at a node with several sons, %lld Mcyc in cut_branch\n", sum[16] / 1000000, sum[19], sum[18], sum[17] / 1000000, sum[20], sum[21], sum[22] / 1000000);
 #endif
+#ifdef HP_PROF_EDGE
+        fprintf(stderr, "[HP_PROF] main pass (-DHP_PROF_EDGE: the line_build stamps below are off), Mcyc: dp_cluster_lds load+pack %lld, MIN extension %lld, target loop %lld, write-back %lld; cluster_lane %lld; build_sons %lld\n",
+                sum[16] / 1000000, sum[17] / 1000000, sum[18] / 1000000, sum[19] / 1000000, sum[20] / 1000000, sum[21] / 1000000);
+#else
         fprintf(stderr, "[HP_PROF] line_build: %lld lines (%lld without a gap), %lld anchors, %lld gaps | Mcyc: anchor walk %lld, gap list %lld, gaps in lanes %lld, gaps one by one %lld, assembly %lld\n",
                 sum[21], sum[22], sum[12], sum[23], sum[16] / 1000000, sum[17] / 1000000, sum[18] / 1000000, sum[19] / 1000000, sum[20] / 1000000);
+#endif
         fprintf(stderr, "[HP_PROF] gaps: %lld in lines with fewer than HP_GAP_MIN gaps (%lld lines with gaps); lane gaps: %lld hits scanned, %lld refused (range too long or too many active hits)\n", sum[54], sum[55], sum[11], sum[13]);
         { const char *nm[] = {"ksw_global", "ksw_extend", "backtrack", "ref_fetch", "head_fix", "frag_extend", "split_mapping", "tail_fix", "res_split", "res_aux", "mini_line_regs", "sort index"};
           for (int k = 0; k < 12; ++k) fprintf(stderr, "[HP_PROF] %-16s %8lld Mcyc %10lld calls\n", nm[k], sum[24 + 2 * k] / 1000000, sum[25 + 2 * k]);
diff --git a/lamsa_amd/csrc/hp_chain.h b/lamsa_amd/csrc/hp_chain.h
--- a/lamsa_amd/csrc/hp_chain.h
+++ b/lamsa_amd/csrc/hp_chain.h
@@ -91,6 +91,43 @@
     EdgeK k; k.seed_step = P->seed_step; k.seed_len = P->seed_len; k.match_dis = P->match_dis; k.high_err = P->aln_mode & 2;
     k.mis3 = 3 * P->mismatch_thd; k.sv_len = P->SV_len_thd; k.half_split = P->split_len / 2;
     return k;
+}
+HP_INL int mul24(int a, int k)
+{
+#if defined(__HIP_DEVICE_COMPILE__)
+    int p;
+    asm("v_mul_i32_i24 %0, %1, %2" : "=v"(p) : "s"(__builtin_amdgcn_readfirstlane(k)), "v"(a));
+    return p;
+#else
+    return a * k;
+#endif
+}
+HP_INL EdgeK edge_uni(EdgeK k)
+{
+    k.seed_step = wv::uni(k.seed_step); k.seed_len = wv::uni(k.seed_len); k.match_dis = wv::uni(k.match_dis); k.high_err = wv::uni(k.high_err);
+    k.mis3 = wv::uni(k.mis3); k.sv_len = wv::uni(k.sv_len); k.half_split = wv::uni(k.half_split);
+    return k;
+}
+HP_INL bool edge_k24(const EdgeK &k) { return k.seed_step >= 0 && k.seed_step <= 0x7fffff && k.match_dis >= 0 && k.match_dis <= 0x7fffff; }
+
+HP_INL int hit_diag(const EdgeK &k, int sp, int rel, int sid) { return (int)((unsigned)(sp > 0 ? rel : 0 - rel) - (unsigned)mul24(sid, k.seed_step)); }
+HP_INL int edge_dis(int d_q, int d_t, int ld) { return (int)((unsigned)d_t - (unsigned)d_q - (unsigned)ld); }
+template <bool M24> HP_INL int edge_mul(int a, int k) { return M24 ? mul24(a, k) : a * k; }
+template <bool M24 = true>
+HP_INL int edge_class_diag(const EdgeK &k, int dis, int dsid)
+{
+    const int span = edge_mul<M24>(dsid, k.seed_step);
+    if (span < k.seed_len) return F_UNCONNECT;
+    const int mat_dis = edge_mul<M24>(dsid, k.high_err ? k.match_dis : 0) + (k.high_err ? 0 : k.match_dis);
+    if (dis <= mat_dis && dis >= -mat_dis) return dsid == 1 ? F_MATCH : (dsid <= k.mis3 ? F_MISMATCH : F_LONG_MISMATCH);
+    if (dis > mat_dis && dis < k.sv_len) return F_DELETE;
+    if ((dis < -mat_dis && dis >= k.seed_len - span) || (dis < -k.half_split && dis >= -k.sv_len)) return F_INSERT;
+    return F_UNCONNECT;
+}
+HP_INL bool edge_match_diag(const EdgeK &k, int dis, int dsid)
+{
+    const int mat_dis = mul24(dsid, k.high_err ? k.match_dis : 0) + (k.high_err ? 0 : k.match_dis);
+    return mul24(dsid, k.seed_step) >= k.seed_len && dis <= mat_dis && dis >= -mat_dis;
 }
 HP_INL int edge_flag_packed(const EdgeK &k, const NodeS &pre, const NodeS &cur)
 {
@@ -1518,8 +1555,14 @@
                 if (geo32 && HP_CL_CAP_RT(1 << 20) >= HP_CLL_MCAP) {
                     const EdgeK K = edge_consts(P);
                     wv::sync();
+#ifdef HP_PROF_EDGE
+                    const long long tl0_ = wv::clock();
+#endif
                     WAVE_FOR(l) { const int n = csn[l] - csl[l]; if (l < cn && n >= 2 && n <= HP_CLL_MCAP) { HP_STAT_ADD(34, 1); HP_STAT_MAX(47, n); cluster_lane(r, K, C, r.cx.lds + l, csl[l], n, do_me); } }
                     wv::sync();
+#ifdef HP_PROF_EDGE
+                    if (r.prof) r.prof[20] += wv::clock() - tl0_;
+#endif
                 }
                 for (int q = 0; q < cn; ++q) {
                     const int lo = wv::bcast(csl, q), n = wv::bcast(csl, q + 1) - lo;
@@ -1536,7 +1579,13 @@
             if (any_big) dp_update_range(r, hoff(r, 1), H, 0, MIN_FLAG, false, false, C.big);
         }
         if (!have_cl) arena_release(r.cx.tmp, cmark);
+#ifdef HP_PROF_EDGE
+        const long long ts0_ = wv::clock();
+#endif
         if (!build_sons(r, (HP_L uint64_t *)r.cx.lds, r.cx.lds_words / 2)) return false;
+#ifdef HP_PROF_EDGE
+        if (r.prof) r.prof[21] += wv::clock() - ts0_;
+#endif
     }
 
     HP_CSTAMP(7);
diff --git a/lamsa_amd/csrc/hp_cluster.h b/lamsa_amd/csrc/hp_cluster.h
--- a/lamsa_amd/csrc/hp_cluster.h
+++ b/lamsa_amd/csrc/hp_cluster.h
@@ -189,14 +189,9 @@
 #define HP_CLL_MCAP (HP_LANE_STRIP_WORDS / 384 < 6 ? HP_LANE_STRIP_WORDS / 384 : 6)
 HP_INL int gap_edge(const EdgeK &K, int sp, int qpos, int qsid, int qld, int tpos, int tsid, int tld)
 {
-    const int dsid = tsid - qsid, span = dsid * K.seed_step;
-    if (span < K.seed_len) return F_UNCONNECT;
-    const int dis = sp * (tpos - qpos) - span - (sp > 0 ? qld : tld);
-    const int mat_dis = K.match_dis * (K.high_err ? dsid : 1);
-    if (dis <= mat_dis && dis >= -mat_dis) return dsid == 1 ? F_MATCH : (dsid <= K.mis3 ? F_MISMATCH : F_LONG_MISMATCH);
-    if (dis > mat_dis && dis < K.sv_len) return F_DELETE;
-    if ((dis < -mat_dis && dis >= 0 - (span - K.seed_len)) || (dis < -K.half_split && dis >= -K.sv_len)) return F_INSERT;
-    return F_UNCONNECT;
+    const int dsid = tsid - qsid, d = tpos - qpos;
+    const int dis = (sp > 0 ? d : 0 - d) - dsid * K.seed_step - (sp > 0 ? qld : tld);
+    return edge_class_diag<false>(K, dis, dsid);
 }
 
 HP_INL void cluster_lane(ReadCtx &r, const EdgeK &K, const Clusters &C, HP_L int32_t *strip, int lo, int n, bool do_me)
@@ -300,27 +295,147 @@
 struct ClLds { HP_L int32_t *w0, *w1, *w2, *w3, *w4; };
 HP_INL ClLds cl_lds(HP_L int32_t *lds, int cap) { ClLds c; c.w0 = lds; c.w1 = lds + cap; c.w2 = lds + 2 * cap; c.w3 = lds + 3 * cap; c.w4 = lds + 4 * cap; return c; }
 
-HP_INL NodeS cl_unpack(int w0, int w1, int w2, int w3, int chr, int strand)
-{
-    NodeS q;
-    q.pos = (int64_t)(unsigned)w0; q.chr = chr; q.slot_j = (int)((unsigned)w1 >> 4);
-    q.sid = (int16_t)((unsigned)w2 >> 17); q.strand = (int8_t)strand; q.len_dif8 = (int8_t)((w2 >> 9) & 0xff);
-    q.dp_flag = (int8_t)((int)((unsigned)w1 << 28) >> 28); q.son_flag = (uint8_t)((w2 >> 4) & 31); q.match_flag = (uint8_t)(w2 & 15); q.pad_ = 0;
-    q.score = w3 >> 16; q.NM = w3 & 0xffff;
-    return q;
-}
-
-HP_NOINL bool dp_cluster_lds(ReadCtx &r, const Clusters &C, int lo, int n, bool do_me)
-{
+template <int SP>
+HP_INL void cl_block(const EdgeK &K, int i0, int n, int x, int t0, int tsid, int tld, int t_NM,
+                     const wv::Lane<int> &c0, const wv::Lane<int> &c1, const wv::Lane<int> &c2, const wv::Lane<int> &c3,
+                     wv::Lane<int> &bhi, wv::Lane<int> &blo, wv::Lane<int> &bi, wv::Lane<int> &bf, wv::Lane<int> &negp, wv::Lane<int> &n_i, wv::Lane<int> &n_f, wv::Lane<int> &n_hi)
+{
+    const int dp_flag = MIN_FLAG, POSMAX = (1 << 28) - 1, NEG = -0x7fffffff;
+    WAVE_FOR(l) {
+        const int i = i0 + l;
+        const int q0 = c0[l], q1 = c1[l], q2 = c2[l], q3 = c3[l];
+        const int qslot = (int)((unsigned)q1 >> 18), qdpf = (int)((unsigned)q1 << 28) >> 28;
+        const int dsid = tsid - (int)((unsigned)q2 >> 17);
+        const int qld = (int)(int8_t)((q2 >> 9) & 0xff);
+        const int flag = edge_class_diag(K, edge_dis(q0, t0, SP > 0 ? qld : tld), dsid);
+        int ok = (i < n) & (qslot < x) & (qdpf == dp_flag) & (flag != F_UNCONNECT);
+        if (SP > 0) ok &= ((q2 >> 4) & 31) > F_MATCH_THD;
+        const int pos = ((x - 1 - qslot) << 14) | ((q1 >> 4) & 16383);
+        const int cand = (q3 >> 16) + 1 + score_table(flag);
+        const int hi = ok ? (int)(((unsigned)cand << 16) | (unsigned)(65535 - ((q3 & 0xffff) + t_NM))) : NEG;
+        const int lo_ = POSMAX - pos;
+        const bool better = hi > bhi[l] || (hi == bhi[l] && ok && lo_ > blo[l]);
+        bhi[l] = better ? hi : bhi[l]; blo[l] = better ? lo_ : blo[l]; bi[l] = better ? i : bi[l]; bf[l] = better ? flag : bf[l];
+        if (SP < 0) {
+            const int np = (ok & (flag <= F_MATCH_THD)) ? -pos : NEG;
+            const bool nb_ = np > negp[l];
+            negp[l] = nb_ ? np : negp[l]; n_i[l] = nb_ ? i : n_i[l]; n_f[l] = nb_ ? flag : n_f[l]; n_hi[l] = nb_ ? hi : n_hi[l];
+        }
+    }
+}
+
+#ifndef HP_PAIRS_BLOCK
+#define HP_PAIRS_BLOCK(hits) ((void)0)
+#define HP_PAIRS_TARGET(pairs, blocks_skipped) ((void)0)
+#endif
+template <int SP>
+HP_INL void cl_targets(const ClLds &L, const EdgeK &K, const HP_G int32_t *g_rnk, const HP_G int32_t *g_csrt, int lo, int n, const wv::Lane<int> &bmin, long long &pairs_)
+{
+    const int dp_flag = MIN_FLAG, NEG = -0x7fffffff;
+    const int nb = (n + 63) >> 6, last_short = 64 - (n - ((nb - 1) << 6));
+    for (int o0 = 0; o0 < n; o0 += 64) {
+        wv::Lane<int> tloc, T0, T1, T2, T3;
+        WAVE_FOR(l) {
+            const int o = o0 + l; const int tl = o < n ? g_rnk[g_csrt[lo + o]] - lo : 0;
+            tloc[l] = tl; T0[l] = L.w0[tl]; T1[l] = L.w1[tl]; T2[l] = L.w2[tl]; T3[l] = L.w3[tl];
+        }
+        const int cnt = n - o0 < 64 ? n - o0 : 64;
+        for (int q = 0; q < cnt; ++q) {
+            const int t1 = wv::bcast(T1, q);
+            if ((int)((unsigned)t1 << 28) >> 28 != dp_flag) continue;
+            const int x = (int)((unsigned)t1 >> 18);
+            if (x == 0) continue;
+            wv::Lane<int> bl;
+            WAVE_FOR(l) bl[l] = bmin[l] < x;
+            unsigned long long bm = wv::ballot(bl);
+            if (!bm) continue;
+            pairs_ += 64 * __builtin_popcountll(bm) - (((bm >> (nb - 1)) & 1) ? last_short : 0);
+            HP_PAIRS_TARGET(64 * __builtin_popcountll(bm) - (((bm >> (nb - 1)) & 1) ? last_short : 0), nb - __builtin_popcountll(bm));
+            const int ct = wv::bcast(tloc, q), t0 = wv::bcast(T0, q), t2 = wv::bcast(T2, q), t3 = wv::bcast(T3, q);
+            const int tsid = (int)((unsigned)t2 >> 17), tld = (int)(int8_t)((t2 >> 9) & 0xff), t_score = t3 >> 16, t_NM = t3 & 0xffff;
+            wv::Lane<int> bhi, blo, bi, bf, negp, n_i, n_f, n_hi;
+            WAVE_FOR(l) { bhi[l] = NEG; blo[l] = -1; bi[l] = 0; bf[l] = 0; negp[l] = NEG; n_i[l] = 0; n_f[l] = 0; n_hi[l] = 0; }
+            wv::Lane<int> a0, a1, a2, a3, b0, b1, b2, b3;
+            int ia = __builtin_ctzll(bm) << 6, ib;
+            bm &= bm - 1;
+            WAVE_FOR(l) { const int i = ia + l, ii = i < n ? i : 0; a0[l] = L.w0[ii]; a1[l] = L.w1[ii]; a2[l] = L.w2[ii]; a3[l] = L.w3[ii]; }
+            for (;;) {
+                const bool more_b = bm != 0;
+                ib = more_b ? __builtin_ctzll(bm) << 6 : ia; bm &= bm - 1;
+                WAVE_FOR(l) { const int i = ib + l, ii = i < n ? i : 0; b0[l] = L.w0[ii]; b1[l] = L.w1[ii]; b2[l] = L.w2[ii]; b3[l] = L.w3[ii]; }
+                HP_PAIRS_BLOCK(n - ia < 64 ? n - ia : 64);
+                cl_block<SP>(K, ia, n, x, t0, tsid, tld, t_NM, a0, a1, a2, a3, bhi, blo, bi, bf, negp, n_i, n_f, n_hi);
+                if (!more_b) break;
+                const bool more_a = bm != 0;
+                ia = more_a ? __builtin_ctzll(bm) << 6 : ib; bm &= bm - 1;
+                WAVE_FOR(l) { const int i = ia + l, ii = i < n ? i : 0; a0[l] = L.w0[ii]; a1[l] = L.w1[ii]; a2[l] = L.w2[ii]; a3[l] = L.w3[ii]; }
+                HP_PAIRS_BLOCK(n - ib < 64 ? n - ib : 64);
+                cl_block<SP>(K, ib, n, x, t0, tsid, tld, t_NM, b0, b1, b2, b3, bhi, blo, bi, bf, negp, n_i, n_f, n_hi);
+                if (!more_a) break;
+            }
+            int max_from = -1, max_score = t_score, max_NM = t_NM, max_flag = 0;
+            bool changed = false;
+            if (SP < 0) {
+                const int npos = wv::reduce_max(negp);
+                if (npos != NEG) {
+                    wv::Lane<int> w;
+                    WAVE_FOR(l) w[l] = negp[l] == npos;
+                    const int wl = __builtin_ctzll(wv::ballot(w));
+                    const int hi = wv::bcast(n_hi, wl);
+                    max_from = wv::bcast(n_i, wl); max_flag = wv::bcast(n_f, wl); max_score = hi >> 16; max_NM = 65535 - (hi & 0xffff);
+                    changed = true;
+                }
+            }
+            const int mh = changed ? NEG : wv::reduce_max(bhi);
+            if (!changed && mh == NEG) continue;
+            if (!changed) {
+                const int cand = mh >> 16, nm = 65535 - (mh & 0xffff);
+                if (cand > max_score || (cand == max_score && nm < max_NM)) {
+                    wv::Lane<int> w;
+                    WAVE_FOR(l) w[l] = bhi[l] == mh;
+                    unsigned long long wm = wv::ballot(w);
+                    if (wm & (wm - 1)) {
+                        wv::Lane<int> l2;
+                        WAVE_FOR(l) l2[l] = bhi[l] == mh ? blo[l] : -1;
+                        const int ml = wv::reduce_max(l2);
+                        WAVE_FOR(l) w[l] = bhi[l] == mh && blo[l] == ml;
+                        wm = wv::ballot(w);
+                    }
+                    const int wl = __builtin_ctzll(wm);
+                    max_from = wv::bcast(bi, wl); max_flag = wv::bcast(bf, wl); max_score = cand; max_NM = nm;
+                    changed = true;
+                }
+            }
+            if (changed) {
+                const int f2 = wv::uni(L.w2[max_from]), f4 = wv::uni(L.w4[max_from]);
+                L.w2[max_from] = (f2 & ~(31 << 4)) | ((max_flag & 31) << 4);
+                L.w2[ct] = (t2 & ~15) | (max_flag & 15);
+                L.w3[ct] = (int)(((unsigned)max_score << 16) | ((unsigned)max_NM & 0xffffu));
+                L.w4[ct] = ((max_from + 1) << 16) | (((f4 & 0xffff) + 1) & 0xffff);
+                wv::sync();
+            }
+        }
+    }
+}
+
+HP_NOINL bool dp_cluster_lds(ReadCtx &r, const Clusters &C, int lo_, int n_, bool do_me_)
+{
+    const int lo = wv::uni(lo_), n = wv::uni(n_); const bool do_me = wv::uni(do_me_) != 0;
     const HP_G NodeS *ns = (const HP_G NodeS *)r.nd;
     HP_G NodeS *gd = (HP_G NodeS *)r.nd;
     const HP_G int32_t *g_srt = (const HP_G int32_t *)r.srt, *g_rnk = (const HP_G int32_t *)r.rnk, *g_csrt = (const HP_G int32_t *)C.csrt;
     const HP_G int16_t *g_hnm = (const HP_G int16_t *)r.h_nm;
     HP_G int32_t *g_from = (HP_G int32_t *)r.n_from, *g_node_n = (HP_G int32_t *)r.n_node_n;
     const ClLds L = cl_lds(r.cx.lds, r.cx.lds_words / 5);
-    const EdgeK K = edge_consts(r.cx.P);
-    const int dp_flag = MIN_FLAG;
-    if ((long long)(r.seed_id[r.seed_out - 1] - r.seed_id[0] + 1) * K.seed_step > 0x3fffffffll) return false;
+    const EdgeK K = edge_uni(edge_consts(r.cx.P));
+#ifdef HP_PROF_EDGE
+    long long te_ = wv::clock();
+#define HP_ESTAMP(k) do { const long long now_ = wv::clock(); if (r.prof) r.prof[(k)] += now_ - te_; te_ = now_; } while (0)
+#else
+#define HP_ESTAMP(k) do { } while (0)
+#endif
+    if ((long long)(r.seed_id[r.seed_out - 1] - r.seed_id[0] + 1) * K.seed_step > 0x3fffffffll || !edge_k24(K)) return false;
+    const int sid0 = r.seed_id[0];
     const NodeS first = node_load(ns + g_srt[lo]);
     const int64_t pos0 = first.pos; const int strand = first.strand;
     int nm_sum = 0; int bad = 0;
@@ -336,9 +451,9 @@
                 const int id = g_srt[lo + i];
                 const NodeS q = node_load(ns + id);
                 const int64_t rel = q.pos - pos0;
-                bv = rel < 0 || rel > 0x7ffffff0ll || q.score < -30000 || q.score > 30000 || q.NM < 0 || q.NM > 65535 || q.sid < 0;
+                bv = rel < 0 || rel > 0x3fffff00ll || q.score < -30000 || q.score > 30000 || q.NM < 0 || q.NM > 65535 || q.sid < 0;
                 nmv = g_hnm[id]; sv = 0 - (q.slot_j >> 14);
-                L.w0[i] = (int)(unsigned)rel;
+                L.w0[i] = hit_diag(K, strand, (int)rel, q.sid - sid0);
                 L.w1[i] = (int)(((unsigned)q.slot_j << 4) | ((unsigned)q.dp_flag & 15u));
                 L.w2[i] = (int)(((unsigned)(unsigned short)q.sid << 17) | (((unsigned)q.len_dif8 & 255u) << 9) | (((unsigned)q.son_flag & 31u) << 4) | ((unsigned)q.match_flag & 15u));
                 L.w3[i] = (int)(((unsigned)q.score << 16) | ((unsigned)q.NM & 0xffffu));
@@ -353,8 +468,9 @@
     }
     if (bad || nm_sum > 65535 || n > 64 * 64) return false;
     wv::sync();
-    const int sp = strand, POSMAX = (1 << 28) - 1, NEG = -0x7fffffff;
+    const int sp = strand;
     long long pairs_ = 0;
+    HP_ESTAMP(16);
     if (do_me) {
         const size_t mark = arena_mark(r.cx.tmp);
         int32_t *ml = (int32_t *)arena_alloc(r.cx, sizeof(int32_t) * 2 * (size_t)(n + 64));
@@ -411,10 +527,9 @@
                             int v = 0;
                             if (sd[l] >= 0 && sd[l] != xm) {
                                 const bool q_first = sd[l] < xm;
-                                const int dsid = q_first ? msid - qsid[l] : qsid[l] - msid, span = dsid * K.seed_step;
-                                const int dis = (q_first ? sp * (m0 - q0[l]) : sp * (q0[l] - m0)) - span - (sp > 0 ? (q_first ? qld[l] : mld) : (q_first ? mld : qld[l]));
-                                const int mat_dis = K.match_dis * (K.high_err ? dsid : 1);
-                                v = span >= K.seed_len && dis <= mat_dis && dis >= -mat_dis;
+                                const int dsid = q_first ? msid - qsid[l] : qsid[l] - msid;
+                                const int ld = sp > 0 ? (q_first ? qld[l] : mld) : (q_first ? mld : qld[l]);
+                                v = edge_match_diag(K, q_first ? edge_dis(q0[l], m0, ld) : edge_dis(m0, q0[l], ld), dsid);
                             }
                             q[l] = v;
                         }
@@ -441,91 +556,10 @@
         }
         arena_release(r.cx.tmp, mark);
     }
-    for (int o0 = 0; o0 < n; o0 += 64) {
-        wv::Lane<int> tloc, T0, T1, T2, T3;
-        WAVE_FOR(l) {
-            const int o = o0 + l; const int tl = o < n ? g_rnk[g_csrt[lo + o]] - lo : 0;
-            tloc[l] = tl; T0[l] = L.w0[tl]; T1[l] = L.w1[tl]; T2[l] = L.w2[tl]; T3[l] = L.w3[tl];
-        }
-        const int cnt = n - o0 < 64 ? n - o0 : 64;
-        for (int q = 0; q < cnt; ++q) {
-            const int t1 = wv::bcast(T1, q);
-            if ((int)((unsigned)t1 << 28) >> 28 != dp_flag) continue;
-            const int x = (int)((unsigned)t1 >> 18);
-            if (x == 0) continue;
-            const int ct = wv::bcast(tloc, q), t0 = wv::bcast(T0, q), t2 = wv::bcast(T2, q), t3 = wv::bcast(T3, q);
-            const int tsid = (int)((unsigned)t2 >> 17), tld = (int)(int8_t)((t2 >> 9) & 0xff), t_score = t3 >> 16, t_NM = t3 & 0xffff;
-            wv::Lane<int> bhi, blo, bi, bf, negp, n_i, n_f, n_hi, okl;
-            WAVE_FOR(l) { bhi[l] = NEG; blo[l] = -1; bi[l] = 0; bf[l] = 0; negp[l] = NEG; n_i[l] = 0; n_f[l] = 0; n_hi[l] = 0; okl[l] = 0; }
-            for (int i0 = 0; i0 < n; i0 += 64) {
-                if (wv::bcast(bmin, i0 >> 6) >= x) continue;
-                pairs_ += n - i0 < 64 ? n - i0 : 64;
-                WAVE_FOR(l) {
-                    const int i = i0 + l, ii = i < n ? i : 0;
-                    const int q0 = L.w0[ii], q1 = L.w1[ii], q2 = L.w2[ii], q3 = L.w3[ii];
-                    const int qslot = (int)((unsigned)q1 >> 18), qdpf = (int)((unsigned)q1 << 28) >> 28;
-                    const int dsid = tsid - (int)((unsigned)q2 >> 17);
-                    const int span = dsid * K.seed_step;
-                    const int qld = (int)(int8_t)((q2 >> 9) & 0xff);
-                    const int dis = sp * (t0 - q0) - span - (sp > 0 ? qld : tld);
-                    const int mat_dis = K.match_dis * (K.high_err ? dsid : 1);
-                    int flag = F_UNCONNECT;
-                    if (span >= K.seed_len) {
-                        if (dis <= mat_dis && dis >= -mat_dis) flag = dsid == 1 ? F_MATCH : (dsid <= K.mis3 ? F_MISMATCH : F_LONG_MISMATCH);
-                        else if (dis > mat_dis && dis < K.sv_len) flag = F_DELETE;
-                        else if ((dis < -mat_dis && dis >= 0 - (span - K.seed_len)) || (dis < -K.half_split && dis >= -K.sv_len)) flag = F_INSERT;
-                    }
-                    const int ok = (i < n) & (qslot < x) & (qdpf == dp_flag) & !((sp == 1) & (((q2 >> 4) & 31) <= F_MATCH_THD)) & (flag != F_UNCONNECT);
-                    const int pos = ((x - 1 - qslot) << 14) | ((q1 >> 4) & 16383);
-                    const int cand = (q3 >> 16) + 1 + score_table(flag);
-                    const int hi = ok ? (int)(((unsigned)cand << 16) | (unsigned)(65535 - ((q3 & 0xffff) + t_NM))) : NEG;
-                    const int lo_ = POSMAX - pos;
-                    const bool better = hi > bhi[l] || (hi == bhi[l] && ok && lo_ > blo[l]);
-                    bhi[l] = better ? hi : bhi[l]; blo[l] = better ? lo_ : blo[l]; bi[l] = better ? i : bi[l]; bf[l] = better ? flag : bf[l];
-                    const int np = (ok & (sp == -1) & (flag <= F_MATCH_THD)) ? -pos : NEG;
-                    const bool nb = np > negp[l];
-                    negp[l] = nb ? np : negp[l]; n_i[l] = nb ? i : n_i[l]; n_f[l] = nb ? flag : n_f[l]; n_hi[l] = nb ? hi : n_hi[l];
-                    okl[l] |= ok;
-                }
-            }
-            if (wv::ballot(okl) == 0) continue;
-            int max_from = -1, max_score = t_score, max_NM = t_NM, max_flag = 0;
-            bool changed = false;
-            const int npos = wv::reduce_max(negp);
-            if (npos != NEG) {
-                wv::Lane<int> w;
-                WAVE_FOR(l) w[l] = negp[l] == npos;
-                const int wl = __builtin_ctzll(wv::ballot(w));
-                const int hi = wv::bcast(n_hi, wl);
-                max_from = wv::bcast(n_i, wl); max_flag = wv::bcast(n_f, wl); max_score = hi >> 16; max_NM = 65535 - (hi & 0xffff);
-                changed = true;
-            } else {
-                const int mh = wv::reduce_max(bhi);
-                if (mh != NEG) {
-                    const int cand = mh >> 16, nm = 65535 - (mh & 0xffff);
-                    if (cand > max_score || (cand == max_score && nm < max_NM)) {
-                        wv::Lane<int> l2;
-                        WAVE_FOR(l) l2[l] = bhi[l] == mh ? blo[l] : -1;
-                        const int ml = wv::reduce_max(l2);
-                        wv::Lane<int> w;
-                        WAVE_FOR(l) w[l] = bhi[l] == mh && blo[l] == ml;
-                        const int wl = __builtin_ctzll(wv::ballot(w));
-                        max_from = wv::bcast(bi, wl); max_flag = wv::bcast(bf, wl); max_score = cand; max_NM = nm;
-                        changed = true;
-                    }
-                }
-            }
-            if (changed) {
-                const int f2 = wv::uni(L.w2[max_from]), f4 = wv::uni(L.w4[max_from]);
-                L.w2[max_from] = (f2 & ~(31 << 4)) | ((max_flag & 31) << 4);
-                L.w2[ct] = (t2 & ~15) | (max_flag & 15);
-                L.w3[ct] = (int)(((unsigned)max_score << 16) | ((unsigned)max_NM & 0xffffu));
-                L.w4[ct] = ((max_from + 1) << 16) | (((f4 & 0xffff) + 1) & 0xffff);
-                wv::sync();
-            }
-        }
-    }
+    HP_ESTAMP(17);
+    if (sp > 0) cl_targets<1>(L, K, g_rnk, g_csrt, lo, n, bmin, pairs_); else cl_targets<-1>(L, K, g_rnk, g_csrt, lo, n, bmin, pairs_);
     r.n_pairs += pairs_;
+    HP_ESTAMP(18);
     wv::sync();
     for (int i0 = 0; i0 < n; i0 += 64) {
         WAVE_FOR(l) {
@@ -543,6 +577,8 @@
         }
     }
     wv::sync();
+    HP_ESTAMP(19);
+#undef HP_ESTAMP
     return true;
 }
 
diff --git a/lamsa_amd/csrc/hp_core.h b/lamsa_amd/csrc/hp_core.h
--- a/lamsa_amd/csrc/hp_core.h
+++ b/lamsa_amd/csrc/hp_core.h
@@ -42,6 +42,9 @@
     long long *prof_dp = nullptr;
     int lds_epoch;
 };
+#if defined(HP_PROF_EDGE) && (defined(HP_PROF_TRACK) || defined(HP_PROF_FILL))
+#error "-DHP_PROF_EDGE, -DHP_PROF_TRACK and -DHP_PROF_FILL all use prof slots 16 .. 23: one of them per build"
+#endif
 #ifdef HP_PROF_FILL
 #define HP_PROF_CHAIN_ON 0
 #define HP_TADD_FILL(cx, slot, v) HP_TADD(cx, slot, v)
diff --git a/lamsa_amd/csrc/hp_gaps.h b/lamsa_amd/csrc/hp_gaps.h
--- a/lamsa_amd/csrc/hp_gaps.h
+++ b/lamsa_amd/csrc/hp_gaps.h
@@ -461,7 +461,7 @@
     if (!anc) { arena_release(cx.tmp, mark); return -1; }
     int32_t *anc_x = anc + (H + 2);
     int A = 0;
-#if defined(HP_PROF) && !defined(HP_PROF_TRACK)
+#if defined(HP_PROF) && !defined(HP_PROF_TRACK) && !defined(HP_PROF_EDGE)
     long long tl_ = wv::clock();
 #define HP_LSTAMP(k) do { const long long now_ = wv::clock(); if (r.prof) r.prof[(k)] += now_ - tl_; tl_ = now_; } while (0)
 #else
@@ -501,7 +501,7 @@
     for (int i0 = 0; i0 < A; i0 += 64) { WAVE_FOR(l) { if (i0 + l < A) g_ancx[i0 + l] = g_seed[g_anc[i0 + l]]; } }
     wv::sync();
     HP_LSTAMP(16);
-#if defined(HP_PROF) && !defined(HP_PROF_TRACK)
+#if defined(HP_PROF) && !defined(HP_PROF_TRACK) && !defined(HP_PROF_EDGE)
     if (HP_PROF_CHAIN_ON && r.prof) { r.prof[21] += 1; r.prof[12] += A; }
 #endif
     {
@@ -517,7 +517,7 @@
             wv::sync();
             arena_release(cx.tmp, mark);
             HP_LSTAMP(17);
-#if defined(HP_PROF) && !defined(HP_PROF_TRACK)
+#if defined(HP_PROF) && !defined(HP_PROF_TRACK) && !defined(HP_PROF_EDGE)
             if (HP_PROF_CHAIN_ON && r.prof) r.prof[22] += 1;
 #endif
             return A;
@@ -553,7 +553,7 @@
     }
     wv::sync();
     HP_LSTAMP(17);
-#if defined(HP_PROF) && !defined(HP_PROF_TRACK)
+#if defined(HP_PROF) && !defined(HP_PROF_TRACK) && !defined(HP_PROF_EDGE)
     if (HP_PROF_CHAIN_ON && r.prof) { r.prof[23] += G; if (G < HP_GAP_MIN) r.prof[54] += G; r.prof[55] += 1; }
 #endif
     int pool_n = 0, d_score = 0, d_NM = 0;
```

Result: faster. 4.270, median of 6 (+2.0%).
